# Kloudy-Sky/openintel

Hardware: AMD Instinct MI355X
Metric: queries/sec + p50 latency, 10M-post/768-d hybrid BM25+cosine+RRF top-100 (higher is better)
Workload: dtype f32

## Files before the change

### openintel_amd/csrc/cosine_prefilter.hip

```cpp
#include <algorithm>
#include <cstdlib>
#include <type_traits>

#include "oi_device.h"
#include "oi_internal.h"
#include "oi_lds_dma.h"

typedef float pf_f32x16 __attribute__((ext_vector_type(16)));
typedef float pf_f32x4 __attribute__((ext_vector_type(4)));
typedef __bf16 pf_bf16x8 __attribute__((ext_vector_type(8)));

#define PF_TILE_ROWS 32
#define PF_SLOT_K 32
#define PF_SLOT_BYTES (PF_TILE_ROWS * 128)

__device__ __forceinline__ pf_bf16x8 pf_pack(const pf_f32x4 &a, const pf_f32x4 &b) {
    pf_bf16x8 r;
    r[0] = (__bf16)a[0]; r[1] = (__bf16)a[1]; r[2] = (__bf16)a[2]; r[3] = (__bf16)a[3];
    r[4] = (__bf16)b[0]; r[5] = (__bf16)b[1]; r[6] = (__bf16)b[2]; r[7] = (__bf16)b[3];
    return r;
}

template <int D, int NQT>
__global__ __launch_bounds__(256, 1) void cosine_screen_filter(
    const float *__restrict__ rows, uint64_t row_begin, uint64_t row_end,
    const uint16_t *__restrict__ queries,
    uint32_t n_queries, uint32_t doc_id_base, uint64_t *pools, uint32_t *seg_cnt, uint32_t seg_cnt_stride,
    const uint32_t *tau_keys, uint64_t pool_stride, uint32_t carry_cap, uint32_t seg_cap, uint32_t *overflow) {
    constexpr int NKC = D / PF_SLOT_K;
    constexpr int NBUF = NKC % 8 == 0 ? 8 : (NKC % 6 == 0 ? 6 : NKC);
    constexpr int P = NBUF - 1;
    constexpr int KSTEPS = D / 16;
    static_assert(D % PF_SLOT_K == 0 && NKC % NBUF == 0 && P >= 1 && P < NKC, "unsupported D");
    static_assert(NQT * KSTEPS * 4 <= 400, "the query block must fit the register file");

    extern __shared__ __attribute__((aligned(1024))) unsigned char smem[];
    unsigned char *ring = smem;
    uint32_t *seg_fill = reinterpret_cast<uint32_t *>(smem + 4 * NBUF * PF_SLOT_BYTES);

    OI_CLAIM_WHOLE_SIMD();
    const uint32_t tid = threadIdx.x, lane = tid & 63;
    const uint32_t w = __builtin_amdgcn_readfirstlane(tid >> 6);
    const uint32_t li = lane & 31, lh = lane >> 5;
    uint64_t *stage_keys = reinterpret_cast<uint64_t *>(smem + 4 * NBUF * PF_SLOT_BYTES + 256) + w * OI_STAGE;
    uint32_t *stage_q = reinterpret_cast<uint32_t *>(smem + 4 * NBUF * PF_SLOT_BYTES + 256 + 4 * OI_STAGE * 8) + w * OI_STAGE;
    uint32_t st_head = 0, st_n = 0;

    pf_bf16x8 qreg[NQT][KSTEPS];
#pragma unroll
    for (int t = 0; t < NQT; ++t)
#pragma unroll
        for (int s = 0; s < KSTEPS; ++s)
            qreg[t][s] = *reinterpret_cast<const pf_bf16x8 *>(queries + (uint64_t)(32 * t + li) * D + 16 * s + 8 * lh);
    float tauf[NQT];
#pragma unroll
    for (int t = 0; t < NQT; ++t) {
        const uint32_t q = 32u * t + li;
        const uint32_t k = q < n_queries ? tau_keys[q] : 0xFFFFFFFFu;
        tauf[t] = k <= 0x007FFFFFu ? -__builtin_inff() : oi_key_f32(k);
    }
    if (tid < 32 * NQT) seg_fill[tid] = 0;
    __syncthreads();

    const uint64_t n_rows = row_end - row_begin;
    const uint64_t n_tiles = (n_rows + PF_TILE_ROWS - 1) / PF_TILE_ROWS;
    const uint64_t first = (uint64_t)blockIdx.x * 4 + w, stride = (uint64_t)gridDim.x * 4;
    const uint64_t my_nt = first < n_tiles ? (n_tiles - first + stride - 1) / stride : 0;
    uint64_t *my_seg = pools + carry_cap + (uint64_t)blockIdx.x * seg_cap;

    if (my_nt) {
        uint32_t voff[4];
#pragma unroll
        for (int m = 0; m < 4; ++m) {
            const uint32_t prow = 8 * m + (lane >> 3);
            voff[m] = prow * (uint32_t)(D * 4) + (((lane & 7) ^ ((prow >> 1) & 7)) << 4);
        }
        const uint32_t ring_w = oi_lds_addr(ring) + w * (NBUF * PF_SLOT_BYTES);
        const unsigned char *ring_rd = ring + w * (NBUF * PF_SLOT_BYTES);
        uint32_t frag_off[2][2];
#pragma unroll
        for (int g = 0; g < 2; ++g)
#pragma unroll
            for (int h = 0; h < 2; ++h) frag_off[g][h] = li * 128 + (((4 * g + 2 * lh + h) ^ ((li >> 1) & 7)) << 4);

        auto tile_row0 = [&](uint64_t ti) { return row_begin + (first + ti * stride) * (uint64_t)PF_TILE_ROWS; };
        auto tile_srd = [&](uint64_t ti) {
            const uint64_t r0 = tile_row0(ti < my_nt ? ti : 0);
            return oi_make_srd(rows + r0 * D, ti < my_nt ? (row_end - r0) * (uint64_t)(D * 4) : 0ull);
        };
        oi_u32x4 cur = tile_srd(0), nxt = tile_srd(1);
        __builtin_amdgcn_s_waitcnt(0x0F70);
#pragma unroll
        for (int kc = 0; kc < P; ++kc)
#pragma unroll
            for (int m = 0; m < 4; ++m)
                oi_dma_piece(cur, voff[m], kc * 128, ring_w + (kc % NBUF) * PF_SLOT_BYTES + m * 1024);

        for (uint64_t ti = 0; ti < my_nt; ++ti) {
            pf_f32x16 acc[NQT];
#pragma unroll
            for (int t = 0; t < NQT; ++t)
#pragma unroll
                for (int r = 0; r < 16; ++r) acc[t][r] = 0.f;

            oi_wait_vm<4 * (P - 1)>();
            pf_bf16x8 a_cur = pf_pack(*reinterpret_cast<const pf_f32x4 *>(ring_rd + frag_off[0][0]),
                                      *reinterpret_cast<const pf_f32x4 *>(ring_rd + frag_off[0][1]));
            oi_static_for<0, NKC * 2>([&](auto gi_) {
                constexpr int gi = decltype(gi_)::value;
                constexpr int kc = gi / 2, g = gi % 2;
                constexpr int sn = kc + P;
                pf_f32x4 f0, f1;
                if constexpr (g == 0) {
                    f0 = *reinterpret_cast<const pf_f32x4 *>(ring_rd + (kc % NBUF) * PF_SLOT_BYTES + frag_off[1][0]);
                    f1 = *reinterpret_cast<const pf_f32x4 *>(ring_rd + (kc % NBUF) * PF_SLOT_BYTES + frag_off[1][1]);
                }
#pragma unroll
                for (int t = 0; t < NQT; ++t)
                    acc[t] = __builtin_amdgcn_mfma_f32_32x32x16_bf16(a_cur, qreg[t][gi], acc[t], 0, 0, 0);
#pragma unroll
                for (int m = 2 * g; m < 2 * g + 2; ++m) {
                    if constexpr (sn < NKC)
                        oi_dma_piece(cur, voff[m], sn * 128, ring_w + (sn % NBUF) * PF_SLOT_BYTES + m * 1024);
                    else
                        oi_dma_piece(nxt, voff[m], (sn - NKC) * 128, ring_w + (sn % NBUF) * PF_SLOT_BYTES + m * 1024);
                }
                if constexpr (g == 1 && kc + 1 < NKC) {
                    oi_wait_vm<4 * (P - 1)>();
                    f0 = *reinterpret_cast<const pf_f32x4 *>(ring_rd + ((kc + 1) % NBUF) * PF_SLOT_BYTES + frag_off[0][0]);
                    f1 = *reinterpret_cast<const pf_f32x4 *>(ring_rd + ((kc + 1) % NBUF) * PF_SLOT_BYTES + frag_off[0][1]);
                }
                if constexpr (gi + 1 < NKC * 2) a_cur = pf_pack(f0, f1);
            });

            const uint64_t row0 = tile_row0(ti);
            uint32_t m = 0;
#pragma unroll
            for (int t = 0; t < NQT; ++t)
#pragma unroll
                for (int r = 0; r < 16; ++r) m |= acc[t][r] >= tauf[t] ? 1u << (16 * t + r) : 0u;
            if (row_end - row0 < (uint64_t)PF_TILE_ROWS) {
                const uint32_t left = (uint32_t)(row_end - row0);
#pragma unroll
                for (int r = 0; r < 16; ++r)
                    if ((uint32_t)((r & 3) + 8 * (r >> 2)) + 4u * lh >= left) m &= ~(0x00010001u << r);
            }
            if (__builtin_amdgcn_ballot_w64(m != 0u) != 0ull) {
                const uint32_t cnt = (uint32_t)__builtin_popcount(m);
                const uint32_t incl = oi_wave_incl_scan(cnt);
                const uint32_t total = (uint32_t)__builtin_amdgcn_readlane((int)incl, 63);
                if (total <= OI_STAGE - OI_STAGE_FLUSH) {
                    uint32_t idx = st_head + st_n + incl - cnt;
#pragma unroll
                    for (int t = 0; t < NQT; ++t)
#pragma unroll
                        for (int r = 0; r < 16; ++r)
                            if (m & (1u << (16 * t + r))) {
                                const uint32_t row = (uint32_t)row0 + (r & 3) + 8 * (r >> 2) + 4 * lh;
                                stage_keys[idx & (OI_STAGE - 1)] = oi_rank_key(acc[t][r], doc_id_base + row);
                                stage_q[idx & (OI_STAGE - 1)] = 32u * t + li;
                                ++idx;
                            }
                    st_n += total;
                    while (st_n >= OI_STAGE_FLUSH) {
                        OI_STAGE_FLUSH_TO_POOL(OI_STAGE_FLUSH);
                    }
                } else {
                    uint32_t pos[NQT];
#pragma unroll
                    for (int t = 0; t < NQT; ++t)
                        pos[t] = atomicAdd(&seg_fill[32u * t + li], (uint32_t)__builtin_popcount((m >> (16 * t)) & 0xFFFFu));
#pragma unroll
                    for (int t = 0; t < NQT; ++t) {
                        uint64_t *dst = my_seg + (uint64_t)(32u * t + li) * pool_stride;
#pragma unroll
                        for (int r = 0; r < 16; ++r) {
                            if (m & (1u << (16 * t + r))) {
                                const uint32_t row = (uint32_t)row0 + (r & 3) + 8 * (r >> 2) + 4 * lh;
                                if (pos[t] < seg_cap) dst[pos[t]] = oi_rank_key(acc[t][r], doc_id_base + row);
                                else *overflow = 1u;
                                ++pos[t];
                            }
                        }
                    }
                }
            }
            cur = nxt;
            nxt = tile_srd(ti + 2);
        }
        if (st_n) {
            OI_STAGE_FLUSH_TO_POOL(st_n);
        }
    }
    __syncthreads();
    if (tid < 32 * NQT && tid < n_queries) {
        const uint32_t c = seg_fill[tid];
        seg_cnt[(uint64_t)tid * seg_cnt_stride + blockIdx.x] = c < seg_cap ? c : seg_cap;
    }
}

__global__ __launch_bounds__(256) void pf_row_norm_max_kernel(const float *__restrict__ rows, uint64_t n, uint32_t dim,
                                                              uint32_t *out) {
    double sum_x2 = 0.0, sum_e2 = 0.0;
    const uint32_t lane = threadIdx.x & 63;
    const uint64_t wave = ((uint64_t)blockIdx.x * blockDim.x + threadIdx.x) >> 6;
    const uint64_t n_waves = ((uint64_t)gridDim.x * blockDim.x) >> 6;
    const uint32_t nvec = dim >> 2;
    float best = 0.f, best_e = 0.f;
    bool bad = false;
    for (uint64_t r = wave; r < n; r += n_waves) {
        const float4 *x = reinterpret_cast<const float4 *>(rows + r * dim);
        float ss = 0.f, se = 0.f;
        for (uint32_t v = lane; v < nvec; v += 64) {
            const float4 a = x[v];
            ss = fmaf(a.x, a.x, ss); ss = fmaf(a.y, a.y, ss); ss = fmaf(a.z, a.z, ss); ss = fmaf(a.w, a.w, ss);
            const pf_f32x4 f = {a.x, a.y, a.z, a.w};
            const pf_bf16x8 b = pf_pack(f, f);
            const float e0 = (float)b[0] - a.x, e1 = (float)b[1] - a.y, e2 = (float)b[2] - a.z, e3 = (float)b[3] - a.w;
            se = fmaf(e0, e0, se); se = fmaf(e1, e1, se); se = fmaf(e2, e2, se); se = fmaf(e3, e3, se);
        }
        ss = oi_wave_sum(ss);
        se = oi_wave_sum(se);
        const float nm = sqrtf(ss), ne = sqrtf(se);
        bad = bad || !(nm == nm) || !(ne == ne);
        best = nm > best ? nm : best;
        best_e = ne > best_e ? ne : best_e;
        sum_x2 += (double)ss;
        sum_e2 += (double)se;
    }
    if (lane == 0) {
        atomicMax(out, bad ? 0x7FC00000u : __float_as_uint(best));
        atomicMax(out + 1, bad ? 0x7FC00000u : __float_as_uint(best_e));
        atomicAdd(reinterpret_cast<double *>(out + 2), sum_x2);
        atomicAdd(reinterpret_cast<double *>(out + 4), sum_e2);
    }
}

__global__ __launch_bounds__(256) void pf_row_norm_class_kernel(const float *__restrict__ rows, uint64_t n, uint32_t dim, float X0,
                                                                float E0, uint32_t *cls, uint32_t *bitmap, uint32_t *list,
                                                                uint32_t cap) {
    const uint32_t lane = threadIdx.x & 63;
    const uint64_t wave = ((uint64_t)blockIdx.x * blockDim.x + threadIdx.x) >> 6;
    const uint64_t n_waves = ((uint64_t)gridDim.x * blockDim.x) >> 6;
    const uint32_t nvec = dim >> 2;
    float best = 0.f, best_e = 0.f;
    for (uint64_t r = wave; r < n; r += n_waves) {
        const float4 *x = reinterpret_cast<const float4 *>(rows + r * dim);
        float ss = 0.f, se = 0.f;
        for (uint32_t v = lane; v < nvec; v += 64) {
            const float4 a = x[v];
            ss = fmaf(a.x, a.x, ss); ss = fmaf(a.y, a.y, ss); ss = fmaf(a.z, a.z, ss); ss = fmaf(a.w, a.w, ss);
            const pf_f32x4 f = {a.x, a.y, a.z, a.w};
            const pf_bf16x8 b = pf_pack(f, f);
            const float e0 = (float)b[0] - a.x, e1 = (float)b[1] - a.y, e2 = (float)b[2] - a.z, e3 = (float)b[3] - a.w;
            se = fmaf(e0, e0, se); se = fmaf(e1, e1, se); se = fmaf(e2, e2, se); se = fmaf(e3, e3, se);
        }
        ss = oi_wave_sum(ss);
        se = oi_wave_sum(se);
        const float nm = sqrtf(ss), ne = sqrtf(se);
        if (nm > X0 || ne > E0) {
            if (lane == 0) {
                const uint32_t pos = atomicAdd(cls + 2, 1u);
                if (pos < cap) list[pos] = (uint32_t)r;
                atomicOr(bitmap + (r >> 5), 1u << (r & 31));
            }
        } else {
            best = nm > best ? nm : best;
            best_e = ne > best_e ? ne : best_e;
        }
    }
    if (lane == 0) {
        atomicMax(cls, __float_as_uint(best));
        atomicMax(cls + 1, __float_as_uint(best_e));
    }
}

#define PF_NORM_LIMIT 1.0e15f
#define PF_QNORM_MIN 1.0e-12f
__device__ __forceinline__ float pf_eps(float X, float E, float qn, float qtn, float en, uint32_t dim) {
    const float tiny = 4.0e-18f, d = (float)dim;
    const float Xs = X + tiny, Es = E + tiny, qts = qtn + tiny, ens = en + tiny;
    const float acc = d * 2.384185791015625e-07f;
    return 1.001f * (Es * qts + Xs * ens + acc * (Xs + Es) * qts) + d * 7.5231638452626401e-37f * (Xs + qn) + 1.0e-30f;
}

__global__ __launch_bounds__(256) void pf_stage_queries_kernel(const float *__restrict__ q, uint32_t n_queries,
                                                               uint32_t n_padded, uint32_t dim,
                                                               const uint32_t *__restrict__ max_norm_bits,
                                                               uint16_t *__restrict__ out, float *__restrict__ eps2,
                                                               uint32_t *gate) {
    const uint32_t lane = threadIdx.x & 63;
    const uint32_t wave = (blockIdx.x * blockDim.x + threadIdx.x) >> 6, n_waves = (gridDim.x * blockDim.x) >> 6;
    for (uint32_t row = wave; row < n_padded; row += n_waves) {
        float ss = 0.f, st = 0.f, se = 0.f;
        for (uint32_t k = lane; k < dim; k += 64) {
            uint16_t v = 0;
            if (row < n_queries) {
                const float f = q[(uint64_t)row * dim + k];
                const uint32_t u = __float_as_uint(f);
                v = (u & 0x7F800000u) == 0x7F800000u ? (uint16_t)(u >> 16)
                                                     : (uint16_t)((u + 0x7FFFu + ((u >> 16) & 1u)) >> 16);
                const float ft = __uint_as_float((uint32_t)v << 16), e = ft - f;
                ss = fmaf(f, f, ss);
                st = fmaf(ft, ft, st);
                se = fmaf(e, e, se);
            }
            out[(uint64_t)row * dim + k] = v;
        }
        if (row < n_queries) {
            ss = oi_wave_sum(ss);
            st = oi_wave_sum(st);
            se = oi_wave_sum(se);
            const float qn = sqrtf(ss), qtn = sqrtf(st), en = sqrtf(se);
            const float X = __uint_as_float(max_norm_bits[0]), E = __uint_as_float(max_norm_bits[1]);
            const bool ok = qn < PF_NORM_LIMIT && qn >= PF_QNORM_MIN && qtn < PF_NORM_LIMIT && X < PF_NORM_LIMIT &&
                            E < PF_NORM_LIMIT && en == en;
            if (lane == 0) {
                eps2[row] = ok ? 2.0f * pf_eps(X, E, qn, qtn, en, dim) : __builtin_inff();
                if (!ok) *gate = 1u;
            }
        }
    }
}

__global__ __launch_bounds__(64) void pf_probe_kernel(const float *__restrict__ rows, uint64_t row_begin, uint32_t n_rows,
                                                      uint32_t dim, const uint16_t *__restrict__ queries,
                                                      uint32_t n_queries, float *__restrict__ out) {
    const uint32_t lane = threadIdx.x, li = lane & 31, lh = lane >> 5;
    const uint32_t r0 = blockIdx.x * 32, q0 = blockIdx.y * 32;
    pf_f32x16 acc;
#pragma unroll
    for (int r = 0; r < 16; ++r) acc[r] = 0.f;
    const uint32_t row = r0 + li < n_rows ? r0 + li : n_rows - 1;
    const float *x = rows + (row_begin + row) * (uint64_t)dim;
    const uint16_t *qq = queries + (uint64_t)(q0 + li) * dim;
    for (uint32_t k = 0; k < dim; k += 16) {
        const pf_bf16x8 a = pf_pack(*reinterpret_cast<const pf_f32x4 *>(x + k + 8 * lh),
                                    *reinterpret_cast<const pf_f32x4 *>(x + k + 8 * lh + 4));
        const pf_bf16x8 b = *reinterpret_cast<const pf_bf16x8 *>(qq + k + 8 * lh);
        acc = __builtin_amdgcn_mfma_f32_32x32x16_bf16(a, b, acc, 0, 0, 0);
    }
#pragma unroll
    for (int r = 0; r < 16; ++r) {
        const uint32_t rr = r0 + (r & 3) + 8 * (r >> 2) + 4 * lh, qx = q0 + li;
        if (rr < n_rows && qx < n_queries) out[(uint64_t)qx * n_rows + rr] = acc[r];
    }
}

__global__ __launch_bounds__(256) void pf_make_copy_kernel(const float *__restrict__ rows, uint64_t n_vec8, uint4 *__restrict__ out) {
    for (uint64_t i = (uint64_t)blockIdx.x * blockDim.x + threadIdx.x; i < n_vec8; i += (uint64_t)gridDim.x * blockDim.x) {
        const pf_f32x4 a = *reinterpret_cast<const pf_f32x4 *>(rows + i * 8), b = *reinterpret_cast<const pf_f32x4 *>(rows + i * 8 + 4);
        const pf_bf16x8 v = pf_pack(a, b);
        out[i] = *reinterpret_cast<const uint4 *>(&v);
    }
}
int oi_launch_make_screen_copy(oi_ctx *ctx, const float *rows, uint64_t n, uint32_t dim, uint16_t *out) {
    const uint64_t n_vec8 = n * dim / 8;
    if (n_vec8 == 0) return OI_OK;
    const uint64_t blocks = std::min<uint64_t>((n_vec8 + 255) / 256, (uint64_t)ctx->num_cus * 16);
    hipLaunchKernelGGL(pf_make_copy_kernel, dim3((uint32_t)blocks), dim3(256), 0, ctx->stream, rows, n_vec8, reinterpret_cast<uint4 *>(out));
    OI_HIP_CHECK(hipGetLastError());
    return OI_OK;
}

__global__ __launch_bounds__(256) void pf_rescore_kernel(const float *__restrict__ rows, uint32_t dim, uint32_t doc_id_base,
                                                         uint64_t n_rows, const float *__restrict__ queries,
                                                         const uint64_t *__restrict__ in_pools, const uint32_t *__restrict__ in_cnt,
                                                         uint64_t in_stride, uint32_t cap, uint64_t *out_pools,
                                                         uint32_t *out_cnt, uint64_t out_stride,
                                                         const uint32_t *__restrict__ extra_docs, uint32_t n_extra,
                                                         const uint32_t *__restrict__ spec_max, const uint32_t *__restrict__ tau_final,
                                                         uint32_t *gate, uint32_t *fail_host,
                                                         const uint4 *__restrict__ filt, const uint2 *__restrict__ attrs) {
    if (spec_max && blockIdx.x == 0 && threadIdx.x == 0 && spec_max[blockIdx.y] > tau_final[blockIdx.y]) {
        gate[0] = 1u;
        if (fail_host) *fail_host = 1u;
    }
    const uint32_t q = blockIdx.y, lane = threadIdx.x & 63;
    const uint32_t wave = (blockIdx.x * blockDim.x + threadIdx.x) >> 6, n_waves = (gridDim.x * blockDim.x) >> 6;
    uint32_t c0 = in_cnt[q];
    c0 = c0 < cap ? c0 : cap;
    const uint32_t c = c0 + n_extra;
    const uint32_t nvec = dim >> 2;
    const uint4 fq = filt ? filt[q] : make_uint4(0u, 0u, 0u, 0u);
    auto long_passing = [&](uint32_t j) {
        uint32_t cnt = 0;
        for (uint32_t k0 = 0; k0 < j; k0 += 64) {
            const uint32_t k = k0 + lane;
            cnt += (uint32_t)__popcll(__builtin_amdgcn_ballot_w64(k < j && oi_doc_passes(fq, attrs[extra_docs[k]])));
        }
        return cnt;
    };
    const float4 *qv = reinterpret_cast<const float4 *>(queries + (uint64_t)q * dim);
    for (uint32_t i0 = wave * 4u; i0 < c; i0 += n_waves * 4u) {
        uint32_t doc[4];
        const float4 *x[4];
        float a[4];
#pragma unroll
        for (int u = 0; u < 4; ++u) {
            const uint32_t i = i0 + u < c ? i0 + u : c - 1u;
            doc[u] = i < c0 ? oi_rank_key_doc(in_pools[(uint64_t)q * in_stride + i]) : doc_id_base + extra_docs[i - c0];
            const uint64_t r = (uint64_t)(doc[u] - doc_id_base);
            x[u] = reinterpret_cast<const float4 *>(rows + (r < n_rows ? r : 0) * dim);
            a[u] = 0.f;
        }
        for (uint32_t v = lane; v < nvec; v += 64) {
            const float4 yv = qv[v];
            float4 xv[4];
#pragma unroll
            for (int u = 0; u < 4; ++u) xv[u] = oi_load_stream(x[u] + v);
#pragma unroll
            for (int u = 0; u < 4; ++u) {
                a[u] = oi_fma_unpacked(xv[u].x, yv.x, a[u]); a[u] = oi_fma_unpacked(xv[u].y, yv.y, a[u]);
                a[u] = oi_fma_unpacked(xv[u].z, yv.z, a[u]); a[u] = oi_fma_unpacked(xv[u].w, yv.w, a[u]);
            }
        }
#pragma unroll
        for (int u = 0; u < 4; ++u) {
            const uint64_t r = (uint64_t)(doc[u] - doc_id_base);
            float s = oi_wave_sum(a[u]);
            if (!(r < n_rows)) s = 0.f;
            if (filt && i0 + u >= c0 && i0 + u < c) {
                const uint32_t j = i0 + u - c0, slot = c0 + long_passing(j);
                if (lane == 0 && oi_doc_passes(fq, attrs[extra_docs[j]])) out_pools[(uint64_t)q * out_stride + slot] = oi_rank_key(s, doc[u]);
                continue;
            }
            if (lane == 0 && i0 + u < c) out_pools[(uint64_t)q * out_stride + i0 + u] = oi_rank_key(s, doc[u]);
        }
    }
    if (filt) {
        if (blockIdx.x == 0 && threadIdx.x < 64) {
            const uint32_t cf = c0 + long_passing(n_extra);
            if (threadIdx.x == 0) out_cnt[q] = cf;
        }
    } else if (blockIdx.x == 0 && threadIdx.x == 0) out_cnt[q] = c;
}

__global__ __launch_bounds__(256) void pf_spec_kernel(const uint64_t *__restrict__ pools, const uint32_t *__restrict__ carry_cnt,
                                                      uint64_t stride, uint32_t cap, uint32_t r, const float *__restrict__ eps2,
                                                      const uint32_t *__restrict__ tau_keys, uint32_t *spec_tau, uint32_t *spec_max) {
    __shared__ uint32_t hist[256];
    __shared__ uint32_t s_prefix, s_rank;
    const uint32_t q = blockIdx.x, tid = threadIdx.x;
    uint32_t c = carry_cnt[q];
    if (c > cap) c = cap;
    const uint32_t tau = tau_keys[q];
    if (r == 0 || c < r) {
        if (tid == 0) spec_tau[q] = tau;
        return;
    }
    const uint64_t *k = pools + (uint64_t)q * stride;
    if (tid == 0) { s_prefix = 0; s_rank = r; }
    for (int shift = 24; shift >= 0; shift -= 8) {
        hist[tid] = 0;
        __syncthreads();
        const uint32_t prefix = s_prefix, rank = s_rank, himask = shift == 24 ? 0u : 0xFFFFFFFFu << (shift + 8);
        for (uint32_t i = tid; i < c; i += 256) {
            const uint32_t sk = (uint32_t)(k[i] >> 32);
            if ((sk & himask) == prefix) atomicAdd(&hist[(sk >> shift) & 255u], 1u);
        }
        __syncthreads();
        if (tid < 64) {
            const uint32_t h0 = hist[4 * tid], h1 = hist[4 * tid + 1], h2 = hist[4 * tid + 2], h3 = hist[4 * tid + 3];
            const uint32_t own = h0 + h1 + h2 + h3;
            uint32_t v = own;
#pragma unroll
            for (int o = 1; o < 64; o <<= 1) {
                const uint32_t t = __shfl_down(v, o, 64);
                if (tid + o < 64) v += t;
            }
            uint32_t above = v - own;
            const uint32_t hd[4] = {h3, h2, h1, h0};
#pragma unroll
            for (int d = 0; d < 4; ++d) {
                if (above < rank && rank <= above + hd[d]) {
                    s_prefix = prefix | ((uint32_t)(4 * tid + 3 - d) << shift);
                    s_rank = rank - above;
                }
                above += hd[d];
            }
        }
        __syncthreads();
    }
    if (tid == 0) {
        const float s = oi_key_f32(s_prefix) - eps2[q];
        const uint32_t T = s == s ? oi_f32_key(s) : 0u;
        const uint32_t st = T > tau ? T : tau;
        spec_tau[q] = st;
        if (st > tau && st > spec_max[q]) spec_max[q] = st;
    }
}
int oi_launch_spec_threshold(oi_ctx *ctx, const PoolView &pool, uint32_t n_queries, uint32_t r, const float *eps2, uint32_t *spec_tau,
                             uint32_t *spec_max) {
    if (n_queries == 0) return OI_OK;
    ProfScope ps(ctx, "spec");
    hipLaunchKernelGGL(pf_spec_kernel, dim3(n_queries), dim3(256), 0, ctx->stream, pool.keys, pool.carry_cnt, pool.stride, pool.carry_cap, r,
                       eps2, pool.tau_keys, spec_tau, spec_max);
    OI_HIP_CHECK(hipGetLastError());
    return OI_OK;
}

bool oi_cosine_screen_supported(uint32_t dim) { return dim == 384 || dim == 768; }

void oi_cosine_screen_geometry(const oi_ctx *ctx, uint64_t n_rows, uint32_t *n_segs, uint32_t *seg_cap) {
    const uint64_t n_tiles = (n_rows + PF_TILE_ROWS - 1) / PF_TILE_ROWS;
    const uint64_t quads = (n_tiles + 3) / 4;
    const char *cus_s = oi_ablation_env("OI_SCREEN_CUS");
    const uint64_t cus = cus_s ? (uint64_t)std::max(1, atoi(cus_s)) : std::max<uint64_t>(1, (uint64_t)ctx->num_cus * 7 / 8);
    static const bool small_full = oi_ablation_env("OI_SCREEN_SMALL_FULL") != nullptr;
    const uint64_t grid = small_full && quads <= (uint64_t)ctx->num_cus ? (quads ? quads : 1) : (quads < cus ? (quads ? quads : 1) : cus);
    *n_segs = (uint32_t)grid;
    *seg_cap = (uint32_t)((quads + grid - 1) / grid) * 4 * PF_TILE_ROWS;
}

int oi_launch_row_norm_classes(oi_ctx *ctx, const float *rows, uint64_t n, uint32_t dim, float X0, float E0, uint32_t *cls,
                               uint32_t *bitmap, uint32_t *list, uint32_t cap) {
    OI_HIP_CHECK(hipMemsetAsync(cls, 0, 16, ctx->stream));
    OI_HIP_CHECK(hipMemsetAsync(bitmap, 0, ((n + 31) / 32) * 4, ctx->stream));
    uint64_t blocks = (n + 3) / 4;
    const uint64_t capb = (uint64_t)ctx->num_cus * 8;
    if (blocks > capb) blocks = capb;
    hipLaunchKernelGGL(pf_row_norm_class_kernel, dim3((uint32_t)blocks), dim3(256), 0, ctx->stream, rows, n, dim, X0, E0, cls, bitmap,
                       list, cap);
    OI_HIP_CHECK(hipGetLastError());
    return OI_OK;
}

int oi_launch_row_norm_max(oi_ctx *ctx, const float *rows, uint64_t n, uint32_t dim, uint32_t *max_bits) {
    OI_HIP_CHECK(hipMemsetAsync(max_bits, 0, 24, ctx->stream));
    if (n == 0) return OI_OK;
    uint64_t blocks = (n + 3) / 4;
    const uint64_t cap = (uint64_t)ctx->num_cus * 8;
    if (blocks > cap) blocks = cap;
    hipLaunchKernelGGL(pf_row_norm_max_kernel, dim3((uint32_t)blocks), dim3(256), 0, ctx->stream, rows, n, dim, max_bits);
    OI_HIP_CHECK(hipGetLastError());
    return OI_OK;
}

int oi_launch_screen_stage(oi_ctx *ctx, const float *d_queries, uint32_t n_queries, uint32_t dim,
                           const uint32_t *max_norm_bits, uint16_t *q_bf16, float *eps2, uint32_t *gate) {
    const uint32_t n_padded = (n_queries + 31u) & ~31u;
    hipLaunchKernelGGL(pf_stage_queries_kernel, dim3((n_padded + 3) / 4), dim3(256), 0, ctx->stream, d_queries, n_queries,
                       n_padded, dim, max_norm_bits, q_bf16, eps2, gate);
    OI_HIP_CHECK(hipGetLastError());
    return OI_OK;
}

template <int D, int NQT>
static int launch_screen(oi_ctx *ctx, const float *rows, uint64_t row_begin, uint64_t row_end, const uint16_t *q,
                         uint32_t nq, uint32_t doc_id_base, const PoolView &p) {
    constexpr int NKC = D / PF_SLOT_K, NBUF = NKC % 8 == 0 ? 8 : (NKC % 6 == 0 ? 6 : NKC);
    constexpr size_t smem = 4 * NBUF * PF_SLOT_BYTES + 64 * 4 + OI_STAGE_LDS;
    OI_CHECK(oi_dyn_lds(ctx, reinterpret_cast<const void *>(cosine_screen_filter<D, NQT>), (size_t)(smem)));
    hipLaunchKernelGGL((cosine_screen_filter<D, NQT>), dim3(p.n_segs), dim3(256), smem, ctx->stream, rows, row_begin,
                       row_end, q, nq, doc_id_base, p.keys, p.seg_cnt, p.seg_cnt_stride, p.tau_keys, p.stride,
                       p.carry_cap, p.seg_cap, p.overflow);
    OI_HIP_CHECK(hipGetLastError());
    return OI_OK;
}

int oi_launch_cosine_screen_chunk(oi_ctx *ctx, const float *rows, uint64_t row_begin, uint64_t row_end, uint32_t dim,
                                  const uint16_t *q_bf16, uint32_t n_queries, uint32_t doc_id_base, PoolView &pool) {
    OI_REQUIRE(oi_cosine_screen_supported(dim), "cosine screen: dim %u not instantiated (384, 768)", dim);
    oi_cosine_screen_geometry(ctx, row_end > row_begin ? row_end - row_begin : 0, &pool.n_segs, &pool.seg_cap);
    OI_REQUIRE(pool.n_segs <= pool.seg_cnt_stride && pool.carry_cap + (uint64_t)pool.n_segs * pool.seg_cap <= pool.stride,
               "cosine screen: chunk does not fit the candidate pool");
    OI_REQUIRE(!pool.filt, "cosine screen: a filtered search does not take the f32-stream screen (search.hip routes it)");
    if (row_end <= row_begin || n_queries == 0) return OI_OK;
    ProfScope ps(ctx, "cosine");
    for (uint32_t q0 = 0; q0 < n_queries; q0 += 64) {
        const uint32_t nq_here = std::min(64u, n_queries - q0);
        PoolView p = pool.for_queries(q0);
        static const bool tau_max = oi_ablation_env("OI_SCREEN_TAU_MAX") != nullptr;
        if (tau_max && row_end - row_begin >= (1u << 20)) {
            DevBuf &tb = ctx->buf("abl_tau_max");
            if (!tb.p) { OI_CHECK(tb.ensure(4096 * 4)); OI_HIP_CHECK(hipMemsetAsync(tb.p, 0xFF, 4096 * 4, ctx->stream)); }
            p.tau_keys = tb.as<uint32_t>();
        }
        const uint16_t *qptr = q_bf16 + (uint64_t)q0 * dim;
        const bool two = nq_here > 32;
        if (dim == 768) {
            if (two) OI_CHECK((launch_screen<768, 2>(ctx, rows, row_begin, row_end, qptr, nq_here, doc_id_base, p)));
            else OI_CHECK((launch_screen<768, 1>(ctx, rows, row_begin, row_end, qptr, nq_here, doc_id_base, p)));
        } else {
            if (two) OI_CHECK((launch_screen<384, 2>(ctx, rows, row_begin, row_end, qptr, nq_here, doc_id_base, p)));
            else OI_CHECK((launch_screen<384, 1>(ctx, rows, row_begin, row_end, qptr, nq_here, doc_id_base, p)));
        }
    }
    return OI_OK;
}

int oi_launch_rescore(oi_ctx *ctx, const float *rows, uint64_t n_rows, uint32_t dim, uint32_t doc_id_base,
                      const float *d_queries, uint32_t n_queries, const PoolView &in, const PoolView &out,
                      const uint32_t *extra_docs, uint32_t n_extra, const uint32_t *spec_max, const uint32_t *tau_final,
                      uint32_t *gate, uint32_t *fail_host) {
    if (n_queries == 0) return OI_OK;
    OI_REQUIRE(out.carry_cap >= in.carry_cap + n_extra, "rescore: output pool too small");
    ProfScope ps(ctx, "rescore");
    hipLaunchKernelGGL(pf_rescore_kernel, dim3(64, n_queries), dim3(256), 0, ctx->stream, rows, dim, doc_id_base, n_rows,
                       d_queries, in.keys, in.carry_cnt, in.stride, in.carry_cap, out.keys, out.carry_cnt, out.stride, extra_docs,
                       n_extra, spec_max, tau_final, gate, fail_host, out.filt, out.attrs);
    OI_HIP_CHECK(hipGetLastError());
    return OI_OK;
}

int oi_launch_screen_probe(oi_ctx *ctx, const float *rows, uint64_t row_begin, uint32_t n_rows, uint32_t dim,
                           const uint16_t *q_bf16, uint32_t n_queries, float *d_out) {
    if (n_rows == 0 || n_queries == 0) return OI_OK;
    OI_REQUIRE(dim % 16 == 0, "screen probe: dim %u is not a multiple of 16", dim);
    hipLaunchKernelGGL(pf_probe_kernel, dim3((n_rows + 31) / 32, (n_queries + 31) / 32), dim3(64), 0, ctx->stream, rows,
                       row_begin, n_rows, dim, q_bf16, n_queries, d_out);
    OI_HIP_CHECK(hipGetLastError());
    return OI_OK;
}
```

### openintel_amd/csrc/cosine_screen_i8.hip

```cpp
#include <algorithm>
#include <cmath>
#include <cstdlib>
#include <type_traits>

#include "oi_device.h"
#include "oi_internal.h"
#include "oi_lds_dma.h"

typedef int i8s_i32x4 __attribute__((ext_vector_type(4)));
typedef int i8s_i32x16 __attribute__((ext_vector_type(16)));
typedef float i8s_f32x2 __attribute__((ext_vector_type(2)));
template <int N>
struct i8s_ivec {
    typedef int type __attribute__((ext_vector_type(N)));
};

#define I8S_TILE_ROWS 32
#define I8S_SLOT_BYTES (I8S_TILE_ROWS * 128)
#define I8S_META_BYTES 256
#define I8S_PAD_ROWS 64

size_t oi_screen_i8_meta_offset(uint64_t n, uint32_t dim) { return ((size_t)n * dim + 255) & ~(size_t)255; }
size_t oi_screen_i8_bytes(uint64_t n, uint32_t dim) {
    return oi_screen_i8_meta_offset(n, dim) + 8 * ((size_t)n + I8S_PAD_ROWS) + 256;
}

__global__ __launch_bounds__(256) void i8s_make_kernel(const float *__restrict__ rows, uint64_t n, uint32_t dim,
                                                       const uint32_t *__restrict__ long_bitmap, uint32_t *__restrict__ out_i8,
                                                       float *__restrict__ meta, uint32_t *__restrict__ emax_bits) {
    const uint32_t lane = threadIdx.x & 63;
    const uint64_t wave = ((uint64_t)blockIdx.x * blockDim.x + threadIdx.x) >> 6;
    const uint64_t n_waves = ((uint64_t)gridDim.x * blockDim.x) >> 6;
    const uint32_t nv = dim >> 2;
    float best = 0.f;
    for (uint64_t r = wave; r < n; r += n_waves) {
        const float4 *x = reinterpret_cast<const float4 *>(rows + r * dim);
        float4 v[3];
        float amax = 0.f;
#pragma unroll
        for (int u = 0; u < 3; ++u) {
            const uint32_t j = lane + 64u * u;
            v[u] = j < nv ? x[j] : make_float4(0.f, 0.f, 0.f, 0.f);
            amax = fmaxf(amax, fmaxf(fmaxf(fabsf(v[u].x), fabsf(v[u].y)), fmaxf(fabsf(v[u].z), fabsf(v[u].w))));
        }
#pragma unroll
        for (int o = 32; o > 0; o >>= 1) amax = fmaxf(amax, __shfl_xor(amax, o, OI_WAVE));
        const float s = amax / 127.f;
        double e2 = 0.0;
#pragma unroll
        for (int u = 0; u < 3; ++u) {
            const uint32_t j = lane + 64u * u;
            const float xs[4] = {v[u].x, v[u].y, v[u].z, v[u].w};
            uint32_t packed = 0;
#pragma unroll
            for (int c = 0; c < 4; ++c) {
                float t = s > 0.f ? rintf(xs[c] / s) : 0.f;
                t = fminf(127.f, fmaxf(-127.f, t));
                const int iv = (int)t;
                const double e = (double)s * (double)iv - (double)xs[c];
                e2 += j < nv ? e * e : 0.0;
                packed |= ((uint32_t)iv & 0xFFu) << (8 * c);
            }
            if (j < nv) out_i8[r * nv + j] = packed;
        }
        e2 = oi_wave_sum(e2);
        const float er = (float)sqrt(e2) * 1.00000095367431640625f;
        if (lane == 0) {
            meta[2 * r] = s;
            meta[2 * r + 1] = er;
        }
        const bool is_long = long_bitmap && ((long_bitmap[r >> 5] >> (r & 31)) & 1u);
        if (!is_long) best = fmaxf(best, er);
    }
    if (lane == 0) atomicMax(emax_bits, __float_as_uint(best));
}

int oi_launch_make_screen_i8(oi_ctx *ctx, const float *rows, uint64_t n, uint32_t dim, const uint32_t *long_bitmap, uint8_t *out) {
    OI_REQUIRE(oi_cosine_screen_supported(dim), "int8 screening copy: dim %u not instantiated (384, 768)", dim);
    const size_t mo = oi_screen_i8_meta_offset(n, dim);
    OI_HIP_CHECK(hipMemsetAsync(out + mo, 0, 8 * ((size_t)n + I8S_PAD_ROWS) + 256, ctx->stream));
    if (n == 0) return OI_OK;
    uint64_t blocks = (n + 3) / 4;
    const uint64_t cap = (uint64_t)ctx->num_cus * 8;
    if (blocks > cap) blocks = cap;
    float *meta = reinterpret_cast<float *>(out + mo);
    hipLaunchKernelGGL(i8s_make_kernel, dim3((uint32_t)blocks), dim3(256), 0, ctx->stream, rows, n, dim, long_bitmap,
                       reinterpret_cast<uint32_t *>(out), meta, reinterpret_cast<uint32_t *>(meta + 2 * (n + I8S_PAD_ROWS)));
    OI_HIP_CHECK(hipGetLastError());
    return OI_OK;
}

#define I8S_NORM_LIMIT 1.0e15f
#define I8S_QNORM_MIN 1.0e-12f
__global__ __launch_bounds__(256) void i8s_stage_kernel(const float *__restrict__ q, uint32_t n_queries, uint32_t n_padded, uint32_t dim,
                                                        const uint32_t *__restrict__ max_norm_bits, const uint32_t *__restrict__ emax_bits,
                                                        int8_t *__restrict__ qi8, float *__restrict__ qf, uint32_t *gate) {
    const uint32_t lane = threadIdx.x & 63;
    const uint32_t wave = (blockIdx.x * blockDim.x + threadIdx.x) >> 6, n_waves = (gridDim.x * blockDim.x) >> 6;
    for (uint32_t row = wave; row < n_padded; row += n_waves) {
        const bool real = row < n_queries;
        float amax = 0.f;
        bool fin = true;
        for (uint32_t k = lane; k < dim; k += 64) {
            const float f = real ? q[(uint64_t)row * dim + k] : 0.f;
            fin = fin && (f - f == 0.f);
            amax = fmaxf(amax, fabsf(f));
        }
#pragma unroll
        for (int o = 32; o > 0; o >>= 1) amax = fmaxf(amax, __shfl_xor(amax, o, OI_WAVE));
        fin = __builtin_amdgcn_ballot_w64(!fin) == 0ull;
        const float a = fin ? amax / 127.f : 0.f;
        double qn2 = 0.0, en2 = 0.0;
        for (uint32_t k = lane; k < dim; k += 64) {
            const float f = real ? q[(uint64_t)row * dim + k] : 0.f;
            float h = 0.f, l = 0.f;
            if (a > 0.f) {
                const float t = f / a;
                h = fminf(127.f, fmaxf(-127.f, rintf(t)));
                l = fminf(127.f, fmaxf(-127.f, rintf((t - h) * 128.f)));
            }
            const double qh = (double)a * ((double)h + (double)l * 0.0078125);
            qn2 += qh * qh;
            en2 += (qh - (double)f) * (qh - (double)f);
            qi8[(uint64_t)row * dim + k] = (int8_t)(int)h;
            qi8[((uint64_t)n_padded + row) * dim + k] = (int8_t)(int)l;
        }
        qn2 = oi_wave_sum(qn2);
        en2 = oi_wave_sum(en2);
        if (lane == 0) {
            const float up = 1.00000095367431640625f;
            const float qn = (float)sqrt(qn2) * up, en = (float)sqrt(en2) * up;
            const float X = __uint_as_float(max_norm_bits[0]), em = __uint_as_float(*emax_bits);
            const bool ok = fin && amax > 0.f && qn < I8S_NORM_LIMIT && qn >= I8S_QNORM_MIN && X < I8S_NORM_LIMIT && em < I8S_NORM_LIMIT;
            const float rnd = 3.814697265625e-06f + (float)dim * 2.384185791015625e-07f;
            const float cq = 1.001f * (X * en + rnd * (X + em) * (qn + en)) + 1.0e-27f;
            const float m2 = 2.002f * (em * qn + cq);
            qf[row] = ok ? a : 0.f;
            qf[n_padded + row] = ok ? qn : 0.f;
            qf[2 * n_padded + row] = ok ? cq : 0.f;
            qf[3 * n_padded + row] = ok || !real ? m2 : __builtin_inff();
            if (real && !ok) *gate = 1u;
        }
    }
}

int oi_launch_screen_stage_i8(oi_ctx *ctx, const float *d_queries, uint32_t n_queries, uint32_t dim, const uint32_t *max_norm_bits,
                              const uint8_t *i8_copy, uint64_t n_rows, int8_t *qi8, float *qf, uint32_t *gate) {
    const uint32_t n_padded = (n_queries + 31u) & ~31u;
    if (n_padded == 0) return OI_OK;
    const uint32_t *emax = reinterpret_cast<const uint32_t *>(i8_copy + oi_screen_i8_meta_offset(n_rows, dim)) + 2 * (n_rows + I8S_PAD_ROWS);
    hipLaunchKernelGGL(i8s_stage_kernel, dim3((n_padded + 3) / 4), dim3(256), 0, ctx->stream, d_queries, n_queries, n_padded, dim,
                       max_norm_bits, emax, qi8, qf, gate);
    OI_HIP_CHECK(hipGetLastError());
    return OI_OK;
}

__device__ __forceinline__ void i8s_issue_piece(const oi_u32x4 &srd, uint32_t voff, uint32_t soff, uint32_t lds_dst) {
#ifdef I8S_NO_DMA
    (void)srd; (void)voff; (void)soff; (void)lds_dst;
#else
    oi_dma_piece(srd, voff, soff, lds_dst);
#endif
}
__device__ __forceinline__ void i8s_issue_meta(const oi_u32x4 &srd, uint32_t voff, uint32_t lds_dst) {
#ifdef I8S_NO_DMA
    (void)srd; (void)voff; (void)lds_dst;
#else
    uint32_t keep;
    const uint32_t d = __builtin_amdgcn_readfirstlane(lds_dst);
    asm volatile(
        "s_mov_b32 %0, m0\n\t"
        "s_mov_b32 m0, %3\n\t"
        "s_nop 0\n\t"
        "buffer_load_dword %1, %2, 0 offen " OI_DMA_NT "lds\n\t"
        "s_mov_b32 m0, %0"
        : "=&s"(keep)
        : "v"(voff), "s"(srd), "s"(d)
        : "memory");
#endif
}

template <int D, int NQT, int NBUF, bool FILT>
__global__ __launch_bounds__(256, 1) void cosine_i8_screen(
    const uint8_t *__restrict__ rows, const float *__restrict__ meta, uint64_t row_begin, uint64_t row_end,
    const int8_t *__restrict__ qhi, const int8_t *__restrict__ qlo,
    const float *__restrict__ qf, uint32_t qf_stride, uint32_t n_queries, uint32_t doc_id_base, uint64_t *pools, uint32_t *seg_cnt,
    uint32_t seg_cnt_stride, const uint32_t *tau_keys, uint64_t pool_stride, uint32_t carry_cap, uint32_t seg_cap, uint32_t *overflow,
    const uint4 *__restrict__ filt, const uint2 *__restrict__ attrs) {
    constexpr int NKC = D / 128;
    constexpr int P = NBUF - 1;
    constexpr int KSTEPS = D / 32;
    constexpr uint32_t RING = NBUF * I8S_SLOT_BYTES;
    static_assert(D % 128 == 0 && P >= 2 && P <= 2 * NKC, "unsupported ring depth for this D");
    constexpr uint32_t QLO_LDS = NQT * KSTEPS * 64 * 16;
    static_assert(NQT * KSTEPS * 4 <= 200, "the hi query block must fit the register file");
    static_assert(4 * RING + 4 * 2 * I8S_META_BYTES + 256 + OI_STAGE_LDS + QLO_LDS <= 160 * 1024, "LDS");

    extern __shared__ __attribute__((aligned(1024))) unsigned char smem[];
    unsigned char *ring = smem;
    unsigned char *meta_lds = smem + 4 * RING;
    uint32_t *seg_fill = reinterpret_cast<uint32_t *>(smem + 4 * RING + 8 * I8S_META_BYTES);
    unsigned char *stage_base = smem + 4 * RING + 8 * I8S_META_BYTES + 256;
    unsigned char *qlo_lds = stage_base + OI_STAGE_LDS;

    OI_CLAIM_WHOLE_SIMD();
    const uint32_t tid = threadIdx.x, lane = tid & 63;
    const uint32_t w = __builtin_amdgcn_readfirstlane(tid >> 6);
    const uint32_t li = lane & 31, lh = lane >> 5;
    uint64_t *stage_keys = reinterpret_cast<uint64_t *>(stage_base) + w * OI_STAGE;
    uint32_t *stage_q = reinterpret_cast<uint32_t *>(stage_base + 4 * OI_STAGE * 8) + w * OI_STAGE;
    uint32_t st_head = 0, st_n = 0;

    i8s_i32x4 qh[NQT][KSTEPS];
#pragma unroll
    for (int t = 0; t < NQT; ++t)
#pragma unroll
        for (int s = 0; s < KSTEPS; ++s)
            qh[t][s] = *reinterpret_cast<const i8s_i32x4 *>(qhi + (uint64_t)(32 * t + li) * D + 32 * s + 16 * lh);
    for (uint32_t c = tid; c < (uint32_t)(NQT * KSTEPS * 64); c += 256) {
        const uint32_t t = c / (KSTEPS * 64), s = (c / 64) % KSTEPS, l = c % 64;
        *reinterpret_cast<i8s_i32x4 *>(qlo_lds + c * 16) =
            *reinterpret_cast<const i8s_i32x4 *>(qlo + (uint64_t)(32 * t + (l & 31)) * D + 32 * s + 16 * (l >> 5));
    }
    float qa[NQT], qn[NQT], cq[NQT], tc[NQT];
#pragma unroll
    for (int t = 0; t < NQT; ++t) {
        const uint32_t q = 32u * t + li;
        const bool real = q < n_queries;
        const uint32_t k = real ? tau_keys[q] : 0xFFFFFFFFu;
        const float tau = k <= 0x007FFFFFu ? -__builtin_inff() : oi_key_f32(k);
        qa[t] = real ? qf[q] * 0.0078125f : 0.f;
        qn[t] = real ? qf[qf_stride + q] : 0.f;
        cq[t] = real ? qf[2 * qf_stride + q] : 0.f;
        const float m2 = real ? qf[3 * qf_stride + q] : 0.f;
        const float T = m2 < __builtin_inff() ? (tau + m2) - (fabsf(tau) + m2) * 9.5367431640625e-07f : -__builtin_inff();
        tc[t] = T - cq[t];
    }
    if (tid < 32 * NQT) seg_fill[tid] = 0;
#ifdef I8S_NO_DMA
    for (uint32_t i = tid; i < (4 * RING + 8 * I8S_META_BYTES) / 4; i += 256) reinterpret_cast<uint32_t *>(smem)[i] = 0u;
#endif
    __syncthreads();

    const uint64_t n_rows = row_end - row_begin;
    const uint64_t n_tiles = (n_rows + I8S_TILE_ROWS - 1) / I8S_TILE_ROWS;
    const uint64_t first = (uint64_t)blockIdx.x * 4 + w, stride = (uint64_t)gridDim.x * 4;
    const uint64_t my_nt = first < n_tiles ? (n_tiles - first + stride - 1) / stride : 0;
    uint64_t *my_seg = pools + carry_cap + (uint64_t)blockIdx.x * seg_cap;

    if (my_nt) {
        uint32_t voff[4];
#pragma unroll
        for (int m = 0; m < 4; ++m) {
            const uint32_t prow = 8 * m + (lane >> 3);
            voff[m] = prow * (uint32_t)D + (((lane & 7) ^ ((prow >> 1) & 7)) << 4);
        }
        const uint32_t ring_w = oi_lds_addr(ring) + w * RING;
        const unsigned char *ring_rd = ring + w * RING;
        const uint32_t meta_w = oi_lds_addr(meta_lds) + w * 2 * I8S_META_BYTES;
        const unsigned char *meta_rd = meta_lds + w * 2 * I8S_META_BYTES;
        uint32_t frag_off[4];
#pragma unroll
        for (int g = 0; g < 4; ++g) frag_off[g] = li * 128 + (((2 * g + lh) ^ ((li >> 1) & 7)) << 4);

        auto tile_row0 = [&](uint64_t ti) { return row_begin + (first + ti * stride) * (uint64_t)I8S_TILE_ROWS; };
        auto tile_srd = [&](uint64_t ti) {
            const uint64_t r0 = tile_row0(ti < my_nt ? ti : 0);
            return oi_make_srd(rows + r0 * D, ti < my_nt ? (row_end - r0) * (uint64_t)D : 0ull);
        };
        auto issue_meta = [&](uint64_t ti) {
            const uint64_t r0 = tile_row0(ti);
            i8s_issue_meta(oi_make_srd(meta + 2 * r0, (row_end - r0) * 8ull), lane * 4u, meta_w + (uint32_t)(ti & 1) * I8S_META_BYTES);
        };
        oi_u32x4 s0 = tile_srd(0), s1 = tile_srd(1), s2 = tile_srd(2);
        __builtin_amdgcn_s_waitcnt(0x0F70);
        oi_static_for<0, P>([&](auto j_) {
            constexpr int j = decltype(j_)::value;
            constexpr int tj = j / NKC, kj = j % NKC;
#pragma unroll
            for (int m = 0; m < 4; ++m)
                i8s_issue_piece(tj == 0 ? s0 : (tj == 1 ? s1 : s2), voff[m], kj * 128, ring_w + j * I8S_SLOT_BYTES + m * 1024);
        });
        issue_meta(0);
        uint32_t rd_off = 0, wr_off = (NBUF - 1) * I8S_SLOT_BYTES;
        auto lo_frag = [&](int t, int s) {
            return *reinterpret_cast<const i8s_i32x4 *>(qlo_lds + ((t * KSTEPS + s) * 64 + lane) * 16);
        };
        i8s_i32x4 b_cur[NQT];
#ifndef I8S_NO_MFMA
#pragma unroll
        for (int t = 0; t < NQT; ++t) b_cur[t] = lo_frag(t, 0);
#endif

        oi_wait_vm<4 * (P - 1)>();
        i8s_i32x4 a_cur = *reinterpret_cast<const i8s_i32x4 *>(ring_rd + frag_off[0]);

        constexpr int NS = 16 * NQT;
        constexpr int RPK = KSTEPS >= 20 ? 1 : 2;
        constexpr int NSL = 16 / RPK, T0 = 4;
        static_assert(T0 + NSL <= KSTEPS, "the tile test does not fit the span");
        static_assert(4 * NKC + 4 >= 4 * (P - 1) - 1, "the ring's wait in k-step 3 must retire the previous tile's metadata");
        typename i8s_ivec<NS>::type S;
#pragma unroll
        for (int i = 0; i < NS; ++i) S[i] = 0;
        i8s_i32x16 ah[NQT], al[NQT];
        i8s_f32x2 md_cur[RPK];
#pragma unroll
        for (int u = 0; u < RPK; ++u) md_cur[u] = i8s_f32x2{0.f, 0.f};
        const uint32_t lh32 = 32u * lh;
        auto meta_row = [&](const unsigned char *mt, int r) {
            return *reinterpret_cast<const i8s_f32x2 *>(mt + lh32 + ((r & 3) + 8 * (r >> 2)) * 8);
        };
        auto test_row = [&](int t, int r, const i8s_f32x2 md) -> uint32_t {
            const float sc = oi_mul_unpacked((float)S[16 * t + r], oi_mul_unpacked(md[0], qa[t]));
            return sc >= oi_fma_unpacked(-md[1], qn[t], tc[t]) ? 1u << (16 * t + r) : 0u;
        };

        for (uint64_t ti = 0;; ++ti) {
            const bool live = ti < my_nt;
            const unsigned char *mt = meta_rd + (uint32_t)((ti + 1) & 1) * I8S_META_BYTES;
            uint32_t m = 0;
            if (live) {
#pragma unroll
                for (int t = 0; t < NQT; ++t)
#pragma unroll
                    for (int r = 0; r < 16; ++r) { ah[t][r] = 0; al[t][r] = 0; }

                oi_static_for<0, NKC * 4>([&](auto gi_) {
                    constexpr int gi = decltype(gi_)::value;
                    constexpr int kc = gi / 4, g = gi % 4;
                    constexpr int sn = kc + P;
                    constexpr int tn = sn / NKC, kn = sn % NKC;
                    i8s_i32x4 a_nxt;
                    if constexpr (g < 3) {
                        a_nxt = *reinterpret_cast<const i8s_i32x4 *>(ring_rd + rd_off + frag_off[g + 1]);
                    } else {
                        oi_wait_vm<4 * (P - 1) - 1>();
                        const uint32_t nx_off = rd_off + I8S_SLOT_BYTES == RING ? 0u : rd_off + I8S_SLOT_BYTES;
                        a_nxt = *reinterpret_cast<const i8s_i32x4 *>(ring_rd + nx_off + frag_off[0]);
                    }
                    i8s_f32x2 md_nxt[RPK];
                    if constexpr (gi >= T0 - 1 && gi < T0 - 1 + NSL) {
#pragma unroll
                        for (int u = 0; u < RPK; ++u) md_nxt[u] = meta_row(mt, RPK * (gi - (T0 - 1)) + u);
                    }
#ifndef I8S_NO_MFMA
                    i8s_i32x4 b_nxt[NQT];
#pragma unroll
                    for (int t = 0; t < NQT; ++t) b_nxt[t] = lo_frag(t, (gi + 1) % KSTEPS);
#endif
                    __builtin_amdgcn_sched_barrier(0);
#pragma unroll
                    for (int t = 0; t < NQT; ++t) {
#ifndef I8S_NO_MFMA
                        ah[t] = __builtin_amdgcn_mfma_i32_32x32x32_i8(a_cur, qh[t][gi], ah[t], 0, 0, 0);
                        al[t] = __builtin_amdgcn_mfma_i32_32x32x32_i8(a_cur, b_cur[t], al[t], 0, 0, 0);
#else
                        asm volatile("" : : "v"(a_cur));
#endif
                        if constexpr (gi >= T0 && gi < T0 + NSL) if (t == 0) {
#pragma unroll
                            for (int u = 0; u < RPK; ++u)
#pragma unroll
                                for (int tt = 0; tt < NQT; ++tt) m |= test_row(tt, RPK * (gi - T0) + u, md_cur[u]);
                            asm volatile("" : "+v"(m));
                        }
                        __builtin_amdgcn_sched_barrier(0);
                    }
#ifndef I8S_NO_MFMA
#pragma unroll
                    for (int t = 0; t < NQT; ++t) b_cur[t] = b_nxt[t];
#endif
                    if constexpr (gi >= T0 - 1 && gi < T0 - 1 + NSL) {
#pragma unroll
                        for (int u = 0; u < RPK; ++u) md_cur[u] = md_nxt[u];
                    }
                    i8s_issue_piece(tn == 0 ? s0 : (tn == 1 ? s1 : s2), voff[g], kn * 128, ring_w + wr_off + g * 1024);
                    if constexpr (g == 3) {
                        wr_off = rd_off;
                        rd_off = rd_off + I8S_SLOT_BYTES == RING ? 0u : rd_off + I8S_SLOT_BYTES;
                    }
                    a_cur = a_nxt;
                });
            } else {
                oi_wait_vm<0>();
#pragma unroll
                for (int r = 0; r < 16; ++r) {
                    const i8s_f32x2 md = meta_row(mt, r);
#pragma unroll
                    for (int t = 0; t < NQT; ++t) m |= test_row(t, r, md);
                }
            }

            const uint64_t row0 = tile_row0(ti ? ti - 1 : 0);
            if (ti == 0) m = 0u;
            if (row_end - row0 < (uint64_t)I8S_TILE_ROWS) {
                const uint32_t left = (uint32_t)(row_end - row0);
#pragma unroll
                for (int r = 0; r < 16; ++r)
                    if ((uint32_t)((r & 3) + 8 * (r >> 2)) + 4u * lh >= left) m &= ~(0x00010001u << r);
            }
#if defined(I8S_NO_DMA) || defined(I8S_NO_MFMA)
            if (seg_cap != 0xFFFFFFFFu) m = 0u;
#endif
            if (__builtin_amdgcn_ballot_w64(m != 0u) != 0ull) {
                if constexpr (FILT) m = oi_filter_tile<NQT>(m, filt, attrs, row0, lh, li);
                const uint32_t cnt = (uint32_t)__builtin_popcount(m);
                const uint32_t incl = oi_wave_incl_scan(cnt);
                const uint32_t total = (uint32_t)__builtin_amdgcn_readlane((int)incl, 63);
                const uint32_t any = oi_wave_or(m);
                auto lower_key = [&](int t, uint32_t r) -> uint64_t {
                    const uint32_t rit = (r & 3) + 8 * (r >> 2) + 4 * lh;
                    const i8s_f32x2 md = *reinterpret_cast<const i8s_f32x2 *>(mt + rit * 8);
                    const float sc = (float)S[16 * t + r] * (md[0] * qa[t]);
                    return oi_rank_key(sc - fmaf(md[1], qn[t], cq[t]), doc_id_base + ((uint32_t)row0 + rit));
                };
                if (total <= OI_STAGE - OI_STAGE_FLUSH) {
                    uint32_t idx = st_head + st_n + incl - cnt;
#pragma unroll
                    for (int t = 0; t < NQT; ++t)
                        for (uint32_t wd = (any >> (16 * t)) & 0xFFFFu; wd; wd &= wd - 1) {
                            const uint32_t r = (uint32_t)__builtin_ctz(wd);
                            if (m & (1u << (16 * t + r))) {
                                stage_keys[idx & (OI_STAGE - 1)] = lower_key(t, r);
                                stage_q[idx & (OI_STAGE - 1)] = 32u * t + li;
                                ++idx;
                            }
                        }
                    st_n += total;
                    while (st_n >= OI_STAGE_FLUSH) {
                        OI_STAGE_FLUSH_TO_POOL(OI_STAGE_FLUSH);
                    }
                } else {
                    uint32_t pos[NQT];
#pragma unroll
                    for (int t = 0; t < NQT; ++t)
                        pos[t] = atomicAdd(&seg_fill[32u * t + li], (uint32_t)__builtin_popcount((m >> (16 * t)) & 0xFFFFu));
#pragma unroll
                    for (int t = 0; t < NQT; ++t) {
                        uint64_t *dst = my_seg + (uint64_t)(32u * t + li) * pool_stride;
                        for (uint32_t wd = (any >> (16 * t)) & 0xFFFFu; wd; wd &= wd - 1) {
                            const uint32_t r = (uint32_t)__builtin_ctz(wd);
                            if (m & (1u << (16 * t + r))) {
                                if (pos[t] < seg_cap) dst[pos[t]] = lower_key(t, r);
                                else *overflow = 1u;
                                ++pos[t];
                            }
                        }
                    }
                }
            }
            if (!live) break;
#pragma unroll
            for (int t = 0; t < NQT; ++t)
#pragma unroll
                for (int r = 0; r < 16; ++r) S[16 * t + r] = ah[t][r] * 128 + al[t][r];
            if (ti + 1 < my_nt) issue_meta(ti + 1);
            s0 = s1;
            s1 = s2;
            s2 = tile_srd(ti + 3);
        }
        if (st_n) {
            OI_STAGE_FLUSH_TO_POOL(st_n);
        }
        oi_wait_vm<0>();
    }
    __syncthreads();
    if (tid < 32 * NQT && tid < n_queries) {
        const uint32_t c = seg_fill[tid];
        seg_cnt[(uint64_t)tid * seg_cnt_stride + blockIdx.x] = c < seg_cap ? c : seg_cap;
    }
}

template <int D, int NQT, int NBUF, bool FILT>
static int launch_i8_screen_k(oi_ctx *ctx, const uint8_t *rows, const float *meta, uint64_t row_begin, uint64_t row_end, const int8_t *qhi,
                              const int8_t *qlo, const float *qf, uint32_t qf_stride, uint32_t nq, uint32_t doc_id_base, const PoolView &p) {
    constexpr size_t smem = 4 * NBUF * I8S_SLOT_BYTES + 8 * I8S_META_BYTES + 256 + OI_STAGE_LDS + NQT * (D / 32) * 64 * 16;
    OI_CHECK(oi_dyn_lds(ctx, reinterpret_cast<const void *>(cosine_i8_screen<D, NQT, NBUF, FILT>), (size_t)(smem)));
    hipLaunchKernelGGL((cosine_i8_screen<D, NQT, NBUF, FILT>), dim3(p.n_segs), dim3(256), smem, ctx->stream, rows, meta, row_begin, row_end,
                       qhi, qlo, qf, qf_stride, nq, doc_id_base, p.keys, p.seg_cnt, p.seg_cnt_stride, p.tau_keys, p.stride, p.carry_cap,
                       p.seg_cap, p.overflow, p.filt, p.attrs);
    OI_HIP_CHECK(hipGetLastError());
    return OI_OK;
}
template <int D, int NQT, int NBUF>
static int launch_i8_screen(oi_ctx *ctx, const uint8_t *rows, const float *meta, uint64_t row_begin, uint64_t row_end, const int8_t *qhi,
                            const int8_t *qlo, const float *qf, uint32_t qf_stride, uint32_t nq, uint32_t doc_id_base, const PoolView &p) {
    return p.filt ? launch_i8_screen_k<D, NQT, NBUF, true>(ctx, rows, meta, row_begin, row_end, qhi, qlo, qf, qf_stride, nq, doc_id_base, p)
                  : launch_i8_screen_k<D, NQT, NBUF, false>(ctx, rows, meta, row_begin, row_end, qhi, qlo, qf, qf_stride, nq, doc_id_base, p);
}

int oi_launch_cosine_screen_i8_chunk(oi_ctx *ctx, const uint8_t *i8_copy, uint64_t n_rows_total, uint64_t row_begin, uint64_t row_end,
                                     uint32_t dim, const int8_t *qi8, const float *qf, uint32_t n_queries, uint32_t doc_id_base,
                                     PoolView &pool) {
    OI_REQUIRE(oi_cosine_screen_supported(dim), "cosine screen (int8): dim %u not instantiated (384, 768)", dim);
    OI_REQUIRE(row_end <= n_rows_total, "cosine screen (int8): rows past the copy");
    oi_cosine_screen_geometry(ctx, row_end > row_begin ? row_end - row_begin : 0, &pool.n_segs, &pool.seg_cap);
    OI_REQUIRE(pool.n_segs <= pool.seg_cnt_stride && pool.carry_cap + (uint64_t)pool.n_segs * pool.seg_cap <= pool.stride,
               "cosine screen (int8): chunk does not fit the candidate pool");
    if (row_end <= row_begin || n_queries == 0) return OI_OK;
    const float *meta = reinterpret_cast<const float *>(i8_copy + oi_screen_i8_meta_offset(n_rows_total, dim));
    const uint32_t np = (n_queries + 31u) & ~31u;
    ProfScope ps(ctx, "cosine");
    for (uint32_t q0 = 0; q0 < n_queries; q0 += 64) {
        const uint32_t nq_here = std::min(64u, n_queries - q0);
        const PoolView p = pool.for_queries(q0);
        const int8_t *qhi = qi8 + (uint64_t)q0 * dim, *qlo = qi8 + ((uint64_t)np + q0) * dim;
        const float *qfp = qf + q0;
        const bool two = nq_here > 32;
        if (dim == 768) {
            if (two) OI_CHECK((launch_i8_screen<768, 2, 6>(ctx, i8_copy, meta, row_begin, row_end, qhi, qlo, qfp, np, nq_here, doc_id_base, p)));
            else OI_CHECK((launch_i8_screen<768, 1, 6>(ctx, i8_copy, meta, row_begin, row_end, qhi, qlo, qfp, np, nq_here, doc_id_base, p)));
        } else {
            if (two) OI_CHECK((launch_i8_screen<384, 2, 6>(ctx, i8_copy, meta, row_begin, row_end, qhi, qlo, qfp, np, nq_here, doc_id_base, p)));
            else OI_CHECK((launch_i8_screen<384, 1, 6>(ctx, i8_copy, meta, row_begin, row_end, qhi, qlo, qfp, np, nq_here, doc_id_base, p)));
        }
    }
    return OI_OK;
}

__device__ __forceinline__ float i8s_bf16_lo(uint32_t w) { return __uint_as_float(w << 16); }
__device__ __forceinline__ float i8s_bf16_hi(uint32_t w) { return __uint_as_float(w & 0xFFFF0000u); }
__global__ __launch_bounds__(256) void pf_rescreen_kernel(const uint16_t *__restrict__ copy, uint64_t n_rows, uint32_t dim,
                                                          uint32_t doc_id_base, const uint16_t *__restrict__ qb, uint64_t *pools,
                                                          const uint32_t *__restrict__ cnt, uint64_t stride, uint32_t cap) {
    const uint32_t q = blockIdx.y, lane = threadIdx.x & 63;
    const uint32_t wave = (blockIdx.x * blockDim.x + threadIdx.x) >> 6, n_waves = (gridDim.x * blockDim.x) >> 6;
    uint32_t c = cnt[q];
    c = c < cap ? c : cap;
    uint64_t *keys = pools + (uint64_t)q * stride;
    const uint32_t nvec = dim >> 3;
    const uint4 *qv = reinterpret_cast<const uint4 *>(qb + (uint64_t)q * dim);
    for (uint32_t i0 = wave * 4u; i0 < c; i0 += n_waves * 4u) {
        uint32_t doc[4];
        const uint4 *x[4];
        float a[4];
#pragma unroll
        for (int u = 0; u < 4; ++u) {
            const uint32_t i = i0 + u < c ? i0 + u : c - 1u;
            doc[u] = oi_rank_key_doc(keys[i]);
            const uint64_t r = (uint64_t)(doc[u] - doc_id_base);
            x[u] = reinterpret_cast<const uint4 *>(copy + (r < n_rows ? r : 0) * dim);
            a[u] = 0.f;
        }
        for (uint32_t v = lane; v < nvec; v += 64) {
            const uint4 yv = qv[v];
            uint4 xv[4];
#pragma unroll
            for (int u = 0; u < 4; ++u) xv[u] = oi_load_stream(x[u] + v);
#pragma unroll
            for (int u = 0; u < 4; ++u) {
                const uint32_t xw[4] = {xv[u].x, xv[u].y, xv[u].z, xv[u].w}, yw[4] = {yv.x, yv.y, yv.z, yv.w};
#pragma unroll
                for (int e = 0; e < 4; ++e) {
                    a[u] = oi_fma_unpacked(i8s_bf16_lo(xw[e]), i8s_bf16_lo(yw[e]), a[u]);
                    a[u] = oi_fma_unpacked(i8s_bf16_hi(xw[e]), i8s_bf16_hi(yw[e]), a[u]);
                }
            }
        }
        float s[4];
#pragma unroll
        for (int u = 0; u < 4; ++u) s[u] = oi_wave_sum(a[u]);
#pragma unroll
        for (int u = 0; u < 4; ++u) {
            const uint64_t r = (uint64_t)(doc[u] - doc_id_base);
            const float sc = r < n_rows ? s[u] : 0.f;
            if (lane == 0 && i0 + u < c) keys[i0 + u] = oi_rank_key(sc, doc[u]);
        }
    }
}

int oi_launch_rescreen_bf16(oi_ctx *ctx, const uint16_t *copy_rows, uint64_t n_rows, uint32_t dim, uint32_t doc_id_base,
                            const uint16_t *q_bf16, uint32_t n_queries, const PoolView &pool) {
    if (n_queries == 0) return OI_OK;
    ProfScope ps(ctx, "rescreen");
    hipLaunchKernelGGL(pf_rescreen_kernel, dim3(32, n_queries), dim3(256), 0, ctx->stream, copy_rows, n_rows, dim, doc_id_base, q_bf16,
                       pool.keys, pool.carry_cnt, pool.stride, pool.carry_cap);
    OI_HIP_CHECK(hipGetLastError());
    return OI_OK;
}
```

### openintel_amd/csrc/oi_internal.h

```cpp
#pragma once

#include <hip/hip_runtime.h>

#include <cstdarg>
#include <cstdint>
#include <cstdio>
#include <cstdlib>
#include <cstring>
#include <atomic>
#include <map>
#include <mutex>
#include <string>
#include <utility>
#include <vector>

#include "openintel_hip.h"

void oi_set_error(const char *fmt, ...);

#define OI_HIP_CHECK(expr)                                                                   \
    do {                                                                                     \
        hipError_t oi_e_ = (expr);                                                           \
        if (oi_e_ != hipSuccess) {                                                           \
            oi_set_error("%s failed: %s (%s:%d)", #expr, hipGetErrorString(oi_e_), __FILE__, \
                         __LINE__);                                                          \
            return OI_ERR_HIP;                                                               \
        }                                                                                    \
    } while (0)

#define OI_CHECK(expr)              \
    do {                            \
        int oi_rc_ = (expr);        \
        if (oi_rc_ != OI_OK) return oi_rc_; \
    } while (0)

#define OI_REQUIRE(cond, ...)         \
    do {                              \
        if (!(cond)) {                \
            oi_set_error(__VA_ARGS__); \
            return OI_ERR_INVALID_ARG; \
        }                             \
    } while (0)

struct oi_ctx;
int oi_dyn_lds(oi_ctx *ctx, const void *kernel, size_t bytes);

#ifdef OI_ABLATION
inline const char *oi_ablation_env(const char *name) { return getenv(name); }
#else
inline const char *oi_ablation_env(const char *) { return nullptr; }
#endif

struct DevBuf {
    void *p = nullptr;
    size_t cap = 0;
    bool borrowed = false;
    DevBuf() = default;
    DevBuf(const DevBuf &) = delete;
    DevBuf &operator=(const DevBuf &) = delete;
    ~DevBuf() { release(); }
    int ensure(size_t bytes);
    void release();
    template <class T> T *as() const { return reinterpret_cast<T *>(p); }
};

#define OI_PINNED_STAGE_MAX ((size_t)1 << 20)
struct PinBuf {
    void *p = nullptr;
    size_t cap = 0;
    bool pinned = false;
    PinBuf() = default;
    PinBuf(const PinBuf &) = delete;
    PinBuf &operator=(const PinBuf &) = delete;
    int ensure(size_t bytes);
    void release();
    template <class T> T *as() const { return reinterpret_cast<T *>(p); }
};

struct ProfSpan {
    hipEvent_t a, b;
};

extern std::atomic<uint64_t> g_oi_ws_epoch;

struct GraphEntry {
    uint64_t key[10] = {0, 0, 0, 0, 0, 0, 0, 0, 0, 0};
    uint64_t epoch = 0, last_use = 0;
    int state = 0;
    hipGraph_t graph = nullptr;
    hipGraphExec_t exec = nullptr;
};

struct oi_ctx {
    std::atomic<int> refs{1};
    int device = 0;
    int num_cus = 256;
    hipStream_t stream = nullptr;
    hipStream_t side_stream = nullptr;
    bool side_stream_failed = false;
    hipEvent_t ev_fork = nullptr, ev_join = nullptr;
    bool overlap_legs = true;
    bool speculate = true;
    uint32_t spec_skip = 0, spec_backoff = 0;
    uint32_t *spec_fail_host = nullptr;
    uint64_t spec_searches = 0, spec_failures = 0;
    int cosine_mode = 2;
    std::mutex mu;
    std::map<std::string, DevBuf> ws;
    int prof_enabled = 0;
    const uint32_t *run_gate = nullptr;
    const uint32_t *last_screen_gate = nullptr;
    std::map<std::string, std::vector<ProfSpan>> prof;
    std::vector<hipEvent_t> event_pool;
    bool use_graphs = false;
    std::vector<GraphEntry> graphs;
    uint64_t graph_clock = 0, graph_replays = 0, graph_captures = 0;

    PinBuf pin_in, pin_out;

    DevBuf &buf(const char *name) { return ws[name]; }
    void prof_begin(const char *tag);
    void prof_end(const char *tag);
};

struct ProfScope {
    oi_ctx *c;
    const char *tag;
    bool on;
    ProfScope(oi_ctx *ctx, const char *t) : c(ctx), tag(t) {
        on = c->prof_enabled == 1 || (c->prof_enabled == 2 && strcmp(t, "cosine") == 0);
        if (on) c->prof_begin(tag);
    }
    ~ProfScope() {
        if (on) c->prof_end(tag);
    }
};

#define OI_BM25_FLOOR_RANKS 4
struct oi_index {
    uint64_t uid = 0;
    std::atomic<int> refs{1};
    oi_index *src = nullptr;
    oi_ctx *ctx = nullptr;
    uint64_t n_docs = 0;
    uint32_t dim = 0, vocab = 0, doc_id_base = 0;

    float *rows = nullptr;
    bool rows_owned = false;
    uint16_t *rows_bf16 = nullptr;
    bool rows_bf16_owned = false;
    DevBuf max_row_norm;
    bool screen_ok = false;
    uint32_t n_long = 0;
    DevBuf long_list, long_bitmap;
    DevBuf screen_copy;
    int screen_copy_policy = -1;
    DevBuf screen_i8;
    DevBuf doc_attrs;
    DevBuf signals;

    bool forward_set = false, finalized = false;
    uint64_t total_tokens = 0;
    uint64_t n_postings = 0;
    uint32_t n_blocks = 0;
    uint32_t n_win = 0;
    DevBuf uniq_keys;
    DevBuf tf;
    DevBuf doc_len;
    DevBuf df_local;

    DevBuf postings;
    DevBuf cell_start;
    DevBuf idf;
    DevBuf impact_floor;
    DevBuf fwd_terms;
    DevBuf fwd_offsets;
    float avgdl = 0.f;
    uint32_t max_query_terms = 16;
    int bm25_mode = 0;
    bool is_view = false;
};

int search_lists_device(oi_index *idx, const float *d_qv, const uint32_t *d_qt, const uint32_t *d_qo, uint32_t B, uint32_t depth,
                        float *cos_s, uint32_t *cos_d, uint32_t *cos_c, float *bm_s, uint32_t *bm_d, uint32_t *bm_c,
                        const uint4 *d_filt = nullptr, const uint2 *d_attrs = nullptr);
void oi_spec_take_failure(oi_ctx *ctx);

int oi_launch_lexicon(oi_ctx *ctx, const uint8_t *d_blob, const uint64_t *d_offsets, uint64_t n,
                      uint64_t blob_bytes, double *d_pol, uint8_t *d_spec);
int oi_launch_lexicon_fused(oi_ctx *ctx, const uint8_t *d_blob, const uint64_t *d_offsets, uint64_t n, uint64_t blob_bytes,
                            double *d_pol, uint8_t *d_spec, const uint8_t *d_sources, double tau, oi_social_counters *summary);
int oi_launch_social_summary(oi_ctx *ctx, const uint8_t *d_sources, const double *d_pol,
                             const uint8_t *d_spec, uint64_t n, double tau,
                             oi_social_counters *out_host);
int oi_launch_social_summary_segmented(oi_ctx *ctx, const uint8_t *d_sources, const double *d_pol, const uint8_t *d_spec,
                                       uint64_t n, const uint64_t *d_seg, uint64_t n_seg, double tau,
                                       oi_social_counters *d_out);
int oi_launch_headline_scan(oi_ctx *ctx, const uint8_t *d_blob, const uint64_t *d_offsets, uint64_t n,
                            uint64_t blob_bytes, const uint8_t *ticker, uint64_t ticker_len,
                            const uint8_t *forms_blob, const uint32_t *form_offsets, uint32_t n_forms,
                            uint16_t *d_mask, uint64_t *d_order, uint8_t *d_about);
size_t oi_headline_params_bytes();
int oi_headline_build_params(void *dst, const uint8_t *ticker, uint64_t ticker_len, const uint8_t *forms_blob,
                             const uint32_t *form_offsets, uint32_t n_forms);
int oi_launch_headline_scan_params(oi_ctx *ctx, const uint8_t *d_blob, const uint64_t *d_offsets, uint64_t n,
                                   uint64_t blob_bytes, uint64_t text_bytes, const void *d_params, uint16_t *d_mask,
                                   uint64_t *d_order, uint8_t *d_about);
struct PoolView {
    uint64_t *keys;
    uint32_t *carry_cnt;
    uint32_t *seg_cnt;
    uint32_t *tau_keys;
    uint64_t stride;
    uint32_t carry_cap;
    uint32_t seg_cap;
    uint32_t n_segs;
    uint32_t seg_cnt_stride;
    uint32_t *overflow;
    const uint4 *filt = nullptr;
    const uint2 *attrs = nullptr;

    PoolView for_queries(uint32_t q0) const {
        PoolView p = *this;
        p.keys += (uint64_t)q0 * stride;
        p.carry_cnt += q0;
        p.seg_cnt += (uint64_t)q0 * seg_cnt_stride;
        if (p.tau_keys) p.tau_keys += q0;
        if (p.filt) p.filt += q0;
        return p;
    }
};
struct SelectExtra {
    const float *eps2 = nullptr;
    uint32_t *margin_gate = nullptr;
    const uint32_t *run_gate = nullptr;
    const uint32_t *skip_bitmap = nullptr;
    uint32_t skip_base = 0;
    uint64_t *cand = nullptr;
    uint32_t cand_cap = 0;
    const float *row_meta = nullptr;
    uint32_t meta_base = 0;
    const float *row_qn = nullptr, *row_cq = nullptr;
};
int oi_launch_select(oi_ctx *ctx, const PoolView &pool, uint32_t n_queries, uint32_t k, bool compact,
                     float *out_scores, uint32_t *out_docs, uint32_t *out_counts, uint32_t out_stride,
                     const SelectExtra *extra = nullptr);
int oi_launch_lists_to_pool(oi_ctx *ctx, const float *scores, const uint32_t *docs,
                            const uint32_t *counts, uint64_t shard_stride, uint64_t count_stride,
                            uint32_t n_shards, uint32_t n_queries, uint32_t depth, const PoolView &pool);
int oi_launch_rrf(oi_ctx *ctx, const uint32_t *docs_a, const uint32_t *counts_a, const uint32_t *docs_b,
                  const uint32_t *counts_b, uint32_t n_queries, uint32_t depth, uint32_t k,
                  float *scores_out, uint32_t *docs_out, uint32_t *counts_out);
int oi_launch_collapse(oi_index *idx, const float *d_scores, const uint32_t *d_docs, const uint32_t *d_counts, uint32_t n_queries,
                       uint32_t depth, float threshold, uint32_t k, float *scores_out, uint32_t *docs_out, uint32_t *counts_out,
                       uint32_t *dup_out);
int oi_launch_similar_volume(oi_index *idx, const float *d_q, uint32_t n_queries, const oi_volume_spec &spec, const uint4 *d_filt,
                             uint32_t *d_counts);
int oi_launch_volume_round_queries(oi_ctx *ctx, const float *d_q, uint64_t total, float *d_out);
int oi_launch_pack_signals(oi_ctx *ctx, const double *d_pol, const uint8_t *d_spec, const uint8_t *d_sources, uint64_t n, double tau,
                           uint2 *d_out);
int oi_launch_similar_summary(oi_index *idx, const float *d_q, uint32_t n_queries, const oi_summary_spec &spec, const float *d_thresholds,
                              const uint4 *d_filt, oi_social_counters *d_out);
int oi_launch_cosine_chunk(oi_ctx *ctx, const float *rows, uint64_t row_begin, uint64_t row_end,
                           uint32_t dim, const float *d_queries_padded, uint32_t n_queries,
                           uint32_t n_queries_padded, uint32_t doc_id_base, PoolView &pool);
uint64_t oi_cosine_max_chunk_rows(const oi_ctx *ctx, uint32_t dim, uint32_t n_queries, uint64_t stride,
                                  uint32_t carry_cap);
int oi_launch_l2_normalize(oi_ctx *ctx, float *rows, uint64_t n, uint32_t dim);
bool oi_cosine_split_supported(uint32_t dim);
int oi_launch_cosine_split(oi_ctx *ctx, const float *rows, uint64_t row_begin, uint64_t row_end, uint32_t dim,
                           const float *d_queries, uint32_t nq, uint32_t doc_id_base, const PoolView &p);
bool oi_cosine_bf16_supported(uint32_t dim);
int oi_launch_cosine_bf16_chunk(oi_ctx *ctx, const uint16_t *rows, uint64_t row_begin, uint64_t row_end, uint32_t dim,
                                const float *d_queries, uint32_t n_queries, uint32_t doc_id_base, PoolView &pool);
uint32_t oi_cosine_query_padding(uint32_t n_queries);
bool oi_cosine_ksplit_supported(uint32_t dim);
void oi_cosine_ksplit_geometry(const oi_ctx *ctx, uint64_t n_rows, uint32_t *n_segs, uint32_t *seg_cap);
bool oi_cosine_screen_supported(uint32_t dim);
inline bool oi_index_screenable(const oi_index *idx) {
    return idx->rows && !idx->rows_bf16 && idx->screen_ok && oi_cosine_screen_supported(idx->dim);
}
void oi_cosine_screen_geometry(const oi_ctx *ctx, uint64_t n_rows, uint32_t *n_segs, uint32_t *seg_cap);
int oi_launch_row_norm_max(oi_ctx *ctx, const float *rows, uint64_t n, uint32_t dim, uint32_t *max_bits);
int oi_launch_screen_stage(oi_ctx *ctx, const float *d_queries, uint32_t n_queries, uint32_t dim,
                           const uint32_t *max_norm_bits, uint16_t *q_bf16, float *eps2, uint32_t *gate);
int oi_launch_cosine_screen_chunk(oi_ctx *ctx, const float *rows, uint64_t row_begin, uint64_t row_end, uint32_t dim,
                                  const uint16_t *q_bf16, uint32_t n_queries, uint32_t doc_id_base, PoolView &pool);
int oi_launch_make_screen_copy(oi_ctx *ctx, const float *rows, uint64_t n, uint32_t dim, uint16_t *out);
#define OI_I8_CARRY 16384u
size_t oi_screen_i8_bytes(uint64_t n, uint32_t dim);
size_t oi_screen_i8_meta_offset(uint64_t n, uint32_t dim);
int oi_launch_make_screen_i8(oi_ctx *ctx, const float *rows, uint64_t n, uint32_t dim, const uint32_t *long_bitmap, uint8_t *out);
int oi_launch_screen_stage_i8(oi_ctx *ctx, const float *d_queries, uint32_t n_queries, uint32_t dim, const uint32_t *max_norm_bits,
                              const uint8_t *i8_copy, uint64_t n_rows, int8_t *qi8, float *qf, uint32_t *gate);
int oi_launch_cosine_screen_i8_chunk(oi_ctx *ctx, const uint8_t *i8_copy, uint64_t n_rows_total, uint64_t row_begin, uint64_t row_end,
                                     uint32_t dim, const int8_t *qi8, const float *qf, uint32_t n_queries, uint32_t doc_id_base,
                                     PoolView &pool);
int oi_launch_rescreen_bf16(oi_ctx *ctx, const uint16_t *copy_rows, uint64_t n_rows, uint32_t dim, uint32_t doc_id_base,
                            const uint16_t *q_bf16, uint32_t n_queries, const PoolView &pool);
int oi_launch_cosine_screen_copy_chunk(oi_ctx *ctx, const uint16_t *copy_rows, uint64_t row_begin, uint64_t row_end, uint32_t dim,
                                       const uint16_t *q_bf16, uint32_t n_queries, uint32_t doc_id_base, PoolView &pool);
int oi_launch_screen_probe(oi_ctx *ctx, const float *rows, uint64_t row_begin, uint32_t n_rows, uint32_t dim,
                           const uint16_t *q_bf16, uint32_t n_queries, float *d_out);
int oi_launch_spec_threshold(oi_ctx *ctx, const PoolView &pool, uint32_t n_queries, uint32_t r, const float *eps2, uint32_t *spec_tau,
                             uint32_t *spec_max);
int oi_launch_rescore(oi_ctx *ctx, const float *rows, uint64_t n_rows, uint32_t dim, uint32_t doc_id_base,
                      const float *d_queries, uint32_t n_queries, const PoolView &in, const PoolView &out,
                      const uint32_t *extra_docs = nullptr, uint32_t n_extra = 0, const uint32_t *spec_max = nullptr,
                      const uint32_t *tau_final = nullptr, uint32_t *gate = nullptr, uint32_t *fail_host = nullptr);
#define OI_LONG_ROWS_MAX 1024u
int oi_launch_row_norm_classes(oi_ctx *ctx, const float *rows, uint64_t n, uint32_t dim, float X0, float E0, uint32_t *cls,
                               uint32_t *bitmap, uint32_t *list, uint32_t cap);
int oi_launch_cosine_ksplit(oi_ctx *ctx, const float *rows, uint64_t row_begin, uint64_t row_end, uint32_t dim,
                            const float *q, uint32_t nq, bool two_tiles, uint32_t doc_id_base, const PoolView &p);
int oi_bm25_stage_forward(oi_index *idx, const uint32_t *d_terms, const uint64_t *d_offsets);
int oi_bm25_finalize(oi_index *idx, uint64_t global_n, uint64_t global_tokens, const uint32_t *global_df_host);
void oi_bm25_scan_geometry(const oi_ctx *ctx, uint64_t n_docs, uint32_t *n_segs, uint32_t *seg_cap);
uint32_t oi_bm25_scan_pass_queries(uint32_t max_terms_per_query);
int oi_launch_bm25_scan(oi_index *idx, const uint32_t *d_q_terms, const uint32_t *d_q_offsets, uint32_t q_begin,
                        uint32_t nq, uint64_t doc_begin, uint64_t doc_end, float avgdl, bool run_setup,
                        const PoolView &pool);
uint32_t oi_bm25_wave_pass_queries(void);
int oi_launch_bm25_wave(oi_index *idx, const uint32_t *d_q_terms, const uint32_t *d_q_offsets, uint32_t q_begin,
                        uint32_t nq, const PoolView &pool, uint32_t block_begin, uint32_t block_end);
uint32_t oi_bm25_stream_pass_queries(void);
uint32_t oi_bm25_stream_seg_cap(uint32_t depth, bool first_phase);
int oi_launch_bm25_plan(oi_index *idx, const uint32_t *d_q_terms, const uint32_t *d_q_offsets, uint32_t q_begin, uint32_t nq,
                        uint32_t *state, uint64_t state_words, uint32_t depth, uint32_t tau_off, uint32_t tau_words, bool with_floors);
int oi_launch_bm25_stream(oi_index *idx, const uint32_t *d_q_terms, const uint32_t *d_q_offsets, uint32_t q_begin,
                          uint32_t nq, uint32_t depth, const PoolView &pool, uint32_t block_begin, uint32_t block_end);
int oi_launch_bm25(oi_index *idx, const uint32_t *d_q_terms, const uint32_t *d_q_offsets,
                   uint32_t n_queries, uint32_t depth, const PoolView &pool, uint32_t block_begin,
                   uint32_t block_end);

struct oi_comm {
    oi_ctx *ctx = nullptr;
    void *nccl = nullptr;
    uint32_t rank = 0, world = 1;
};
int oi_rccl_unique_id(uint8_t *id_out);
int oi_rccl_init(void **comm_out, uint32_t world, const uint8_t *id_bytes, uint32_t rank);
void oi_rccl_destroy(void *comm);
int oi_rccl_all_gather_u32(void *comm, const uint32_t *send, uint32_t *recv, size_t words, hipStream_t st);
int oi_rccl_all_reduce_sum(void *comm, void *buf, size_t count, bool u64, hipStream_t st);
```

### openintel_amd/csrc/search.hip

```cpp
#include <algorithm>

#include "oi_internal.h"

namespace {

int env_int(const char *name, int dflt, int lo) { return oi_ablation_env(name) ? std::max(lo, atoi(oi_ablation_env(name))) : dflt; }
bool env_set(const char *name) { return oi_ablation_env(name) != nullptr; }
struct Knobs {
    uint64_t first_mult = env_int("OI_FIRST_CHUNK_MULT", 1, 1), first_div = env_int("OI_FIRST_CHUNK_DIV", 1, 1);
    uint64_t growth = env_int("OI_CHUNK_GROWTH", 0, 2);
    uint64_t spec_growth = env_int("OI_SPEC_GROWTH", 128, 2), spec_first_div = env_int("OI_SPEC_FIRST_DIV", 4, 1);
    uint32_t bm25_first_div = env_int("OI_BM25_FIRST_DIV", 8, 1);
    bool screen_no_round = env_set("OI_SCREEN_NO_ROUND"), no_spec = env_set("OI_NO_SPEC"), no_overlap = env_set("OI_NO_OVERLAP");
    bool bm25_early = env_set("OI_BM25_EARLY"), small_gemv = env_set("OI_SMALL_BATCH_GEMV"), bm25_two_phase = env_set("OI_BM25_TWO_PHASE");
    bool exact_only = env_set("OI_COSINE_V1") || env_set("OI_SELECT_V1");
};
const Knobs &knobs() { static const Knobs k; return k; }

struct Pools { PoolView cos, bm; };
enum { BM25_TAAT = 1, BM25_SCAN = 2, BM25_WAVE = 3, BM25_STREAM = 4 };
int bm25_mode_of(const oi_index *idx) {
    static const char *mode_env = getenv("OI_BM25_MODE");
    int mode = idx->bm25_mode;
    if (mode == 0 && mode_env)
        mode = strcmp(mode_env, "scan") == 0 ? 2 : strcmp(mode_env, "taat") == 0 ? 1 : strcmp(mode_env, "wave") == 0 ? 3 : 4;
    return mode == 0 ? 4 : mode;
}
int prepare_pools(oi_ctx *ctx, uint32_t B, uint64_t cos_alloc_stride, uint64_t cos_stride, uint32_t carry_cap, uint32_t bm_blocks,
                  uint32_t depth, Pools *out, size_t extra_words, uint32_t **extra) {
    DevBuf &flag = ctx->buf("state_flag");
    if (!flag.p) {
        OI_CHECK(flag.ensure(16));
        OI_HIP_CHECK(hipMemsetAsync(flag.p, 0, 16, ctx->stream));
    }
    const uint32_t cos_segs = (uint32_t)ctx->num_cus * (B <= 8 ? 8u : 1u);
    const uint32_t bm_segs = bm_blocks ? bm_blocks : 1;
    const size_t words = (size_t)B * (2 + cos_segs + 2 + bm_segs);
    DevBuf &st = ctx->buf("pool_state");
    OI_CHECK(st.ensure(sizeof(uint32_t) * (words + extra_words)));
    OI_HIP_CHECK(hipMemsetAsync(st.p, 0, sizeof(uint32_t) * (words + extra_words), ctx->stream));
    *extra = st.as<uint32_t>() + words;
    const uint64_t bm_stride = (uint64_t)carry_cap + (uint64_t)bm_segs * depth;
    DevBuf &pc = ctx->buf("pool_cos"), &pb = ctx->buf("pool_bm");
    OI_CHECK(pc.ensure(sizeof(uint64_t) * (size_t)B * cos_alloc_stride));
    OI_CHECK(pb.ensure(sizeof(uint64_t) * (size_t)B * bm_stride));
    uint32_t *s = st.as<uint32_t>();
    uint32_t *cos_carry = s, *cos_tau = s + B, *cos_seg = s + 2 * (size_t)B;
    uint32_t *bm_carry = cos_seg + (size_t)B * cos_segs, *bm_tau = bm_carry + B, *bm_seg = bm_tau + B;
    out->cos = PoolView{pc.as<uint64_t>(), cos_carry, cos_seg, cos_tau, cos_stride, carry_cap, 0, 0, cos_segs, flag.as<uint32_t>()};
    out->bm = PoolView{pb.as<uint64_t>(), bm_carry, bm_seg, bm_tau, bm_stride, carry_cap, depth, bm_segs, bm_segs, flag.as<uint32_t>()};
    return OI_OK;
}

uint64_t oi_first_chunk_rows(uint32_t depth) {
    return std::max<uint64_t>(std::max<uint64_t>(8192, 32ull * depth) * knobs().first_mult / knobs().first_div, 2ull * depth);
}
uint64_t oi_screen_first_chunk_rows(const oi_ctx *ctx, uint32_t depth) {
    uint64_t rows = oi_first_chunk_rows(depth);
    const uint64_t round = 32ull * 4 * std::max<uint64_t>(1, (uint64_t)ctx->num_cus * 7 / 8);
    if (!knobs().screen_no_round && rows >= round) rows -= rows % round;
    return rows;
}
uint64_t oi_chunk_growth(uint32_t B) { return knobs().growth ? knobs().growth : (B <= 8 ? 16 : 8); }
uint64_t oi_chunk_end(uint64_t r, uint64_t chunk, uint64_t n, uint64_t max_chunk, uint64_t next_chunk) {
    uint64_t e = std::min(n, r + chunk);
    if (e < n && (n - e) * 4 <= (e - r) && n - r <= max_chunk) e = n;
    if (e < n && next_chunk >= max_chunk && n - e > max_chunk && n - r <= 2 * max_chunk) e = n - max_chunk;
    return e;
}

struct Chunk { uint64_t r, e; };
std::vector<Chunk> chunk_schedule(uint64_t n, uint64_t first, uint64_t growth, uint64_t max_chunk, bool stretch_first) {
    std::vector<Chunk> out;
    uint64_t chunk = first, r = 0;
    while (r < n) {
        if (chunk > max_chunk) chunk = max_chunk;
        const uint64_t e = oi_chunk_end(r, chunk, n, max_chunk, r == 0 && !stretch_first ? 0 : chunk * growth);
        out.push_back(Chunk{r, e});
        r = e;
        chunk *= growth;
    }
    return out;
}

struct Search {
    oi_index *idx; oi_ctx *ctx;
    const float *qv; const uint32_t *qt, *qo;
    uint32_t B, depth;
    float *cos_s; uint32_t *cos_d, *cos_c;
    float *bm_s; uint32_t *bm_d, *bm_c;
    const uint4 *filt; const uint2 *attrs;
};
enum class CosRoute { none, bf16, exact, screen_f32, screen_copy, screen_i8 };

struct Plan {
    CosRoute cos = CosRoute::none;
    int bm25 = BM25_STREAM;
    uint64_t cos_stride = 0, pf_stride = 0, pf_slack = 0;
    uint32_t pf_carry = 4096;
    bool spec = false;
    std::vector<Chunk> screen_chunks;
    bool overlap = false, late_fork = false;
};
bool screened(CosRoute c) { return c == CosRoute::screen_f32 || c == CosRoute::screen_copy || c == CosRoute::screen_i8; }

Plan plan_search(const Search &s) {
    oi_index *idx = s.idx; oi_ctx *ctx = s.ctx;
    const Knobs &K = knobs();
    const uint64_t n = idx->n_docs;
    const uint32_t B = s.B, depth = s.depth, carry_cap = OI_MAX_DEPTH;
    Plan p;
    const int mode = ctx->cosine_mode;
    const bool want_copy = mode != OI_COSINE_SCREEN_STREAM && (idx->screen_copy.p != nullptr || (mode == OI_COSINE_SCREEN_COPY && !idx->is_view));
    const bool screen = (mode == OI_COSINE_SCREEN || mode == OI_COSINE_SCREEN_COPY || mode == OI_COSINE_SCREEN_STREAM) &&
                        oi_index_screenable(idx) && (B > 8 || (want_copy && !K.small_gemv)) && !K.exact_only;
    if (!s.cos_s) p.cos = CosRoute::none;
    else if (idx->rows_bf16) p.cos = CosRoute::bf16;
    else if (!screen) p.cos = CosRoute::exact;
    else if (!want_copy) p.cos = s.filt ? CosRoute::exact : CosRoute::screen_f32;
    else if (B > 8 && idx->screen_copy.p && idx->screen_i8.p) p.cos = CosRoute::screen_i8;
    else p.cos = CosRoute::screen_copy;
    p.bm25 = bm25_mode_of(idx);
    if (p.bm25 == BM25_SCAN && !(idx->fwd_terms.p && idx->total_tokens > 0)) p.bm25 = BM25_STREAM;
    if (s.filt) p.bm25 = BM25_STREAM;
    const uint64_t slack = (idx->rows_bf16 ? 128ull : 32ull) * ((uint64_t)ctx->num_cus + 1);
    const uint64_t budget = (idx->rows_bf16 ? (8ull << 30) : (13ull << 28)) / 8 / B;
    p.cos_stride = std::min<uint64_t>(carry_cap + n + slack, std::max<uint64_t>(std::min<uint64_t>(1ull << 24, budget), carry_cap + 4 * slack));
    p.pf_carry = p.cos == CosRoute::screen_i8 ? OI_I8_CARRY : 4096;
    p.pf_slack = 128ull * ((uint64_t)ctx->num_cus + 1);
    p.pf_stride = std::min<uint64_t>(p.pf_carry + n + p.pf_slack, std::max<uint64_t>(std::min<uint64_t>(1ull << 24, budget), p.pf_carry + 4 * p.pf_slack));
    uint64_t first = oi_screen_first_chunk_rows(ctx, depth), growth = oi_chunk_growth(B);
    const uint64_t pool_max = p.pf_stride - p.pf_carry - p.pf_slack;
    if (screened(p.cos) && B > 8 && !s.filt) {
        oi_spec_take_failure(ctx);
        p.spec = ctx->speculate && !K.no_spec && !ctx->use_graphs;
        if (p.spec && ctx->spec_skip) { --ctx->spec_skip; p.spec = false; }
        if (p.spec && !ctx->spec_fail_host) {
            if (hipHostMalloc(reinterpret_cast<void **>(&ctx->spec_fail_host), 64, hipHostMallocDefault) == hipSuccess) *ctx->spec_fail_host = 0;
            else { (void)hipGetLastError(); ctx->spec_fail_host = nullptr; p.spec = false; }
        }
        if (p.spec && n) {
            const uint64_t first_short = std::min<uint64_t>(n, std::max<uint64_t>(std::max<uint64_t>(8192, 8ull * depth), first / K.spec_first_div));
            if (n - first_short <= pool_max && 2 * ((3ull * depth * first_short + n - 1) / n + 12) <= depth) {
                growth = K.spec_growth;
                first = first_short;
            } else if (2 * ((3ull * depth * std::min<uint64_t>(n, first) + n - 1) / n + 12) <= depth) growth = K.spec_growth;
        }
    }
    if (screened(p.cos)) p.screen_chunks = chunk_schedule(n, first, growth, pool_max, false);
    if (s.cos_s && s.bm_s && !ctx->side_stream && !ctx->side_stream_failed && ctx->overlap_legs && !K.no_overlap) {
        if (hipStreamCreateWithFlags(&ctx->side_stream, hipStreamNonBlocking) != hipSuccess) { ctx->side_stream = nullptr; ctx->side_stream_failed = true; }
    }
    p.overlap = s.cos_s && s.bm_s && ctx->side_stream && ctx->ev_fork && ctx->ev_join && ctx->overlap_legs && !K.no_overlap;
    p.late_fork = p.overlap && !K.bm25_early && B > 8 && !p.screen_chunks.empty() &&
                  p.screen_chunks.back().e - p.screen_chunks.back().r >= (512u << 10);
    return p;
}

int bm25_stream(const Search &s, const PoolView &bm) {
    oi_index *idx = s.idx; oi_ctx *ctx = s.ctx;
    const uint32_t B = s.B, depth = s.depth, carry_cap = OI_MAX_DEPTH, nb = idx->n_blocks;
    if (nb == 0 || idx->n_postings == 0) {
        OI_HIP_CHECK(hipMemsetAsync(s.bm_c, 0, sizeof(uint32_t) * B, ctx->stream));
        return OI_OK;
    }
    const bool floors = idx->impact_floor.p != nullptr && !knobs().bm25_two_phase && !s.filt;
    const uint32_t first = floors ? nb : nb > 48 ? std::max<uint32_t>(8, nb / knobs().bm25_first_div) : nb;
    const uint32_t cap1 = oi_bm25_stream_seg_cap(depth, !floors), cap2 = oi_bm25_stream_seg_cap(depth, false);
    const uint64_t sstride = (uint64_t)carry_cap + std::max<uint64_t>((uint64_t)first * cap1, (uint64_t)nb * cap2);
    uint64_t pass = (2ull << 30) / 8 / sstride;
    pass = std::max<uint64_t>(1, std::min<uint64_t>(pass, std::min<uint32_t>(B, oi_bm25_stream_pass_queries())));
    DevBuf &sp = ctx->buf("pool_bm_stream"), &sc = ctx->buf("pool_bm_stream_state");
    OI_CHECK(sp.ensure(sizeof(uint64_t) * (size_t)pass * sstride));
    const size_t swords = (size_t)pass * (2 + nb);
    OI_CHECK(sc.ensure(sizeof(uint32_t) * swords));
    for (uint32_t q0 = 0; q0 < B; q0 += (uint32_t)pass) {
        const uint32_t nq = std::min<uint32_t>((uint32_t)pass, B - q0);
        uint32_t *w = sc.as<uint32_t>();
        OI_CHECK(oi_launch_bm25_plan(idx, s.qt, s.qo, q0, nq, w, swords, depth, (uint32_t)pass, (uint32_t)pass, floors));
        PoolView W1{sp.as<uint64_t>(), w, w + 2 * (size_t)pass, w + pass, sstride, carry_cap, cap1, first, nb, bm.overflow, s.filt, s.attrs};
        OI_CHECK(oi_launch_bm25_stream(idx, s.qt, s.qo, q0, nq, depth, W1, 0, first));
        PoolView W2 = W1;
        if (first < nb) {
            OI_CHECK(oi_launch_select(ctx, W1, nq, depth, true, nullptr, nullptr, nullptr, depth));
            W2.seg_cap = cap2; W2.n_segs = nb;
            OI_CHECK(oi_launch_bm25_stream(idx, s.qt, s.qo, q0, nq, depth, W2, first, nb));
        }
        OI_CHECK(oi_launch_select(ctx, W2, nq, depth, false, s.bm_s + (size_t)q0 * depth, s.bm_d + (size_t)q0 * depth, s.bm_c + q0, depth));
    }
    return OI_OK;
}
int bm25_wave(const Search &s, const PoolView &bm) {
    oi_index *idx = s.idx; oi_ctx *ctx = s.ctx;
    const uint32_t B = s.B, depth = s.depth, carry_cap = OI_MAX_DEPTH, nb = idx->n_blocks;
    if (nb == 0 || idx->n_postings == 0) {
        OI_HIP_CHECK(hipMemsetAsync(s.bm_c, 0, sizeof(uint32_t) * B, ctx->stream));
        return OI_OK;
    }
    const uint64_t wstride = (uint64_t)carry_cap + (uint64_t)nb * OI_BM25_BLOCK_DOCS;
    uint64_t pass = (6ull << 30) / 8 / wstride;
    pass = std::max<uint64_t>(1, std::min<uint64_t>(pass, std::min<uint32_t>(B, oi_bm25_wave_pass_queries())));
    DevBuf &wp = ctx->buf("pool_bm_wave"), &wc = ctx->buf("pool_bm_wave_state");
    OI_CHECK(wp.ensure(sizeof(uint64_t) * (size_t)pass * wstride));
    const size_t wwords = (size_t)pass * (2 + nb);
    OI_CHECK(wc.ensure(sizeof(uint32_t) * wwords));
    const uint32_t first = nb > 16 ? std::max<uint32_t>(8, nb / 8) : nb;
    for (uint32_t q0 = 0; q0 < B; q0 += (uint32_t)pass) {
        const uint32_t nq = std::min<uint32_t>((uint32_t)pass, B - q0);
        OI_HIP_CHECK(hipMemsetAsync(wc.p, 0, sizeof(uint32_t) * wwords, ctx->stream));
        uint32_t *w = wc.as<uint32_t>();
        PoolView W{wp.as<uint64_t>(), w, w + 2 * (size_t)pass, w + pass, wstride, carry_cap, OI_BM25_BLOCK_DOCS, nb, nb, bm.overflow};
        OI_CHECK(oi_launch_bm25_wave(idx, s.qt, s.qo, q0, nq, W, 0, first));
        if (first < nb) {
            OI_CHECK(oi_launch_select(ctx, W, nq, depth, true, nullptr, nullptr, nullptr, depth));
            OI_CHECK(oi_launch_bm25_wave(idx, s.qt, s.qo, q0, nq, W, first, nb));
        }
        OI_CHECK(oi_launch_select(ctx, W, nq, depth, false, s.bm_s + (size_t)q0 * depth, s.bm_d + (size_t)q0 * depth, s.bm_c + q0, depth));
    }
    return OI_OK;
}
int bm25_taat(const Search &s, const PoolView &bm) {
    const uint32_t nb = s.idx->n_blocks;
    const uint32_t first = nb > 16 ? std::max<uint32_t>(8, nb / 8) : nb;
    OI_CHECK(oi_launch_bm25(s.idx, s.qt, s.qo, s.B, s.depth, bm, 0, first));
    if (first < nb) {
        OI_CHECK(oi_launch_select(s.ctx, bm, s.B, s.depth, true, nullptr, nullptr, nullptr, s.depth));
        OI_CHECK(oi_launch_bm25(s.idx, s.qt, s.qo, s.B, s.depth, bm, first, nb));
    }
    return oi_launch_select(s.ctx, bm, s.B, s.depth, false, s.bm_s, s.bm_d, s.bm_c, s.depth);
}
int bm25_scan(const Search &s, const PoolView &bm) {
    oi_index *idx = s.idx; oi_ctx *ctx = s.ctx;
    const uint64_t n = idx->n_docs;
    const uint32_t B = s.B, depth = s.depth, carry_cap = OI_MAX_DEPTH;
    const uint32_t segs = 2u * (uint32_t)ctx->num_cus;
    const uint64_t sslack = 1024ull * (segs + 1);
    uint64_t sstride = carry_cap + std::min<uint64_t>(n, 1ull << 23) + sslack;
    const uint64_t sbudget = (4ull << 30) / 8 / B;
    if (sstride > sbudget) sstride = std::max<uint64_t>(sbudget, carry_cap + 4 * sslack);
    DevBuf &sp = ctx->buf("pool_bm_scan"), &sc = ctx->buf("pool_bm_scan_state");
    OI_CHECK(sp.ensure(sizeof(uint64_t) * (size_t)B * sstride));
    const size_t swords = (size_t)B * (2 + segs);
    OI_CHECK(sc.ensure(sizeof(uint32_t) * swords));
    OI_HIP_CHECK(hipMemsetAsync(sc.p, 0, sizeof(uint32_t) * swords, ctx->stream));
    uint32_t *w = sc.as<uint32_t>();
    PoolView SP{sp.as<uint64_t>(), w, w + 2 * (size_t)B, w + B, sstride, carry_cap, 0, 0, segs, bm.overflow};
    const uint64_t max_chunk = sstride - carry_cap - sslack;
    const uint32_t pass = oi_bm25_scan_pass_queries(idx->max_query_terms);
    for (uint32_t q0 = 0; q0 < B; q0 += pass) {
        const uint32_t nq = std::min(pass, B - q0);
        PoolView V = SP;
        V.carry_cnt += q0; V.tau_keys += q0;
        uint64_t r = 0, chunk = std::max<uint64_t>(n / 8, 65536);
        while (r < n) {
            if (chunk > max_chunk) chunk = max_chunk;
            const uint64_t e = std::min(n, r + chunk);
            oi_bm25_scan_geometry(ctx, e - r, &V.n_segs, &V.seg_cap);
            SP.n_segs = V.n_segs; SP.seg_cap = V.seg_cap;
            OI_CHECK(oi_launch_bm25_scan(idx, s.qt, s.qo, q0, nq, r, e, idx->avgdl, r == 0, SP));
            const bool last = e == n;
            PoolView S2 = SP;
            S2.keys += (uint64_t)q0 * sstride; S2.carry_cnt += q0; S2.tau_keys += q0; S2.seg_cnt += (uint64_t)q0 * segs;
            OI_CHECK(oi_launch_select(ctx, S2, nq, depth, !last, last ? s.bm_s + (size_t)q0 * depth : nullptr,
                                      last ? s.bm_d + (size_t)q0 * depth : nullptr, last ? s.bm_c + q0 : nullptr, depth));
            r = e;
            chunk = n;
        }
    }
    return OI_OK;
}
int bm25_leg(const Search &s, const Plan &p, const PoolView &bm) {
    OI_REQUIRE(s.idx->finalized, "search: index not finalized");
    return p.bm25 == BM25_TAAT ? bm25_taat(s, bm) : p.bm25 == BM25_SCAN ? bm25_scan(s, bm) : p.bm25 == BM25_WAVE ? bm25_wave(s, bm)
                                                                                                               : bm25_stream(s, bm);
}
int fork_bm25(const Search &s, const Plan &p, const PoolView &bm) {
    oi_ctx *ctx = s.ctx;
    hipStream_t st = ctx->stream;
    OI_HIP_CHECK(hipStreamWaitEvent(ctx->side_stream, ctx->ev_fork, 0));
    ctx->stream = ctx->side_stream;
    const int rc = bm25_leg(s, p, bm);
    ctx->stream = st;
    if (rc != OI_OK) { (void)hipStreamSynchronize(ctx->side_stream); return rc; }
    OI_HIP_CHECK(hipEventRecord(ctx->ev_join, ctx->side_stream));
    return OI_OK;
}

int cosine_bf16(const Search &s, const Plan &p, PoolView C) {
    oi_index *idx = s.idx;
    C.filt = s.filt; C.attrs = s.attrs;
    const uint64_t bslack = 128ull * ((uint64_t)s.ctx->num_cus + 1), room = p.cos_stride - OI_MAX_DEPTH;
    const uint64_t max_chunk = room > bslack ? room - bslack : 0;
    if (max_chunk == 0) { oi_set_error("search: cosine pool too small"); return OI_ERR_STATE; }
    for (const Chunk &c : chunk_schedule(idx->n_docs, oi_first_chunk_rows(s.depth), oi_chunk_growth(s.B), max_chunk, true)) {
        OI_CHECK(oi_launch_cosine_bf16_chunk(s.ctx, idx->rows_bf16, c.r, c.e, idx->dim, s.qv, s.B, idx->doc_id_base, C));
        const bool last = c.e == idx->n_docs;
        OI_CHECK(oi_launch_select(s.ctx, C, s.B, s.depth, !last, last ? s.cos_s : nullptr,
                                  last ? s.cos_d : nullptr, last ? s.cos_c : nullptr, s.depth));
    }
    return OI_OK;
}
int cosine_exact(const Search &s, PoolView X, const float *q, uint32_t Bp, uint64_t max_chunk, const uint32_t *gate, uint32_t *screen_tau) {
    oi_index *idx = s.idx;
    SelectExtra ex; ex.run_gate = gate;
    if (screen_tau) X.tau_keys = screen_tau;
    X.filt = s.filt; X.attrs = s.attrs;
    const uint64_t first = gate ? max_chunk : oi_first_chunk_rows(s.depth);
    for (const Chunk &c : chunk_schedule(idx->n_docs, first, oi_chunk_growth(s.B), max_chunk, true)) {
        OI_CHECK(oi_launch_cosine_chunk(s.ctx, idx->rows, c.r, c.e, idx->dim, q, s.B, Bp, idx->doc_id_base, X));
        const bool last = c.e == idx->n_docs;
        OI_CHECK(oi_launch_select(s.ctx, X, s.B, s.depth, !last, last ? s.cos_s : nullptr,
                                  last ? s.cos_d : nullptr, last ? s.cos_c : nullptr, s.depth, gate ? &ex : nullptr));
    }
    return OI_OK;
}
int cosine_screen(const Search &s, const Plan &p, const Pools &P, uint32_t *w, const float *q, uint32_t Bp, uint64_t max_chunk) {
    oi_index *idx = s.idx; oi_ctx *ctx = s.ctx;
    const uint64_t n = idx->n_docs;
    const uint32_t B = s.B, depth = s.depth, dim = idx->dim;
    const bool i8 = p.cos == CosRoute::screen_i8, copy = p.cos != CosRoute::screen_f32;
    const uint32_t segs = (uint32_t)ctx->num_cus;
    DevBuf &pk = ctx->buf("pool_cos"), &rk = ctx->buf("screen_rescored"), &qb = ctx->buf("screen_q_bf16");
    const uint32_t rs_cap = p.pf_carry + OI_LONG_ROWS_MAX;
    OI_CHECK(rk.ensure(sizeof(uint64_t) * (size_t)B * rs_cap));
    const uint32_t n_padded = (B + 31u) & ~31u;
    OI_CHECK(qb.ensure(sizeof(uint16_t) * (size_t)(n_padded + 64) * dim));
    uint32_t *pf_cnt = w, *pf_tau = w + B, *rs_cnt = w + 2 * (size_t)B;
    float *eps2 = reinterpret_cast<float *>(w + 3 * (size_t)B);
    uint32_t *gate = w + 4 * (size_t)B, *pf_seg = gate + 4;
    uint32_t *spec_tau = pf_seg + (size_t)B * segs, *spec_max = spec_tau + B;
    PoolView PF{pk.as<uint64_t>(), pf_cnt, pf_seg, pf_tau, p.pf_stride, p.pf_carry, 0, 0, segs, P.cos.overflow, s.filt, s.attrs};
    PoolView RS{rk.as<uint64_t>(), rs_cnt, pf_seg, nullptr, rs_cap, rs_cap, 0, 0, segs, P.cos.overflow, s.filt, s.attrs};
    OI_CHECK(oi_launch_screen_stage(ctx, s.qv, B, dim, idx->max_row_norm.as<uint32_t>(), qb.as<uint16_t>(), eps2, gate));
    SelectExtra mx; mx.eps2 = eps2; mx.margin_gate = gate;
    if (idx->n_long) { mx.skip_bitmap = idx->long_bitmap.as<uint32_t>(); mx.skip_base = idx->doc_id_base; }
    if (copy && !idx->screen_copy.p) {
        OI_CHECK(idx->screen_copy.ensure(sizeof(uint16_t) * (size_t)n * dim + 64));
        OI_CHECK(oi_launch_make_screen_copy(ctx, idx->rows, n, dim, idx->screen_copy.as<uint16_t>()));
    }
    int8_t *qi8 = nullptr; float *qf8 = nullptr;
    SelectExtra m8 = mx;
    if (i8) {
        DevBuf &qs = ctx->buf("screen_q_i8"), &cb = ctx->buf("screen_i8_cand");
        const size_t qi8_bytes = ((2 * (size_t)n_padded * dim) + 255) & ~(size_t)255;
        OI_CHECK(qs.ensure(qi8_bytes + sizeof(float) * 4 * (size_t)n_padded));
        OI_CHECK(cb.ensure(sizeof(uint64_t) * (size_t)B * OI_I8_CARRY));
        qi8 = reinterpret_cast<int8_t *>(qs.p);
        qf8 = reinterpret_cast<float *>(reinterpret_cast<unsigned char *>(qs.p) + qi8_bytes);
        OI_CHECK(oi_launch_screen_stage_i8(ctx, s.qv, B, dim, idx->max_row_norm.as<uint32_t>(), idx->screen_i8.as<uint8_t>(), n,
                                           qi8, qf8, gate));
        m8.eps2 = qf8 + 3 * (size_t)n_padded; m8.row_qn = qf8 + (size_t)n_padded; m8.row_cq = qf8 + 2 * (size_t)n_padded;
        m8.cand = cb.as<uint64_t>(); m8.cand_cap = OI_I8_CARRY;
        m8.row_meta = reinterpret_cast<const float *>(idx->screen_i8.as<uint8_t>() + oi_screen_i8_meta_offset(n, dim));
        m8.meta_base = idx->doc_id_base;
    }
    bool spec_next = false, spec_any = false;
    for (size_t i = 0; i < p.screen_chunks.size(); ++i) {
        const uint64_t r = p.screen_chunks[i].r, e = p.screen_chunks[i].e;
        const bool last = i + 1 == p.screen_chunks.size();
        if (p.late_fork && last) OI_HIP_CHECK(hipEventRecord(ctx->ev_fork, ctx->stream));
        uint32_t *const proven_tau = PF.tau_keys;
        if (spec_next) PF.tau_keys = spec_tau;
        const int rc_screen = i8 ? oi_launch_cosine_screen_i8_chunk(ctx, idx->screen_i8.as<uint8_t>(), n, r, e, dim, qi8, qf8, B, idx->doc_id_base, PF)
                              : copy ? oi_launch_cosine_screen_copy_chunk(ctx, idx->screen_copy.as<uint16_t>(), r, e, dim, qb.as<uint16_t>(), B, idx->doc_id_base, PF)
                                     : oi_launch_cosine_screen_chunk(ctx, idx->rows, r, e, dim, qb.as<uint16_t>(), B, idx->doc_id_base, PF);
        PF.tau_keys = proven_tau;
        OI_CHECK(rc_screen);
        if (p.late_fork && last) OI_CHECK(fork_bm25(s, p, P.bm));
        OI_CHECK(oi_launch_select(ctx, PF, B, depth, true, nullptr, nullptr, nullptr, depth, i8 ? &m8 : &mx));
        spec_next = false;
        if (p.spec && !last) {
            const uint64_t rank = (3ull * depth * e + n - 1) / n + 12;
            if (2 * rank <= depth) {
                OI_CHECK(oi_launch_spec_threshold(ctx, PF, B, (uint32_t)rank, i8 ? m8.eps2 : eps2, spec_tau, spec_max));
                spec_next = spec_any = true;
            }
        }
    }
    if (spec_any) ++ctx->spec_searches;
    PoolView PR = PF;
    if (i8) {
        OI_CHECK(oi_launch_rescreen_bf16(ctx, idx->screen_copy.as<uint16_t>(), n, dim, idx->doc_id_base, qb.as<uint16_t>(), B, PF));
        PoolView PB = PF; PB.tau_keys = nullptr; PB.n_segs = 0;
        OI_CHECK(oi_launch_select(ctx, PB, B, depth, true, nullptr, nullptr, nullptr, depth, &mx));
        PR.carry_cap = 4096;
    }
    OI_CHECK(oi_launch_rescore(ctx, idx->rows, n, dim, idx->doc_id_base, s.qv, B, PR, RS,
                               idx->n_long ? idx->long_list.as<uint32_t>() : nullptr, idx->n_long,
                               spec_any ? spec_max : nullptr, pf_tau, gate, ctx->spec_fail_host));
    RS.n_segs = 0;
    OI_CHECK(oi_launch_select(ctx, RS, B, depth, false, s.cos_s, s.cos_d, s.cos_c, depth));
    ctx->run_gate = ctx->last_screen_gate = gate;
    const int rc = cosine_exact(s, P.cos, q, Bp, max_chunk, gate, pf_tau);
    ctx->run_gate = nullptr;
    return rc;
}

int cosine_leg(const Search &s, const Plan &p, const Pools &P, uint32_t *screen_state) {
    if (p.cos == CosRoute::none) return OI_OK;
    if (p.cos == CosRoute::bf16) return cosine_bf16(s, p, P.cos);
    oi_index *idx = s.idx; oi_ctx *ctx = s.ctx;
    OI_REQUIRE(idx->rows, "search: embeddings not set");
    const uint32_t Bp = oi_cosine_query_padding(s.B);
    const float *q = s.qv;
    if (Bp != s.B) {
        DevBuf &qp = ctx->buf("q_padded");
        OI_CHECK(qp.ensure(sizeof(float) * (size_t)Bp * idx->dim));
        OI_HIP_CHECK(hipMemsetAsync(qp.p, 0, sizeof(float) * (size_t)Bp * idx->dim, ctx->stream));
        OI_HIP_CHECK(hipMemcpyAsync(qp.p, s.qv, sizeof(float) * (size_t)s.B * idx->dim, hipMemcpyDeviceToDevice, ctx->stream));
        q = qp.as<float>();
    }
    const uint64_t max_chunk = oi_cosine_max_chunk_rows(ctx, idx->dim, s.B, p.cos_stride, OI_MAX_DEPTH);
    if (max_chunk == 0) { oi_set_error("search: cosine pool too small"); return OI_ERR_STATE; }
    if (p.cos == CosRoute::exact) {
        ctx->last_screen_gate = nullptr;
        return cosine_exact(s, P.cos, q, Bp, max_chunk, nullptr, nullptr);
    }
    return cosine_screen(s, p, P, screen_state, q, Bp, max_chunk);
}

}

void oi_spec_take_failure(oi_ctx *ctx) {
    if (!ctx->spec_fail_host || !*ctx->spec_fail_host) return;
    *ctx->spec_fail_host = 0; ++ctx->spec_failures;
    ctx->spec_backoff = ctx->spec_backoff ? std::min(1024u, 2 * ctx->spec_backoff) : 16u;
    ctx->spec_skip = ctx->spec_backoff;
}
int search_lists_device(oi_index *idx, const float *d_qv, const uint32_t *d_qt, const uint32_t *d_qo, uint32_t B, uint32_t depth,
                        float *cos_s, uint32_t *cos_d, uint32_t *cos_c, float *bm_s, uint32_t *bm_d, uint32_t *bm_c,
                        const uint4 *d_filt, const uint2 *d_attrs) {
    oi_ctx *ctx = idx->ctx;
    const Search s{idx, ctx, d_qv, d_qt, d_qo, B, depth, cos_s, cos_d, cos_c, bm_s, bm_d, bm_c, d_filt, d_attrs};
    const Plan p = plan_search(s);
    Pools P;
    const size_t screen_words = (size_t)B * (6 + (size_t)ctx->num_cus) + 4;
    uint32_t *screen_state = nullptr;
    OI_CHECK(prepare_pools(ctx, B, std::max<uint64_t>(p.cos_stride, idx->rows_bf16 ? 0ull : p.pf_stride), p.cos_stride, OI_MAX_DEPTH,
                           p.bm25 == BM25_TAAT ? idx->n_blocks : 0, depth, &P, screen_words, &screen_state));
    if (p.overlap && !p.late_fork) {
        OI_HIP_CHECK(hipEventRecord(ctx->ev_fork, ctx->stream));
        OI_CHECK(fork_bm25(s, p, P.bm));
    }
    const int rc = cosine_leg(s, p, P, screen_state);
    if (rc != OI_OK) {
        if (p.overlap) (void)hipStreamSynchronize(ctx->side_stream);
        return rc;
    }
    if (p.overlap) OI_HIP_CHECK(hipStreamWaitEvent(ctx->stream, ctx->ev_join, 0));
    else if (bm_s) OI_CHECK(bm25_leg(s, p, P.bm));
    return OI_OK;
}
```

### openintel_amd/csrc/select.hip

```cpp
#include "oi_device.h"
#include "oi_internal.h"

#define SEL_THREADS 1024
#define SEL_MAX 1024

__device__ void bitonic_sort_desc(uint64_t *a, uint32_t P) {
    const uint32_t tid = threadIdx.x;
    for (uint32_t size = 2; size <= P; size <<= 1) {
        for (uint32_t stride = size >> 1; stride > 0; stride >>= 1) {
            for (uint32_t t = tid; t < (P >> 1); t += SEL_THREADS) {
                uint32_t lo = 2 * t - (t & (stride - 1));
                uint32_t hi = lo + stride;
                bool desc = ((lo & size) == 0);
                uint64_t x = a[lo], y = a[hi];
                if ((x < y) == desc) { a[lo] = y; a[hi] = x; }
            }
            __syncthreads();
        }
    }
}

#define SEL_LDS_KEYS 8192

struct SelSource {
    const uint64_t *pool;
    const uint32_t *segc;
    const uint64_t *lds_keys;
    uint32_t n, c0, carry_cap, seg_cap, n_segs;
};

template <class F>
__device__ __forceinline__ void sel_for_each(const SelSource &S, F &&f) {
    const uint32_t tid = threadIdx.x;
    if (S.lds_keys) {
        for (uint32_t i = tid; i < S.n; i += SEL_THREADS) f(S.lds_keys[i]);
        return;
    }
    for (uint32_t i = tid; i < S.c0; i += SEL_THREADS) f(S.pool[i]);
    const uint32_t lane = tid & 63, wv = tid >> 6;
    for (uint32_t sg = wv; sg < S.n_segs; sg += SEL_THREADS / 64) {
        uint32_t c = S.segc[sg];
        if (c > S.seg_cap) c = S.seg_cap;
        const uint64_t *base = S.pool + S.carry_cap + (uint64_t)sg * S.seg_cap;
        for (uint32_t i = lane; i < c; i += 64) f(base[i]);
    }
}

__global__ __launch_bounds__(SEL_THREADS) void select_topk_kernel(
    uint64_t *pools, uint32_t *carry_cnt, uint32_t *seg_cnt, uint32_t *tau_keys, uint64_t pool_stride,
    uint32_t carry_cap, uint32_t seg_cap, uint32_t n_segs, uint32_t seg_cnt_stride, uint32_t *overflow,
    uint32_t k, int compact, float *out_scores, uint32_t *out_docs, uint32_t *out_counts, uint32_t out_stride) {
    __shared__ uint32_t hist[256];
    __shared__ uint64_t sel[2 * SEL_MAX];
    __shared__ uint64_t lds_keys[SEL_LDS_KEYS];
    __shared__ uint32_t s_cnt, s_kk, s_bin_cnt, s_total;
    __shared__ uint64_t s_prefix;

    const uint32_t q = blockIdx.x, tid = threadIdx.x;
    uint64_t *pool = pools + (uint64_t)q * pool_stride;
    uint32_t *segc = seg_cnt + (uint64_t)q * seg_cnt_stride;
    SelSource S;
    S.pool = pool; S.segc = segc; S.lds_keys = nullptr;
    S.carry_cap = carry_cap; S.seg_cap = seg_cap; S.n_segs = n_segs;
    S.c0 = carry_cnt[q] < carry_cap ? carry_cnt[q] : carry_cap;
    if (tid == 0) { s_cnt = 0; s_total = 0; }
    __syncthreads();
    {
        uint32_t local = 0;
        for (uint32_t sg = tid; sg < n_segs; sg += SEL_THREADS) {
            uint32_t c = segc[sg];
            if (c > seg_cap) { *overflow = 1u; c = seg_cap; }
            local += c;
        }
        local = oi_wave_sum(local);
        if ((tid & 63) == 0 && local) atomicAdd(&s_total, local);
    }
    __syncthreads();
    const uint32_t n = S.c0 + s_total;
    S.n = n;
    if (n <= SEL_LDS_KEYS) {
        sel_for_each(S, [&](uint64_t key) { lds_keys[atomicAdd(&s_cnt, 1u)] = key; });
        __syncthreads();
        S.lds_keys = lds_keys;
        if (tid == 0) s_cnt = 0;
        __syncthreads();
    }

    uint32_t m;
    if (n <= k) {
        sel_for_each(S, [&](uint64_t key) { sel[atomicAdd(&s_cnt, 1u)] = key; });
        m = n;
        __syncthreads();
    } else {
        if (tid == 0) { s_prefix = 0; s_kk = k; }
        int shift = 56;
        for (;; shift -= 8) {
            if (tid < 256) hist[tid] = 0;
            __syncthreads();
            const uint64_t prefix = s_prefix;
            if (shift == 56)
                sel_for_each(S, [&](uint64_t key) { atomicAdd(&hist[(uint32_t)(key >> 56)], 1u); });
            else
                sel_for_each(S, [&](uint64_t key) {
                    if ((key >> (shift + 8)) == prefix) atomicAdd(&hist[(uint32_t)(key >> shift) & 255u], 1u);
                });
            __syncthreads();
            if (tid < 64) {
                const uint32_t kk = s_kk;
                uint32_t mine = 0;
                for (int i = 0; i < 4; ++i) mine += hist[255 - (tid * 4 + i)];
                uint32_t incl = mine;
#pragma unroll
                for (int o = 1; o < 64; o <<= 1) {
                    uint32_t v = __shfl_up(incl, o, OI_WAVE);
                    if ((int)tid >= o) incl += v;
                }
                const unsigned long long ball = __ballot(incl >= kk);
                const uint32_t owner = ball ? (uint32_t)__builtin_ctzll(ball) : 63u;
                if (tid == owner) {
                    uint32_t cum = incl - mine;
                    int d = 255 - (int)(tid * 4);
                    for (int i = 0; i < 3; ++i, --d) {
                        const uint32_t c = hist[d];
                        if (cum + c >= kk) break;
                        cum += c;
                    }
                    s_prefix = (prefix << 8) | (uint64_t)d;
                    s_kk = kk - cum;
                    s_bin_cnt = hist[d];
                }
            }
            __syncthreads();
            if (s_bin_cnt == 1 || shift == 0) break;
        }
        const uint64_t prefix = s_prefix;
        sel_for_each(S, [&](uint64_t key) {
            if ((key >> shift) >= prefix) {
                const uint32_t pos = atomicAdd(&s_cnt, 1u);
                if (pos < SEL_MAX) sel[pos] = key;
            }
        });
        __syncthreads();
        m = s_cnt < k ? s_cnt : k;
    }
    __shared__ unsigned long long s_min;
    if (out_scores) {
        uint32_t P = 2;
        while (P < m) P <<= 1;
        for (uint32_t i = m + tid; i < P; i += SEL_THREADS) sel[i] = 0;
        __syncthreads();
        bitonic_sort_desc(sel, P);
        for (uint32_t i = tid; i < m; i += SEL_THREADS) {
            const uint64_t key = sel[i];
            out_scores[(uint64_t)q * out_stride + i] = oi_rank_key_score(key);
            out_docs[(uint64_t)q * out_stride + i] = oi_rank_key_doc(key);
        }
        if (tid == 0) { out_counts[q] = m; s_min = m ? sel[m - 1] : 0; }
    } else {
        if (tid == 0) s_min = ~0ull;
        __syncthreads();
        unsigned long long lo = ~0ull;
        for (uint32_t i = tid; i < m; i += SEL_THREADS) lo = sel[i] < lo ? sel[i] : lo;
#pragma unroll
        for (int o = 32; o > 0; o >>= 1) {
            const unsigned long long v = __shfl_xor(lo, o, OI_WAVE);
            lo = v < lo ? v : lo;
        }
        if ((tid & 63) == 0 && lo != ~0ull) atomicMin(&s_min, lo);
    }
    __syncthreads();
    if (compact) {
        for (uint32_t i = tid; i < m; i += SEL_THREADS) pool[i] = sel[i];
        for (uint32_t sg = tid; sg < n_segs; sg += SEL_THREADS) segc[sg] = 0;
        if (tid == 0) {
            carry_cnt[q] = m;
            if (m == k && tau_keys) {
                const uint32_t t = (uint32_t)(s_min >> 32);
                if (t > tau_keys[q]) tau_keys[q] = t;
            }
        }
    }
}

#define SEL_MAX_SEGS 4096
#define SEL_KPT_MAX 32
#ifdef OI_ABLATION
__device__ int sel_dbg_on;
__device__ unsigned long long sel_dbg_t[16];
#define SEL_STAMP(i) do { if (sel_dbg_on && blockIdx.x == 0 && threadIdx.x == 0) sel_dbg_t[i] = __builtin_readcyclecounter(); } while (0)
#else
#define SEL_STAMP(i) do { } while (0)
#endif
#define SEL_CAND 4096

struct SelRowMargin {
    const float *meta;
    uint32_t base;
    float qn, cq;
};
__device__ __forceinline__ bool sel_row_keep(const SelRowMargin *rm, uint64_t kv, float edge, float eps2) {
    if (!rm) return true;
    const float e = rm->meta[2 * (uint64_t)(oi_rank_key_doc(kv) - rm->base) + 1];
    const float u = oi_rank_key_score(kv) + 2.002f * (e * rm->qn + rm->cq);
    return u >= edge - 9.5367431640625e-07f * (fabsf(edge) + eps2);
}

struct SelShared {
    uint32_t hist[256];
    uint32_t hist2k[2048];
    uint32_t seg_off[SEL_MAX_SEGS + 1];
    uint32_t wave_tot[SEL_THREADS / 64];
    uint32_t cnt, kk, bin_cnt, n_samples;
    uint64_t prefix;
    unsigned long long min_key;
};

struct SelFlat {
    const uint64_t *pool;
    const uint32_t *seg_off;
    uint32_t n, c0, carry_cap, seg_cap, n_segs, steps;
};
struct SelCursor {
    uint32_t sg, lo, hi;
};
__device__ __forceinline__ SelCursor sel_seek(const SelFlat &K, uint32_t i) {
    const uint32_t e = i < K.c0 ? 0u : i - K.c0;
    uint32_t lo = 0, hi = K.n_segs;
    for (uint32_t s = 0; s < K.steps; ++s) {
        const uint32_t mid = (lo + hi) >> 1;
        const bool up = K.seg_off[mid] <= e;
        lo = up ? mid : lo;
        hi = up ? hi : mid;
    }
    SelCursor c;
    c.sg = lo; c.lo = K.seg_off[lo]; c.hi = K.seg_off[lo + 1];
    return c;
}
__device__ __forceinline__ uint64_t sel_at(const SelFlat &K, SelCursor &c, uint32_t i) {
    if (i < K.c0) return i;
    const uint32_t e = i - K.c0;
    while (e >= c.hi) {
        ++c.sg;
        c.lo = c.hi;
        c.hi = K.seg_off[c.sg + 1];
    }
    return (uint64_t)K.carry_cap + (uint64_t)c.sg * K.seg_cap + (e - c.lo);
}

__device__ __forceinline__ void sel_hist_add(uint32_t *hist, bool active, uint32_t digit) {
    const uint32_t lane = threadIdx.x & 63;
#pragma unroll
    for (int r = 0; r < 2; ++r) {
        const unsigned long long m = __ballot(active);
        if (!m) return;
        const uint32_t leader = (uint32_t)__builtin_ctzll(m);
        const uint32_t d0 = (uint32_t)__shfl((int)digit, (int)leader, OI_WAVE);
        const unsigned long long same = __ballot(active && digit == d0);
        if (lane == leader) atomicAdd(&hist[d0], (uint32_t)__popcll(same));
        active = active && digit != d0;
    }
    if (active) atomicAdd(&hist[digit], 1u);
}

__device__ __forceinline__ void sel_append(uint64_t *dst, uint32_t *count, uint32_t cap, bool take, uint64_t key) {
    const unsigned long long m = __ballot(take);
    if (!m) return;
    const uint32_t lane = threadIdx.x & 63, leader = (uint32_t)__builtin_ctzll(m);
    uint32_t base = 0;
    if (lane == leader) base = atomicAdd(count, (uint32_t)__popcll(m));
    base = (uint32_t)__shfl((int)base, (int)leader, OI_WAVE);
    const uint32_t pos = base + (uint32_t)__popcll(m & ((1ull << lane) - 1ull));
    if (take && pos < cap) dst[pos] = key;
}

__device__ __forceinline__ void sel_hist_add_w(uint32_t *hist, bool active, uint32_t digit, uint32_t weight) {
    const uint32_t lane = threadIdx.x & 63;
#pragma unroll
    for (int r = 0; r < 2; ++r) {
        const unsigned long long m = __ballot(active);
        if (!m) return;
        const uint32_t leader = (uint32_t)__builtin_ctzll(m);
        const uint32_t d0 = (uint32_t)__builtin_amdgcn_readlane((int)digit, (int)leader);
        const bool same = active && digit == d0;
        const uint32_t sum = (uint32_t)__builtin_amdgcn_readlane((int)oi_wave_incl_scan(same ? weight : 0u), 63);
        if (lane == leader) atomicAdd(&hist[d0], sum);
        active = active && !same;
    }
    if (active) atomicAdd(&hist[digit], weight);
}

template <class FE>
__device__ __forceinline__ void sel_threshold(FE &&for_each, uint32_t kk_in, SelShared &sh, int &shift_out, uint64_t &prefix_out) {
    const uint32_t tid = threadIdx.x;
    if (tid == 0) { sh.prefix = 0; sh.kk = kk_in; }
    int shift = 56;
    for (;; shift -= 8) {
        if (tid < 256) sh.hist[tid] = 0;
        __syncthreads();
        const uint64_t prefix = sh.prefix;
        const bool top = shift == 56;
        for_each([&](bool valid, uint64_t kv) {
            sel_hist_add(sh.hist, valid && (top || (kv >> ((shift + 8) & 63)) == prefix), (uint32_t)(kv >> shift) & 255u);
        });
        __syncthreads();
        if (tid < 64) {
            const uint32_t kk = sh.kk;
            uint32_t mine = 0;
            for (int i = 0; i < 4; ++i) mine += sh.hist[255 - (tid * 4 + i)];
            uint32_t incl = mine;
#pragma unroll
            for (int o = 1; o < 64; o <<= 1) {
                const uint32_t v = __shfl_up(incl, o, OI_WAVE);
                if ((int)tid >= o) incl += v;
            }
            const unsigned long long ball = __ballot(incl >= kk);
            const uint32_t owner = ball ? (uint32_t)__builtin_ctzll(ball) : 63u;
            if (tid == owner) {
                uint32_t cum = incl - mine;
                int d = 255 - (int)(tid * 4);
                for (int i = 0; i < 3; ++i, --d) {
                    const uint32_t c = sh.hist[d];
                    if (cum + c >= kk) break;
                    cum += c;
                }
                sh.prefix = (prefix << 8) | (uint64_t)d;
                sh.kk = kk - cum;
                sh.bin_cnt = sh.hist[d];
            }
        }
        __syncthreads();
        if (sh.bin_cnt == 1 || shift == 0) break;
    }
    shift_out = shift;
    prefix_out = sh.prefix;
    __syncthreads();
}

template <int KPT>
__device__ __forceinline__ uint32_t sel_flat_select(const SelFlat &K, uint32_t k, SelShared &sh, uint64_t *sel,
                                                    uint64_t *cand, float eps2, bool *in_cand, uint32_t *margin_tau,
                                                    bool *margin_overflow, const uint32_t *skip, uint32_t skip_base,
                                                    uint64_t *mc, uint32_t mcap, const SelRowMargin *rm) {
    auto skipped = [&](uint64_t kv) -> bool {
        const uint32_t d = oi_rank_key_doc(kv) - skip_base;
        return (skip[d >> 5] >> (d & 31u)) & 1u;
    };
    const uint32_t tid = threadIdx.x, lane = tid & 63, wv = tid >> 6, n = K.n;
    *in_cand = false;
    *margin_overflow = false;
    if (n == 0) return 0;
    const uint32_t kpt = (n + SEL_THREADS - 1) / SEL_THREADS;
    const uint32_t first = wv * kpt * 64 + lane, last = n - 1;
    constexpr int NR = KPT > 0 ? KPT : 1;
    uint64_t key[NR];
    uint32_t dead = 0;
    if constexpr (KPT > 0) {
        SelCursor cur = sel_seek(K, first < n ? first : last);
        uint64_t at = sel_at(K, cur, first < n ? first : last);
#pragma unroll
        for (int j = 0; j < KPT; ++j) {
            const uint32_t i = first + (uint32_t)j * 64;
            if ((uint32_t)j < kpt && i < n) at = sel_at(K, cur, i);
            key[j] = K.pool[at];
        }
        if (skip) {
#pragma unroll
            for (int j = 0; j < KPT; ++j)
                if ((uint32_t)j < kpt && first + (uint32_t)j * 64 < n && skipped(key[j])) dead |= 1u << j;
        }
    }
    auto for_each = [&](auto &&f) {
        if constexpr (KPT > 0) {
#pragma unroll
            for (int j = 0; j < KPT; ++j)
                if ((uint32_t)j < kpt) f(first + (uint32_t)j * 64 < n && !((dead >> j) & 1u), key[j]);
        } else {
            SelCursor cur = sel_seek(K, first < n ? first : last);
            uint64_t at = sel_at(K, cur, first < n ? first : last);
            for (uint32_t j0 = 0; j0 < kpt; j0 += 4) {
                uint64_t kx[4];
                bool ok[4];
#pragma unroll
                for (int u = 0; u < 4; ++u) {
                    const uint32_t i = first + (j0 + u) * 64;
                    ok[u] = j0 + u < kpt && i < n;
                    if (ok[u]) at = sel_at(K, cur, i);
                    kx[u] = K.pool[at];
                }
#pragma unroll
                for (int u = 0; u < 4; ++u) f(ok[u] && !(skip && skipped(kx[u])), kx[u]);
            }
        }
    };
    if (n <= k) {
        for_each([&](bool valid, uint64_t kv) { sel_append(sel, &sh.cnt, 2 * SEL_MAX, valid, kv); });
        __syncthreads();
        return skip ? sh.cnt : n;
    }
    SEL_STAMP(2);
    if (eps2 >= 0.f) {
        uint32_t kk = k;
        uint32_t pfx = 0;
        bool enough = true;
#pragma unroll
        for (int pass = 0; pass < 2; ++pass) {
            const int shift = 53 - 11 * pass;
            sh.hist2k[tid] = 0;
            sh.hist2k[tid + SEL_THREADS] = 0;
            __syncthreads();
            if (pass == 0) {
                uint32_t run_d = 0, run_c = 0;
                for_each([&](bool valid, uint64_t kv) {
                    if (valid) {
                        const uint32_t d = (uint32_t)(kv >> 53);
                        if (run_c && d != run_d) { atomicAdd(&sh.hist2k[run_d], run_c); run_c = 0; }
                        run_d = d;
                        ++run_c;
                    }
                });
                sel_hist_add_w(sh.hist2k, run_c != 0u, run_d, run_c);
            } else {
                for_each([&](bool valid, uint64_t kv) {
                    if (valid && (uint32_t)(kv >> 53) == pfx) atomicAdd(&sh.hist2k[(uint32_t)(kv >> shift) & 2047u], 1u);
                });
            }
            __syncthreads();
            {
                uint32_t v = sh.hist2k[2 * tid] + sh.hist2k[2 * tid + 1];
                v += (uint32_t)__builtin_amdgcn_update_dpp(0, (int)v, 0x111, 0xf, 0xf, false);
                v += (uint32_t)__builtin_amdgcn_update_dpp(0, (int)v, 0x112, 0xf, 0xf, false);
                v += (uint32_t)__builtin_amdgcn_update_dpp(0, (int)v, 0x114, 0xf, 0xf, false);
                v += (uint32_t)__builtin_amdgcn_update_dpp(0, (int)v, 0x118, 0xf, 0xf, false);
                if ((tid & 15u) == 15u) sh.hist[tid >> 4] = v;
            }
            __syncthreads();
            if (tid < 64) {
                const uint32_t x = sh.hist[63u - tid];
                const uint32_t incl = oi_wave_incl_scan(x);
                const unsigned long long ball = __ballot(incl >= kk);
                if (!ball) {
                    if (tid == 0) sh.bin_cnt = 0xFFFFFFFFu;
                } else {
                    const uint32_t l1 = (uint32_t)__builtin_ctzll(ball), sb = 63u - l1;
                    const uint32_t kk2 = kk - (uint32_t)__builtin_amdgcn_readlane((int)(incl - x), (int)l1);
                    const uint32_t y = tid < 32u ? sh.hist2k[32u * sb + 31u - tid] : 0u;
                    const uint32_t incl2 = oi_wave_incl_scan(y);
                    const unsigned long long ball2 = __ballot(incl2 >= kk2);
                    const uint32_t l2 = ball2 ? (uint32_t)__builtin_ctzll(ball2) : 31u;
                    const uint32_t above = (uint32_t)__builtin_amdgcn_readlane((int)(incl2 - y), (int)l2);
                    if (tid == 0) {
                        sh.prefix = (uint64_t)(32u * sb + 31u - l2);
                        sh.kk = kk2 - above;
                        sh.bin_cnt = 1u;
#ifdef OI_ABLATION
                        if (sel_dbg_on > 1) {
                            uint32_t cum = 0; int dd = 2047;
                            for (; dd >= 0; --dd) { if (cum + sh.hist2k[dd] >= kk) break; cum += sh.hist2k[dd]; }
                            if ((uint32_t)dd != (uint32_t)sh.prefix || kk - cum != sh.kk)
                                printf("MISMATCH q=%u pass=%d kk=%u: walk (%d, %u) super-bin (%u, %u) sb=%u l1=%u kk2=%u l2=%u\n", blockIdx.x, pass, kk, dd, kk - cum,
                                       (uint32_t)sh.prefix, sh.kk, sb, l1, kk2, l2);
                        }
#endif
                    }
                }
            }
            __syncthreads();
            enough = sh.bin_cnt != 0xFFFFFFFFu;
            const uint32_t d = (uint32_t)sh.prefix;
            kk = sh.kk;
            __syncthreads();
            if (!enough) break;
            if (pass == 0) pfx = d;
            else pfx = (pfx << 11) | d;
            SEL_STAMP(3 + pass);
        }
        if (enough) {
            uint32_t tkey = pfx << 10;
            tkey = tkey < 0x007FFFFFu ? 0x007FFFFFu : tkey;
            const uint32_t t32 = eps2 < __builtin_inff() ? oi_f32_key(oi_key_f32(tkey) - eps2) : 0u;
            uint32_t mine = 0;
            const float edge = oi_key_f32(tkey);
            auto keep = [&](bool valid, uint64_t kv) { return valid && (uint32_t)(kv >> 32) >= t32 && sel_row_keep(rm, kv, edge, eps2); };
            for_each([&](bool valid, uint64_t kv) { mine += keep(valid, kv) ? 1u : 0u; });
            const uint32_t incl = oi_wave_incl_scan(mine);
            const uint32_t tot = (uint32_t)__builtin_amdgcn_readlane((int)incl, 63);
            uint32_t base = 0;
            if (lane == 0 && tot) base = atomicAdd(&sh.cnt, tot);
            uint32_t pos = (uint32_t)__builtin_amdgcn_readfirstlane((int)base) + incl - mine;
            for_each([&](bool valid, uint64_t kv) {
                if (keep(valid, kv)) {
                    if (pos < mcap) mc[pos] = kv;
                    ++pos;
                }
            });
            __syncthreads();
            const uint32_t c = sh.cnt;
            *in_cand = true;
            *margin_tau = t32;
            *margin_overflow = c > mcap;
            SEL_STAMP(5);
            return c > mcap ? mcap : c;
        }
    }
    int shift;
    uint64_t prefix;
    bool selected = false;
    if (KPT != 4 && n > SEL_CAND) {
        const uint32_t js = lane % kpt, is = first + js * 64;
        bool sv = is < n;
        uint64_t sk;
        if constexpr (KPT > 0) {
            sk = key[0];
#pragma unroll
            for (int j = 1; j < KPT; ++j) sk = (uint32_t)j == js ? key[j] : sk;
            sv = sv && !((dead >> js) & 1u);
        } else {
            SelCursor cur = sel_seek(K, sv ? is : last);
            sk = K.pool[sel_at(K, cur, sv ? is : last)];
            sv = sv && !(skip && skipped(sk));
        }
        if (tid == 0) sh.n_samples = 0;
        __syncthreads();
        {
            const unsigned long long m = __ballot(sv);
            if (lane == 0 && m) atomicAdd(&sh.n_samples, (uint32_t)__popcll(m));
        }
        __syncthreads();
        const uint32_t ns = sh.n_samples;
        uint32_t r = (uint32_t)(((uint64_t)ns * (2 * k) + n - 1) / n) + 1;
        r = r > ns ? ns : r;
        sel_threshold([&](auto &&f) { f(sv, sk); }, r, sh, shift, prefix);
        for_each([&](bool valid, uint64_t kv) { sel_append(cand, &sh.cnt, SEL_CAND, valid && (kv >> shift) >= prefix, kv); });
        __syncthreads();
        const uint32_t c = sh.cnt;
        __syncthreads();
        if (tid == 0) sh.cnt = 0;
        __syncthreads();
        if (c >= k && c <= SEL_CAND) {
            uint64_t ck[SEL_CAND / SEL_THREADS];
#pragma unroll
            for (int j = 0; j < SEL_CAND / SEL_THREADS; ++j) {
                const uint32_t i = (uint32_t)j * SEL_THREADS + tid;
                ck[j] = cand[i < c ? i : c - 1];
            }
            auto cand_each = [&](auto &&f) {
#pragma unroll
                for (int j = 0; j < SEL_CAND / SEL_THREADS; ++j)
                    if ((uint32_t)j * SEL_THREADS < c) f((uint32_t)j * SEL_THREADS + tid < c, ck[j]);
            };
            if (c == k) {
                cand_each([&](bool valid, uint64_t kv) { sel_append(sel, &sh.cnt, SEL_MAX, valid, kv); });
            } else {
                sel_threshold(cand_each, k, sh, shift, prefix);
                cand_each([&](bool valid, uint64_t kv) { sel_append(sel, &sh.cnt, SEL_MAX, valid && (kv >> shift) >= prefix, kv); });
            }
            __syncthreads();
            selected = true;
        }
    }
    if (!selected) {
        sel_threshold(for_each, k, sh, shift, prefix);
        for_each([&](bool valid, uint64_t kv) { sel_append(sel, &sh.cnt, SEL_MAX, valid && (kv >> shift) >= prefix, kv); });
        __syncthreads();
    }
    const uint32_t m = sh.cnt < k ? sh.cnt : k;
    if (!(eps2 >= 0.f) || m < k) return m;
    __syncthreads();
    unsigned long long lo = ~0ull;
    for (uint32_t i = tid; i < m; i += SEL_THREADS) lo = sel[i] < lo ? sel[i] : lo;
#pragma unroll
    for (int o = 32; o > 0; o >>= 1) {
        const unsigned long long v = __shfl_xor(lo, o, OI_WAVE);
        lo = v < lo ? v : lo;
    }
    if (lane == 0 && lo != ~0ull) atomicMin(&sh.min_key, lo);
    if (tid == 0) sh.cnt = 0;
    __syncthreads();
    const uint32_t t32 = eps2 < __builtin_inff() ? oi_f32_key(oi_key_f32((uint32_t)(sh.min_key >> 32)) - eps2) : 0u;
    const float edge = oi_key_f32((uint32_t)(sh.min_key >> 32));
    for_each([&](bool valid, uint64_t kv) {
        sel_append(mc, &sh.cnt, mcap, valid && (uint32_t)(kv >> 32) >= t32 && sel_row_keep(rm, kv, edge, eps2), kv);
    });
    __syncthreads();
    const uint32_t c = sh.cnt;
    *in_cand = true;
    *margin_tau = t32;
    *margin_overflow = c > mcap;
    return c > mcap ? mcap : c;
}

__global__ __launch_bounds__(SEL_THREADS) void select_flat_kernel(
    uint64_t *pools, uint32_t *carry_cnt, uint32_t *seg_cnt, uint32_t *tau_keys, uint64_t pool_stride,
    uint32_t carry_cap, uint32_t seg_cap, uint32_t n_segs, uint32_t seg_cnt_stride, uint32_t *overflow,
    uint32_t k, int compact, float *out_scores, uint32_t *out_docs, uint32_t *out_counts, uint32_t out_stride,
    const float *eps2, uint32_t *margin_gate, const uint32_t *run_gate, const uint32_t *skip, uint32_t skip_base,
    uint64_t *cand_g, uint32_t cand_cap, const float *row_meta, uint32_t meta_base, const float *row_qn, const float *row_cq) {
    if (run_gate && *run_gate == 0u) return;
    __shared__ SelShared sh;
    __shared__ uint64_t sel[2 * SEL_MAX];
    __shared__ uint64_t cand[SEL_CAND];
    const uint32_t q = blockIdx.x, tid = threadIdx.x, lane = tid & 63, wv = tid >> 6;
    uint64_t *pool = pools + (uint64_t)q * pool_stride;
    uint32_t *segc = seg_cnt + (uint64_t)q * seg_cnt_stride;
    SEL_STAMP(0);
    const uint32_t c0_raw = carry_cnt[q];
    const float e2 = eps2 ? eps2[q] : -1.f;
    uint64_t *const mc = cand_g ? cand_g + (uint64_t)q * cand_cap : cand;
    const uint32_t mcap = cand_g ? cand_cap : SEL_CAND;
    SelRowMargin rm_v;
    if (row_meta) rm_v = SelRowMargin{row_meta, meta_base, row_qn[q], row_cq[q]};
    const SelRowMargin *rm = row_meta && e2 < __builtin_inff() ? &rm_v : nullptr;

    constexpr int SPT = SEL_MAX_SEGS / SEL_THREADS;
    uint32_t c[SPT], local = 0;
#pragma unroll
    for (int u = 0; u < SPT; ++u) {
        const uint32_t sg = tid * SPT + u;
        uint32_t v = segc[sg < n_segs ? sg : 0];
        if (sg >= n_segs) v = 0;
        if (v > seg_cap) { *overflow = 1u; v = seg_cap; }
        c[u] = v;
        local += v;
    }
    const uint32_t incl = oi_wave_incl_scan(local);
    if (lane == 63) sh.wave_tot[wv] = incl;
    if (tid == 0) { sh.cnt = 0; sh.min_key = ~0ull; }
    __syncthreads();
    uint32_t base = 0, total = 0;
#pragma unroll
    for (int w = 0; w < SEL_THREADS / 64; ++w) {
        const uint32_t t = sh.wave_tot[w];
        base += (uint32_t)w < wv ? t : 0u;
        total += t;
    }
    uint32_t run = base + incl - local;
#pragma unroll
    for (int u = 0; u < SPT; ++u) {
        const uint32_t sg = tid * SPT + u;
        if (sg < n_segs) sh.seg_off[sg] = run;
        run += c[u];
    }
    if (tid == 0) sh.seg_off[n_segs] = total;
    __syncthreads();

    SelFlat K;
    K.pool = pool; K.seg_off = sh.seg_off; K.carry_cap = carry_cap; K.seg_cap = seg_cap; K.n_segs = n_segs;
    K.c0 = c0_raw < carry_cap ? c0_raw : carry_cap;
    K.n = K.c0 + total;
    K.steps = 0;
    while ((1u << K.steps) < n_segs) ++K.steps;
    SEL_STAMP(1);

    uint32_t m, m_tau = 0;
    bool in_cand = false, m_over = false;
    if (K.n <= 4 * SEL_THREADS) m = sel_flat_select<4>(K, k, sh, sel, cand, e2, &in_cand, &m_tau, &m_over, skip, skip_base, mc, mcap, rm);
    else if (K.n <= 8 * SEL_THREADS) m = sel_flat_select<8>(K, k, sh, sel, cand, e2, &in_cand, &m_tau, &m_over, skip, skip_base, mc, mcap, rm);
    else if (K.n <= 16 * SEL_THREADS) m = sel_flat_select<16>(K, k, sh, sel, cand, e2, &in_cand, &m_tau, &m_over, skip, skip_base, mc, mcap, rm);
    else if (K.n <= SEL_KPT_MAX * SEL_THREADS) m = sel_flat_select<SEL_KPT_MAX>(K, k, sh, sel, cand, e2, &in_cand, &m_tau, &m_over, skip, skip_base, mc, mcap, rm);
    else m = sel_flat_select<0>(K, k, sh, sel, cand, e2, &in_cand, &m_tau, &m_over, skip, skip_base, mc, mcap, rm);
    if (in_cand) {
        if (m_over && tid == 0 && margin_gate) *margin_gate = 1u;
        for (uint32_t i = tid; i < m; i += SEL_THREADS) pool[i] = mc[i];
        for (uint32_t sg = tid; sg < n_segs; sg += SEL_THREADS) segc[sg] = 0;
        if (tid == 0) {
            carry_cnt[q] = m;
            if (tau_keys && m_tau > tau_keys[q]) tau_keys[q] = m_tau;
        }
#ifdef OI_ABLATION
        __syncthreads();
        if (sel_dbg_on && blockIdx.x == 0 && tid == 0) {
            const unsigned long long e = __builtin_readcyclecounter();
            printf("select margin n=%u m=%u segs=%u: scan %llu, loads+skip %llu, pass0 %llu, pass1 %llu, filter %llu, compact %llu (cycles)\n", K.n, m, n_segs,
                   sel_dbg_t[1] - sel_dbg_t[0], sel_dbg_t[2] - sel_dbg_t[1], sel_dbg_t[3] - sel_dbg_t[2], sel_dbg_t[4] - sel_dbg_t[3], sel_dbg_t[5] - sel_dbg_t[4], e - sel_dbg_t[5]);
        }
#endif
        return;
    }

    if (out_scores) {
        uint32_t P = 2;
        while (P < m) P <<= 1;
        for (uint32_t i = m + tid; i < P; i += SEL_THREADS) sel[i] = 0;
        __syncthreads();
        bitonic_sort_desc(sel, P);
        for (uint32_t i = tid; i < m; i += SEL_THREADS) {
            const uint64_t key = sel[i];
            out_scores[(uint64_t)q * out_stride + i] = oi_rank_key_score(key);
            out_docs[(uint64_t)q * out_stride + i] = oi_rank_key_doc(key);
        }
        if (tid == 0) { out_counts[q] = m; sh.min_key = m ? sel[m - 1] : 0; }
    } else {
        unsigned long long lo = ~0ull;
        for (uint32_t i = tid; i < m; i += SEL_THREADS) lo = sel[i] < lo ? sel[i] : lo;
#pragma unroll
        for (int o = 32; o > 0; o >>= 1) {
            const unsigned long long v = __shfl_xor(lo, o, OI_WAVE);
            lo = v < lo ? v : lo;
        }
        if (lane == 0 && lo != ~0ull) atomicMin(&sh.min_key, lo);
    }
    __syncthreads();
    if (compact) {
        for (uint32_t i = tid; i < m; i += SEL_THREADS) pool[i] = sel[i];
        for (uint32_t sg = tid; sg < n_segs; sg += SEL_THREADS) segc[sg] = 0;
        if (tid == 0) {
            carry_cnt[q] = m;
            if (m == k && tau_keys && !eps2) {
                const uint32_t t = (uint32_t)(sh.min_key >> 32);
                if (t > tau_keys[q]) tau_keys[q] = t;
            }
        }
    }
}

int oi_launch_select(oi_ctx *ctx, const PoolView &pool, uint32_t n_queries, uint32_t k, bool compact,
                     float *out_scores, uint32_t *out_docs, uint32_t *out_counts, uint32_t out_stride,
                     const SelectExtra *extra) {
    if (n_queries == 0) return OI_OK;
    OI_REQUIRE(k >= 1 && k <= OI_MAX_DEPTH && k <= pool.carry_cap, "select: k=%u outside [1,%u]", k, OI_MAX_DEPTH);
    ProfScope ps(ctx, "select");
    static const bool v1 = oi_ablation_env("OI_SELECT_V1") != nullptr;
#ifdef OI_ABLATION
    static const bool stamps = [] {
        const int on = oi_ablation_env("OI_SELECT_STAMPS") ? std::max(1, atoi(oi_ablation_env("OI_SELECT_STAMPS"))) : 0;
        (void)hipMemcpyToSymbol(HIP_SYMBOL(sel_dbg_on), &on, sizeof(int));
        return on != 0;
    }();
    (void)stamps;
#endif
    const bool special = extra && (extra->eps2 || extra->run_gate);
    if (special) {
        OI_REQUIRE(pool.n_segs <= SEL_MAX_SEGS, "select: %u segments (margin / gated selects take <= %u)", pool.n_segs, SEL_MAX_SEGS);
        const uint32_t mcap = extra->cand ? extra->cand_cap : SEL_CAND;
        OI_REQUIRE(!extra->eps2 || (compact && !out_scores && pool.carry_cap >= mcap),
                   "select: margin mode compacts into a carry region of >= %u keys", mcap);
    }
    if ((!v1 || special) && pool.n_segs <= SEL_MAX_SEGS) {
        hipLaunchKernelGGL(select_flat_kernel, dim3(n_queries), dim3(SEL_THREADS), 0, ctx->stream, pool.keys,
                           pool.carry_cnt, pool.seg_cnt, pool.tau_keys, pool.stride, pool.carry_cap, pool.seg_cap,
                           pool.n_segs, pool.seg_cnt_stride, pool.overflow, k, compact ? 1 : 0, out_scores, out_docs,
                           out_counts, out_stride, extra ? extra->eps2 : nullptr, extra ? extra->margin_gate : nullptr,
                           extra ? extra->run_gate : nullptr, extra && extra->eps2 ? extra->skip_bitmap : nullptr,
                           extra ? extra->skip_base : 0u, extra && extra->eps2 ? extra->cand : nullptr,
                           extra && extra->eps2 ? extra->cand_cap : 0u, extra && extra->eps2 ? extra->row_meta : nullptr,
                           extra ? extra->meta_base : 0u, extra ? extra->row_qn : nullptr, extra ? extra->row_cq : nullptr);
        OI_HIP_CHECK(hipGetLastError());
        return OI_OK;
    }
    hipLaunchKernelGGL(select_topk_kernel, dim3(n_queries), dim3(SEL_THREADS), 0, ctx->stream, pool.keys,
                       pool.carry_cnt, pool.seg_cnt, pool.tau_keys, pool.stride, pool.carry_cap, pool.seg_cap,
                       pool.n_segs, pool.seg_cnt_stride, pool.overflow, k, compact ? 1 : 0, out_scores, out_docs,
                       out_counts, out_stride);
    OI_HIP_CHECK(hipGetLastError());
    return OI_OK;
}

__global__ void lists_to_pool_kernel(const float *scores, const uint32_t *docs, const uint32_t *counts,
                                     uint64_t shard_stride, uint64_t count_stride, uint32_t n_queries,
                                     uint32_t depth, uint64_t *pools, uint32_t *carry_cnt,
                                     uint32_t *seg_cnt, uint64_t pool_stride, uint32_t carry_cap,
                                     uint32_t seg_cnt_stride) {
    const uint32_t q = blockIdx.x, sh = blockIdx.y;
    uint32_t c = counts[(uint64_t)sh * count_stride + q];
    if (c > depth) c = depth;
    const uint64_t src = (uint64_t)sh * shard_stride + (uint64_t)q * depth;
    uint64_t *seg = pools + (uint64_t)q * pool_stride + carry_cap + (uint64_t)sh * depth;
    for (uint32_t i = threadIdx.x; i < c; i += blockDim.x) seg[i] = oi_rank_key(scores[src + i], docs[src + i]);
    if (threadIdx.x == 0) {
        seg_cnt[(uint64_t)q * seg_cnt_stride + sh] = c;
        if (sh == 0) carry_cnt[q] = 0;
    }
}

int oi_launch_lists_to_pool(oi_ctx *ctx, const float *scores, const uint32_t *docs,
                            const uint32_t *counts, uint64_t shard_stride, uint64_t count_stride,
                            uint32_t n_shards, uint32_t n_queries, uint32_t depth, const PoolView &pool) {
    if (n_queries == 0) return OI_OK;
    OI_REQUIRE(pool.seg_cap == depth && pool.n_segs == n_shards, "merge: pool geometry mismatch");
    hipLaunchKernelGGL(lists_to_pool_kernel, dim3(n_queries, n_shards), dim3(256), 0, ctx->stream, scores, docs,
                       counts, shard_stride, count_stride, n_queries, depth, pool.keys, pool.carry_cnt, pool.seg_cnt, pool.stride,
                       pool.carry_cap, pool.seg_cnt_stride);
    OI_HIP_CHECK(hipGetLastError());
    return OI_OK;
}

#define RRF_HASH 4096
__global__ __launch_bounds__(SEL_THREADS) void rrf_kernel(const uint32_t *docs_a, const uint32_t *counts_a,
                                                          const uint32_t *docs_b, const uint32_t *counts_b,
                                                          uint32_t depth, uint32_t k, float *scores_out,
                                                          uint32_t *docs_out, uint32_t *counts_out) {
    __shared__ uint32_t h_doc[RRF_HASH];
    __shared__ uint32_t h_idx[RRF_HASH];
    __shared__ uint32_t a_match[SEL_MAX];
    __shared__ uint64_t u[2 * SEL_MAX];
    __shared__ uint32_t s_extra;

    const uint32_t q = blockIdx.x, tid = threadIdx.x;
    uint32_t na = counts_a[q], nb = counts_b[q];
    if (na > depth) na = depth;
    if (nb > depth) nb = depth;
    const uint32_t *da = docs_a + (uint64_t)q * depth, *db = docs_b + (uint64_t)q * depth;

    for (uint32_t i = tid; i < RRF_HASH; i += SEL_THREADS) h_idx[i] = 0;
    for (uint32_t i = tid; i < SEL_MAX; i += SEL_THREADS) a_match[i] = 0;
    if (tid == 0) s_extra = 0;
    __syncthreads();
    for (uint32_t i = tid; i < na; i += SEL_THREADS) {
        uint32_t d = da[i];
        uint32_t h = (d * 2654435761u) >> 20;
        for (;;) {
            uint32_t prev = atomicCAS(&h_idx[h], 0u, i + 1);
            if (prev == 0) { h_doc[h] = d; break; }
            h = (h + 1) & (RRF_HASH - 1);
        }
    }
    __syncthreads();
    for (uint32_t j = tid; j < nb; j += SEL_THREADS) {
        uint32_t d = db[j];
        uint32_t h = (d * 2654435761u) >> 20;
        uint32_t hit = 0;
        for (;;) {
            uint32_t ix = h_idx[h];
            if (ix == 0) break;
            if (h_doc[h] == d) { hit = ix; break; }
            h = (h + 1) & (RRF_HASH - 1);
        }
        if (hit) a_match[hit - 1] = j + 1;
        else {
            uint32_t pos = atomicAdd(&s_extra, 1u);
            float c = 1.0f / (60.0f + (float)(j + 1));
            u[na + pos] = oi_rank_key(c, d);
        }
    }
    __syncthreads();
    for (uint32_t i = tid; i < na; i += SEL_THREADS) {
        float s = 1.0f / (60.0f + (float)(i + 1));
        uint32_t j1 = a_match[i];
        if (j1) s = s + 1.0f / (60.0f + (float)j1);
        u[i] = oi_rank_key(s, da[i]);
    }
    __syncthreads();
    const uint32_t m = na + s_extra;
    uint32_t P = 2;
    while (P < m) P <<= 1;
    for (uint32_t i = m + tid; i < P; i += SEL_THREADS) u[i] = 0;
    __syncthreads();
    bitonic_sort_desc(u, P);
    const uint32_t out = m < k ? m : k;
    for (uint32_t i = tid; i < out; i += SEL_THREADS) {
        scores_out[(uint64_t)q * k + i] = oi_rank_key_score(u[i]);
        docs_out[(uint64_t)q * k + i] = oi_rank_key_doc(u[i]);
    }
    if (tid == 0) counts_out[q] = out;
}

int oi_launch_rrf(oi_ctx *ctx, const uint32_t *docs_a, const uint32_t *counts_a, const uint32_t *docs_b,
                  const uint32_t *counts_b, uint32_t n_queries, uint32_t depth, uint32_t k,
                  float *scores_out, uint32_t *docs_out, uint32_t *counts_out) {
    if (n_queries == 0) return OI_OK;
    OI_REQUIRE(depth >= 1 && depth <= OI_MAX_DEPTH, "rrf: depth=%u outside [1,%u]", depth, OI_MAX_DEPTH);
    OI_REQUIRE(k >= 1 && k <= OI_MAX_DEPTH, "rrf: k=%u outside [1,%u]", k, OI_MAX_DEPTH);
    ProfScope ps(ctx, "rrf");
    hipLaunchKernelGGL(rrf_kernel, dim3(n_queries), dim3(SEL_THREADS), 0, ctx->stream, docs_a, counts_a,
                       docs_b, counts_b, depth, k, scores_out, docs_out, counts_out);
    OI_HIP_CHECK(hipGetLastError());
    return OI_OK;
}
```

Before: 32850.

## Fuse bf16 and int8 query staging; compute speculative threshold inside select

Moves the bf16 query staging into a shared header so one kernel can stage both the int8 and bf16 query forms in a single pass, replacing two launches. The select kernel can now compute the speculative rank threshold (spec_tau/spec_max) directly from its candidates and write survivors straight into the carry region, so the separate pf_spec_kernel pass and a copy are no longer needed. It also adds an ablation-only comparison kernel to check the fused threshold against the old one. The cost is more register pressure and complexity in select, plus the risk of a mismatch with the old threshold.

```diff
diff --git a/openintel_amd/csrc/cosine_prefilter.hip b/openintel_amd/csrc/cosine_prefilter.hip
--- a/openintel_amd/csrc/cosine_prefilter.hip
+++ b/openintel_amd/csrc/cosine_prefilter.hip
@@ -4,6 +4,7 @@
 
 #include "oi_device.h"
 #include "oi_internal.h"
+#include "oi_screen_stage.h"
 #include "oi_lds_dma.h"
 
 typedef float pf_f32x16 __attribute__((ext_vector_type(16)));
@@ -275,51 +276,14 @@
     }
 }
 
-#define PF_NORM_LIMIT 1.0e15f
-#define PF_QNORM_MIN 1.0e-12f
-__device__ __forceinline__ float pf_eps(float X, float E, float qn, float qtn, float en, uint32_t dim) {
-    const float tiny = 4.0e-18f, d = (float)dim;
-    const float Xs = X + tiny, Es = E + tiny, qts = qtn + tiny, ens = en + tiny;
-    const float acc = d * 2.384185791015625e-07f;
-    return 1.001f * (Es * qts + Xs * ens + acc * (Xs + Es) * qts) + d * 7.5231638452626401e-37f * (Xs + qn) + 1.0e-30f;
-}
-
 __global__ __launch_bounds__(256) void pf_stage_queries_kernel(const float *__restrict__ q, uint32_t n_queries,
                                                                uint32_t n_padded, uint32_t dim,
                                                                const uint32_t *__restrict__ max_norm_bits,
                                                                uint16_t *__restrict__ out, float *__restrict__ eps2,
                                                                uint32_t *gate) {
-    const uint32_t lane = threadIdx.x & 63;
     const uint32_t wave = (blockIdx.x * blockDim.x + threadIdx.x) >> 6, n_waves = (gridDim.x * blockDim.x) >> 6;
     for (uint32_t row = wave; row < n_padded; row += n_waves) {
-        float ss = 0.f, st = 0.f, se = 0.f;
-        for (uint32_t k = lane; k < dim; k += 64) {
-            uint16_t v = 0;
-            if (row < n_queries) {
-                const float f = q[(uint64_t)row * dim + k];
-                const uint32_t u = __float_as_uint(f);
-                v = (u & 0x7F800000u) == 0x7F800000u ? (uint16_t)(u >> 16)
-                                                     : (uint16_t)((u + 0x7FFFu + ((u >> 16) & 1u)) >> 16);
-                const float ft = __uint_as_float((uint32_t)v << 16), e = ft - f;
-                ss = fmaf(f, f, ss);
-                st = fmaf(ft, ft, st);
-                se = fmaf(e, e, se);
-            }
-            out[(uint64_t)row * dim + k] = v;
-        }
-        if (row < n_queries) {
-            ss = oi_wave_sum(ss);
-            st = oi_wave_sum(st);
-            se = oi_wave_sum(se);
-            const float qn = sqrtf(ss), qtn = sqrtf(st), en = sqrtf(se);
-            const float X = __uint_as_float(max_norm_bits[0]), E = __uint_as_float(max_norm_bits[1]);
-            const bool ok = qn < PF_NORM_LIMIT && qn >= PF_QNORM_MIN && qtn < PF_NORM_LIMIT && X < PF_NORM_LIMIT &&
-                            E < PF_NORM_LIMIT && en == en;
-            if (lane == 0) {
-                eps2[row] = ok ? 2.0f * pf_eps(X, E, qn, qtn, en, dim) : __builtin_inff();
-                if (!ok) *gate = 1u;
-            }
-        }
+        pf_stage_query_row(q, row, n_queries, dim, max_norm_bits, out, eps2, gate);
     }
 }
 
@@ -497,6 +461,23 @@
     hipLaunchKernelGGL(pf_spec_kernel, dim3(n_queries), dim3(256), 0, ctx->stream, pool.keys, pool.carry_cnt, pool.stride, pool.carry_cap, r,
                        eps2, pool.tau_keys, spec_tau, spec_max);
     OI_HIP_CHECK(hipGetLastError());
+    return OI_OK;
+}
+
+#ifdef OI_ABLATION
+__global__ void pf_spec_compare_kernel(uint32_t n, const uint32_t *tau_a, const uint32_t *max_a, const uint32_t *tau_b, const uint32_t *max_b) {
+    const uint32_t q = blockIdx.x * blockDim.x + threadIdx.x;
+    if (q < n && (tau_a[q] != tau_b[q] || max_a[q] != max_b[q]))
+        printf("SPEC MISMATCH q=%u: select (%08x, %08x) pf_spec_kernel (%08x, %08x)\n", q, tau_a[q], max_a[q], tau_b[q], max_b[q]);
+}
+#endif
+int oi_launch_spec_compare(oi_ctx *ctx, uint32_t n_queries, const uint32_t *tau_a, const uint32_t *max_a, const uint32_t *tau_b,
+                           const uint32_t *max_b) {
+#ifdef OI_ABLATION
+    if (n_queries == 0) return OI_OK;
+    hipLaunchKernelGGL(pf_spec_compare_kernel, dim3((n_queries + 255) / 256), dim3(256), 0, ctx->stream, n_queries, tau_a, max_a, tau_b, max_b);
+    OI_HIP_CHECK(hipGetLastError());
+#endif
     return OI_OK;
 }
 
diff --git a/openintel_amd/csrc/cosine_screen_i8.hip b/openintel_amd/csrc/cosine_screen_i8.hip
--- a/openintel_amd/csrc/cosine_screen_i8.hip
+++ b/openintel_amd/csrc/cosine_screen_i8.hip
@@ -5,6 +5,7 @@
 
 #include "oi_device.h"
 #include "oi_internal.h"
+#include "oi_screen_stage.h"
 #include "oi_lds_dma.h"
 
 typedef int i8s_i32x4 __attribute__((ext_vector_type(4)));
@@ -92,65 +93,86 @@
 
 #define I8S_NORM_LIMIT 1.0e15f
 #define I8S_QNORM_MIN 1.0e-12f
+__device__ __forceinline__ void i8s_stage_query_row(const float *__restrict__ q, uint32_t row, uint32_t n_queries, uint32_t n_padded, uint32_t dim,
+                                                    const uint32_t *__restrict__ max_norm_bits, const uint32_t *__restrict__ emax_bits,
+                                                    int8_t *__restrict__ qi8, float *__restrict__ qf, uint32_t *gate) {
+    const uint32_t lane = threadIdx.x & 63;
+    const bool real = row < n_queries;
+    float amax = 0.f;
+    bool fin = true;
+    for (uint32_t k = lane; k < dim; k += 64) {
+        const float f = real ? q[(uint64_t)row * dim + k] : 0.f;
+        fin = fin && (f - f == 0.f);
+        amax = fmaxf(amax, fabsf(f));
+    }
+#pragma unroll
+    for (int o = 32; o > 0; o >>= 1) amax = fmaxf(amax, __shfl_xor(amax, o, OI_WAVE));
+    fin = __builtin_amdgcn_ballot_w64(!fin) == 0ull;
+    const float a = fin ? amax / 127.f : 0.f;
+    double qn2 = 0.0, en2 = 0.0;
+    for (uint32_t k = lane; k < dim; k += 64) {
+        const float f = real ? q[(uint64_t)row * dim + k] : 0.f;
+        float h = 0.f, l = 0.f;
+        if (a > 0.f) {
+            const float t = f / a;
+            h = fminf(127.f, fmaxf(-127.f, rintf(t)));
+            l = fminf(127.f, fmaxf(-127.f, rintf((t - h) * 128.f)));
+        }
+        const double qh = (double)a * ((double)h + (double)l * 0.0078125);
+        qn2 += qh * qh;
+        en2 += (qh - (double)f) * (qh - (double)f);
+        qi8[(uint64_t)row * dim + k] = (int8_t)(int)h;
+        qi8[((uint64_t)n_padded + row) * dim + k] = (int8_t)(int)l;
+    }
+    qn2 = oi_wave_sum(qn2);
+    en2 = oi_wave_sum(en2);
+    if (lane == 0) {
+        const float up = 1.00000095367431640625f;
+        const float qn = (float)sqrt(qn2) * up, en = (float)sqrt(en2) * up;
+        const float X = __uint_as_float(max_norm_bits[0]), em = __uint_as_float(*emax_bits);
+        const bool ok = fin && amax > 0.f && qn < I8S_NORM_LIMIT && qn >= I8S_QNORM_MIN && X < I8S_NORM_LIMIT && em < I8S_NORM_LIMIT;
+        const float rnd = 3.814697265625e-06f + (float)dim * 2.384185791015625e-07f;
+        const float cq = 1.001f * (X * en + rnd * (X + em) * (qn + en)) + 1.0e-27f;
+        const float m2 = 2.002f * (em * qn + cq);
+        qf[row] = ok ? a : 0.f;
+        qf[n_padded + row] = ok ? qn : 0.f;
+        qf[2 * n_padded + row] = ok ? cq : 0.f;
+        qf[3 * n_padded + row] = ok || !real ? m2 : __builtin_inff();
+        if (real && !ok) *gate = 1u;
+    }
+}
 __global__ __launch_bounds__(256) void i8s_stage_kernel(const float *__restrict__ q, uint32_t n_queries, uint32_t n_padded, uint32_t dim,
                                                         const uint32_t *__restrict__ max_norm_bits, const uint32_t *__restrict__ emax_bits,
                                                         int8_t *__restrict__ qi8, float *__restrict__ qf, uint32_t *gate) {
-    const uint32_t lane = threadIdx.x & 63;
     const uint32_t wave = (blockIdx.x * blockDim.x + threadIdx.x) >> 6, n_waves = (gridDim.x * blockDim.x) >> 6;
     for (uint32_t row = wave; row < n_padded; row += n_waves) {
-        const bool real = row < n_queries;
-        float amax = 0.f;
-        bool fin = true;
-        for (uint32_t k = lane; k < dim; k += 64) {
-            const float f = real ? q[(uint64_t)row * dim + k] : 0.f;
-            fin = fin && (f - f == 0.f);
-            amax = fmaxf(amax, fabsf(f));
-        }
-#pragma unroll
-        for (int o = 32; o > 0; o >>= 1) amax = fmaxf(amax, __shfl_xor(amax, o, OI_WAVE));
-        fin = __builtin_amdgcn_ballot_w64(!fin) == 0ull;
-        const float a = fin ? amax / 127.f : 0.f;
-        double qn2 = 0.0, en2 = 0.0;
-        for (uint32_t k = lane; k < dim; k += 64) {
-            const float f = real ? q[(uint64_t)row * dim + k] : 0.f;
-            float h = 0.f, l = 0.f;
-            if (a > 0.f) {
-                const float t = f / a;
-                h = fminf(127.f, fmaxf(-127.f, rintf(t)));
-                l = fminf(127.f, fmaxf(-127.f, rintf((t - h) * 128.f)));
-            }
-            const double qh = (double)a * ((double)h + (double)l * 0.0078125);
-            qn2 += qh * qh;
-            en2 += (qh - (double)f) * (qh - (double)f);
-            qi8[(uint64_t)row * dim + k] = (int8_t)(int)h;
-            qi8[((uint64_t)n_padded + row) * dim + k] = (int8_t)(int)l;
-        }
-        qn2 = oi_wave_sum(qn2);
-        en2 = oi_wave_sum(en2);
-        if (lane == 0) {
-            const float up = 1.00000095367431640625f;
-            const float qn = (float)sqrt(qn2) * up, en = (float)sqrt(en2) * up;
-            const float X = __uint_as_float(max_norm_bits[0]), em = __uint_as_float(*emax_bits);
-            const bool ok = fin && amax > 0.f && qn < I8S_NORM_LIMIT && qn >= I8S_QNORM_MIN && X < I8S_NORM_LIMIT && em < I8S_NORM_LIMIT;
-            const float rnd = 3.814697265625e-06f + (float)dim * 2.384185791015625e-07f;
-            const float cq = 1.001f * (X * en + rnd * (X + em) * (qn + en)) + 1.0e-27f;
-            const float m2 = 2.002f * (em * qn + cq);
-            qf[row] = ok ? a : 0.f;
-            qf[n_padded + row] = ok ? qn : 0.f;
-            qf[2 * n_padded + row] = ok ? cq : 0.f;
-            qf[3 * n_padded + row] = ok || !real ? m2 : __builtin_inff();
-            if (real && !ok) *gate = 1u;
-        }
+        i8s_stage_query_row(q, row, n_queries, n_padded, dim, max_norm_bits, emax_bits, qi8, qf, gate);
+    }
+}
+
+__global__ __launch_bounds__(256) void i8s_stage_both_kernel(const float *__restrict__ q, uint32_t n_queries, uint32_t n_padded, uint32_t dim,
+                                                             const uint32_t *__restrict__ max_norm_bits, const uint32_t *__restrict__ emax_bits,
+                                                             int8_t *__restrict__ qi8, float *__restrict__ qf, uint16_t *__restrict__ q_bf16,
+                                                             float *__restrict__ eps2, uint32_t *gate) {
+    const uint32_t wave = (blockIdx.x * blockDim.x + threadIdx.x) >> 6, n_waves = (gridDim.x * blockDim.x) >> 6;
+    for (uint32_t row = wave; row < n_padded; row += n_waves) {
+        i8s_stage_query_row(q, row, n_queries, n_padded, dim, max_norm_bits, emax_bits, qi8, qf, gate);
+        pf_stage_query_row(q, row, n_queries, dim, max_norm_bits, q_bf16, eps2, gate);
     }
 }
 
 int oi_launch_screen_stage_i8(oi_ctx *ctx, const float *d_queries, uint32_t n_queries, uint32_t dim, const uint32_t *max_norm_bits,
-                              const uint8_t *i8_copy, uint64_t n_rows, int8_t *qi8, float *qf, uint32_t *gate) {
+                              const uint8_t *i8_copy, uint64_t n_rows, int8_t *qi8, float *qf, uint32_t *gate, uint16_t *q_bf16,
+                              float *eps2) {
     const uint32_t n_padded = (n_queries + 31u) & ~31u;
     if (n_padded == 0) return OI_OK;
     const uint32_t *emax = reinterpret_cast<const uint32_t *>(i8_copy + oi_screen_i8_meta_offset(n_rows, dim)) + 2 * (n_rows + I8S_PAD_ROWS);
-    hipLaunchKernelGGL(i8s_stage_kernel, dim3((n_padded + 3) / 4), dim3(256), 0, ctx->stream, d_queries, n_queries, n_padded, dim,
-                       max_norm_bits, emax, qi8, qf, gate);
+    if (q_bf16)
+        hipLaunchKernelGGL(i8s_stage_both_kernel, dim3((n_padded + 3) / 4), dim3(256), 0, ctx->stream, d_queries, n_queries, n_padded, dim,
+                           max_norm_bits, emax, qi8, qf, q_bf16, eps2, gate);
+    else
+        hipLaunchKernelGGL(i8s_stage_kernel, dim3((n_padded + 3) / 4), dim3(256), 0, ctx->stream, d_queries, n_queries, n_padded, dim,
+                           max_norm_bits, emax, qi8, qf, gate);
     OI_HIP_CHECK(hipGetLastError());
     return OI_OK;
 }
diff --git a/openintel_amd/csrc/oi_internal.h b/openintel_amd/csrc/oi_internal.h
--- a/openintel_amd/csrc/oi_internal.h
+++ b/openintel_amd/csrc/oi_internal.h
@@ -241,6 +241,8 @@
     const float *row_meta = nullptr;
     uint32_t meta_base = 0;
     const float *row_qn = nullptr, *row_cq = nullptr;
+    uint32_t spec_rank = 0;
+    uint32_t *spec_tau = nullptr, *spec_max = nullptr;
 };
 int oi_launch_select(oi_ctx *ctx, const PoolView &pool, uint32_t n_queries, uint32_t k, bool compact,
                      float *out_scores, uint32_t *out_docs, uint32_t *out_counts, uint32_t out_stride,
@@ -292,7 +294,8 @@
 size_t oi_screen_i8_meta_offset(uint64_t n, uint32_t dim);
 int oi_launch_make_screen_i8(oi_ctx *ctx, const float *rows, uint64_t n, uint32_t dim, const uint32_t *long_bitmap, uint8_t *out);
 int oi_launch_screen_stage_i8(oi_ctx *ctx, const float *d_queries, uint32_t n_queries, uint32_t dim, const uint32_t *max_norm_bits,
-                              const uint8_t *i8_copy, uint64_t n_rows, int8_t *qi8, float *qf, uint32_t *gate);
+                              const uint8_t *i8_copy, uint64_t n_rows, int8_t *qi8, float *qf, uint32_t *gate,
+                              uint16_t *q_bf16 = nullptr, float *eps2 = nullptr);
 int oi_launch_cosine_screen_i8_chunk(oi_ctx *ctx, const uint8_t *i8_copy, uint64_t n_rows_total, uint64_t row_begin, uint64_t row_end,
                                      uint32_t dim, const int8_t *qi8, const float *qf, uint32_t n_queries, uint32_t doc_id_base,
                                      PoolView &pool);
@@ -304,6 +307,8 @@
                            const uint16_t *q_bf16, uint32_t n_queries, float *d_out);
 int oi_launch_spec_threshold(oi_ctx *ctx, const PoolView &pool, uint32_t n_queries, uint32_t r, const float *eps2, uint32_t *spec_tau,
                              uint32_t *spec_max);
+int oi_launch_spec_compare(oi_ctx *ctx, uint32_t n_queries, const uint32_t *tau_a, const uint32_t *max_a, const uint32_t *tau_b,
+                           const uint32_t *max_b);
 int oi_launch_rescore(oi_ctx *ctx, const float *rows, uint64_t n_rows, uint32_t dim, uint32_t doc_id_base,
                       const float *d_queries, uint32_t n_queries, const PoolView &in, const PoolView &out,
                       const uint32_t *extra_docs = nullptr, uint32_t n_extra = 0, const uint32_t *spec_max = nullptr,
diff --git a/openintel_amd/csrc/oi_screen_stage.h b/openintel_amd/csrc/oi_screen_stage.h
--- /dev/null
+++ b/openintel_amd/csrc/oi_screen_stage.h
@@ -0,0 +1,45 @@
+#pragma once
+#include "oi_device.h"
+
+#define PF_NORM_LIMIT 1.0e15f
+#define PF_QNORM_MIN 1.0e-12f
+__device__ __forceinline__ float pf_eps(float X, float E, float qn, float qtn, float en, uint32_t dim) {
+    const float tiny = 4.0e-18f, d = (float)dim;
+    const float Xs = X + tiny, Es = E + tiny, qts = qtn + tiny, ens = en + tiny;
+    const float acc = d * 2.384185791015625e-07f;
+    return 1.001f * (Es * qts + Xs * ens + acc * (Xs + Es) * qts) + d * 7.5231638452626401e-37f * (Xs + qn) + 1.0e-30f;
+}
+
+__device__ __forceinline__ void pf_stage_query_row(const float *__restrict__ q, uint32_t row, uint32_t n_queries, uint32_t dim,
+                                                   const uint32_t *__restrict__ max_norm_bits, uint16_t *__restrict__ out,
+                                                   float *__restrict__ eps2, uint32_t *gate) {
+    const uint32_t lane = threadIdx.x & 63;
+    float ss = 0.f, st = 0.f, se = 0.f;
+    for (uint32_t k = lane; k < dim; k += 64) {
+        uint16_t v = 0;
+        if (row < n_queries) {
+            const float f = q[(uint64_t)row * dim + k];
+            const uint32_t u = __float_as_uint(f);
+            v = (u & 0x7F800000u) == 0x7F800000u ? (uint16_t)(u >> 16)
+                                                 : (uint16_t)((u + 0x7FFFu + ((u >> 16) & 1u)) >> 16);
+            const float ft = __uint_as_float((uint32_t)v << 16), e = ft - f;
+            ss = fmaf(f, f, ss);
+            st = fmaf(ft, ft, st);
+            se = fmaf(e, e, se);
+        }
+        out[(uint64_t)row * dim + k] = v;
+    }
+    if (row < n_queries) {
+        ss = oi_wave_sum(ss);
+        st = oi_wave_sum(st);
+        se = oi_wave_sum(se);
+        const float qn = sqrtf(ss), qtn = sqrtf(st), en = sqrtf(se);
+        const float X = __uint_as_float(max_norm_bits[0]), E = __uint_as_float(max_norm_bits[1]);
+        const bool ok = qn < PF_NORM_LIMIT && qn >= PF_QNORM_MIN && qtn < PF_NORM_LIMIT && X < PF_NORM_LIMIT &&
+                        E < PF_NORM_LIMIT && en == en;
+        if (lane == 0) {
+            eps2[row] = ok ? 2.0f * pf_eps(X, E, qn, qtn, en, dim) : __builtin_inff();
+            if (!ok) *gate = 1u;
+        }
+    }
+}
diff --git a/openintel_amd/csrc/search.hip b/openintel_amd/csrc/search.hip
--- a/openintel_amd/csrc/search.hip
+++ b/openintel_amd/csrc/search.hip
@@ -331,7 +331,8 @@
     uint32_t *spec_tau = pf_seg + (size_t)B * segs, *spec_max = spec_tau + B;
     PoolView PF{pk.as<uint64_t>(), pf_cnt, pf_seg, pf_tau, p.pf_stride, p.pf_carry, 0, 0, segs, P.cos.overflow, s.filt, s.attrs};
     PoolView RS{rk.as<uint64_t>(), rs_cnt, pf_seg, nullptr, rs_cap, rs_cap, 0, 0, segs, P.cos.overflow, s.filt, s.attrs};
-    OI_CHECK(oi_launch_screen_stage(ctx, s.qv, B, dim, idx->max_row_norm.as<uint32_t>(), qb.as<uint16_t>(), eps2, gate));
+    static const bool stage_split = oi_ablation_env("OI_STAGE_SPLIT") != nullptr;
+    if (!i8 || stage_split) OI_CHECK(oi_launch_screen_stage(ctx, s.qv, B, dim, idx->max_row_norm.as<uint32_t>(), qb.as<uint16_t>(), eps2, gate));
     SelectExtra mx; mx.eps2 = eps2; mx.margin_gate = gate;
     if (idx->n_long) { mx.skip_bitmap = idx->long_bitmap.as<uint32_t>(); mx.skip_base = idx->doc_id_base; }
     if (copy && !idx->screen_copy.p) {
@@ -348,7 +349,7 @@
         qi8 = reinterpret_cast<int8_t *>(qs.p);
         qf8 = reinterpret_cast<float *>(reinterpret_cast<unsigned char *>(qs.p) + qi8_bytes);
         OI_CHECK(oi_launch_screen_stage_i8(ctx, s.qv, B, dim, idx->max_row_norm.as<uint32_t>(), idx->screen_i8.as<uint8_t>(), n,
-                                           qi8, qf8, gate));
+                                           qi8, qf8, gate, stage_split ? nullptr : qb.as<uint16_t>(), stage_split ? nullptr : eps2));
         m8.eps2 = qf8 + 3 * (size_t)n_padded; m8.row_qn = qf8 + (size_t)n_padded; m8.row_cq = qf8 + 2 * (size_t)n_padded;
         m8.cand = cb.as<uint64_t>(); m8.cand_cap = OI_I8_CARRY;
         m8.row_meta = reinterpret_cast<const float *>(idx->screen_i8.as<uint8_t>() + oi_screen_i8_meta_offset(n, dim));
@@ -367,14 +368,28 @@
         PF.tau_keys = proven_tau;
         OI_CHECK(rc_screen);
         if (p.late_fork && last) OI_CHECK(fork_bm25(s, p, P.bm));
-        OI_CHECK(oi_launch_select(ctx, PF, B, depth, true, nullptr, nullptr, nullptr, depth, i8 ? &m8 : &mx));
+        static const int spec_kernel = oi_ablation_env("OI_SPEC_KERNEL") ? atoi(oi_ablation_env("OI_SPEC_KERNEL")) : 0;
+        const uint64_t rank = (3ull * depth * e + n - 1) / n + 12;
+        const bool spec_here = p.spec && !last && 2 * rank <= depth;
+        SelectExtra sx = i8 ? m8 : mx;
+        if (spec_here && spec_kernel != 1) { sx.spec_rank = (uint32_t)rank; sx.spec_tau = spec_tau; sx.spec_max = spec_max; }
+        uint32_t *chk = nullptr;
+        if (spec_here && spec_kernel == 2) {
+            DevBuf &cw = ctx->buf("spec_check");
+            OI_CHECK(cw.ensure(sizeof(uint32_t) * 2 * (size_t)B));
+            chk = cw.as<uint32_t>();
+            OI_HIP_CHECK(hipMemcpyAsync(chk + B, spec_max, sizeof(uint32_t) * B, hipMemcpyDeviceToDevice, ctx->stream));
+        }
+        OI_CHECK(oi_launch_select(ctx, PF, B, depth, true, nullptr, nullptr, nullptr, depth, &sx));
         spec_next = false;
-        if (p.spec && !last) {
-            const uint64_t rank = (3ull * depth * e + n - 1) / n + 12;
-            if (2 * rank <= depth) {
-                OI_CHECK(oi_launch_spec_threshold(ctx, PF, B, (uint32_t)rank, i8 ? m8.eps2 : eps2, spec_tau, spec_max));
-                spec_next = spec_any = true;
+        if (spec_here) {
+            if (spec_kernel != 1) { ProfScope ps(ctx, "spec"); }
+            if (spec_kernel == 1) OI_CHECK(oi_launch_spec_threshold(ctx, PF, B, (uint32_t)rank, sx.eps2, spec_tau, spec_max));
+            if (chk) {
+                OI_CHECK(oi_launch_spec_threshold(ctx, PF, B, (uint32_t)rank, sx.eps2, chk, chk + B));
+                OI_CHECK(oi_launch_spec_compare(ctx, B, spec_tau, spec_max, chk, chk + B));
             }
+            spec_next = spec_any = true;
         }
     }
     if (spec_any) ++ctx->spec_searches;
diff --git a/openintel_amd/csrc/select.hip b/openintel_amd/csrc/select.hip
--- a/openintel_amd/csrc/select.hip
+++ b/openintel_amd/csrc/select.hip
@@ -198,11 +198,25 @@
     uint32_t base;
     float qn, cq;
 };
+__device__ __forceinline__ float sel_row_e(const SelRowMargin *rm, uint64_t kv) {
+    return rm->meta[2 * (uint64_t)(oi_rank_key_doc(kv) - rm->base) + 1];
+}
+__device__ __forceinline__ bool sel_row_test(const SelRowMargin *rm, uint64_t kv, float e, float edge, float eps2) {
+    const float u = oi_rank_key_score(kv) + 2.002f * (e * rm->qn + rm->cq);
+    return u >= edge - 9.5367431640625e-07f * (fabsf(edge) + eps2);
+}
 __device__ __forceinline__ bool sel_row_keep(const SelRowMargin *rm, uint64_t kv, float edge, float eps2) {
     if (!rm) return true;
-    const float e = rm->meta[2 * (uint64_t)(oi_rank_key_doc(kv) - rm->base) + 1];
-    const float u = oi_rank_key_score(kv) + 2.002f * (e * rm->qn + rm->cq);
-    return u >= edge - 9.5367431640625e-07f * (fabsf(edge) + eps2);
+    return sel_row_test(rm, kv, sel_row_e(rm, kv), edge, eps2);
+}
+
+__device__ __forceinline__ void sel_spec_words(bool have, uint32_t rth_key, float eps2, uint32_t tau, uint32_t *spec_tau, uint32_t *spec_max) {
+    if (!have) { *spec_tau = tau; return; }
+    const float s = oi_key_f32(rth_key) - eps2;
+    const uint32_t T = s == s ? oi_f32_key(s) : 0u;
+    const uint32_t st = T > tau ? T : tau;
+    *spec_tau = st;
+    if (st > tau && st > *spec_max) *spec_max = st;
 }
 
 struct SelShared {
@@ -336,11 +350,93 @@
     __syncthreads();
 }
 
+__device__ __forceinline__ void sel_rank_bin2k(SelShared &sh, uint32_t kk, int pass) {
+    const uint32_t tid = threadIdx.x;
+    {
+        uint32_t v = sh.hist2k[2 * tid] + sh.hist2k[2 * tid + 1];
+        v += (uint32_t)__builtin_amdgcn_update_dpp(0, (int)v, 0x111, 0xf, 0xf, false);
+        v += (uint32_t)__builtin_amdgcn_update_dpp(0, (int)v, 0x112, 0xf, 0xf, false);
+        v += (uint32_t)__builtin_amdgcn_update_dpp(0, (int)v, 0x114, 0xf, 0xf, false);
+        v += (uint32_t)__builtin_amdgcn_update_dpp(0, (int)v, 0x118, 0xf, 0xf, false);
+        if ((tid & 15u) == 15u) sh.hist[tid >> 4] = v;
+    }
+    __syncthreads();
+    if (tid < 64) {
+        const uint32_t x = sh.hist[63u - tid];
+        const uint32_t incl = oi_wave_incl_scan(x);
+        const unsigned long long ball = __ballot(incl >= kk);
+        if (!ball) {
+            if (tid == 0) sh.bin_cnt = 0xFFFFFFFFu;
+        } else {
+            const uint32_t l1 = (uint32_t)__builtin_ctzll(ball), sb = 63u - l1;
+            const uint32_t kk2 = kk - (uint32_t)__builtin_amdgcn_readlane((int)(incl - x), (int)l1);
+            const uint32_t y = tid < 32u ? sh.hist2k[32u * sb + 31u - tid] : 0u;
+            const uint32_t incl2 = oi_wave_incl_scan(y);
+            const unsigned long long ball2 = __ballot(incl2 >= kk2);
+            const uint32_t l2 = ball2 ? (uint32_t)__builtin_ctzll(ball2) : 31u;
+            const uint32_t above = (uint32_t)__builtin_amdgcn_readlane((int)(incl2 - y), (int)l2);
+            if (tid == 0) {
+                sh.prefix = (uint64_t)(32u * sb + 31u - l2);
+                sh.kk = kk2 - above;
+                sh.bin_cnt = 1u;
+#ifdef OI_ABLATION
+                if (sel_dbg_on > 1) {
+                    uint32_t cum = 0; int dd = 2047;
+                    for (; dd >= 0; --dd) { if (cum + sh.hist2k[dd] >= kk) break; cum += sh.hist2k[dd]; }
+                    if ((uint32_t)dd != (uint32_t)sh.prefix || kk - cum != sh.kk)
+                        printf("MISMATCH q=%u pass=%d kk=%u: walk (%d, %u) super-bin (%u, %u) sb=%u l1=%u kk2=%u l2=%u\n", blockIdx.x, pass, kk, dd, kk - cum,
+                               (uint32_t)sh.prefix, sh.kk, sb, l1, kk2, l2);
+                }
+#endif
+            }
+        }
+    }
+    __syncthreads();
+}
+
+template <class FE>
+__device__ __forceinline__ uint32_t sel_rth_score_key(FE &&for_each, uint32_t r, SelShared &sh) {
+    const uint32_t tid = threadIdx.x;
+    uint32_t kk = r, pfx = 0;
+#pragma unroll
+    for (int pass = 0; pass < 3; ++pass) {
+        const int shift = pass == 0 ? 21 : pass == 1 ? 10 : 0, bits = pass == 2 ? 10 : 11;
+        sh.hist2k[tid] = 0;
+        sh.hist2k[tid + SEL_THREADS] = 0;
+        __syncthreads();
+        if (pass == 0) {
+            uint32_t run_d = 0, run_c = 0;
+            for_each([&](bool valid, uint64_t kv) {
+                if (valid) {
+                    const uint32_t d = (uint32_t)(kv >> 53);
+                    if (run_c && d != run_d) { atomicAdd(&sh.hist2k[run_d], run_c); run_c = 0; }
+                    run_d = d;
+                    ++run_c;
+                }
+            });
+            sel_hist_add_w(sh.hist2k, run_c != 0u, run_d, run_c);
+        } else {
+            for_each([&](bool valid, uint64_t kv) {
+                const uint32_t sk = (uint32_t)(kv >> 32);
+                if (valid && (sk >> (shift + bits)) == pfx) atomicAdd(&sh.hist2k[(sk >> shift) & ((1u << bits) - 1u)], 1u);
+            });
+        }
+        __syncthreads();
+        sel_rank_bin2k(sh, kk, 2 + pass);
+        const uint32_t d = sh.bin_cnt != 0xFFFFFFFFu ? (uint32_t)sh.prefix : 0u;
+        kk = sh.kk;
+        __syncthreads();
+        pfx = (pfx << bits) | d;
+    }
+    return pfx;
+}
+
 template <int KPT>
 __device__ __forceinline__ uint32_t sel_flat_select(const SelFlat &K, uint32_t k, SelShared &sh, uint64_t *sel,
                                                     uint64_t *cand, float eps2, bool *in_cand, uint32_t *margin_tau,
                                                     bool *margin_overflow, const uint32_t *skip, uint32_t skip_base,
-                                                    uint64_t *mc, uint32_t mcap, const SelRowMargin *rm) {
+                                                    uint64_t *mc, uint32_t mcap, const SelRowMargin *rm, uint64_t *carry,
+                                                    bool *in_carry, uint32_t spec_rank, uint32_t *spec_key) {
     auto skipped = [&](uint64_t kv) -> bool {
         const uint32_t d = oi_rank_key_doc(kv) - skip_base;
         return (skip[d >> 5] >> (d & 31u)) & 1u;
@@ -425,46 +521,7 @@
                 });
             }
             __syncthreads();
-            {
-                uint32_t v = sh.hist2k[2 * tid] + sh.hist2k[2 * tid + 1];
-                v += (uint32_t)__builtin_amdgcn_update_dpp(0, (int)v, 0x111, 0xf, 0xf, false);
-                v += (uint32_t)__builtin_amdgcn_update_dpp(0, (int)v, 0x112, 0xf, 0xf, false);
-                v += (uint32_t)__builtin_amdgcn_update_dpp(0, (int)v, 0x114, 0xf, 0xf, false);
-                v += (uint32_t)__builtin_amdgcn_update_dpp(0, (int)v, 0x118, 0xf, 0xf, false);
-                if ((tid & 15u) == 15u) sh.hist[tid >> 4] = v;
-            }
-            __syncthreads();
-            if (tid < 64) {
-                const uint32_t x = sh.hist[63u - tid];
-                const uint32_t incl = oi_wave_incl_scan(x);
-                const unsigned long long ball = __ballot(incl >= kk);
-                if (!ball) {
-                    if (tid == 0) sh.bin_cnt = 0xFFFFFFFFu;
-                } else {
-                    const uint32_t l1 = (uint32_t)__builtin_ctzll(ball), sb = 63u - l1;
-                    const uint32_t kk2 = kk - (uint32_t)__builtin_amdgcn_readlane((int)(incl - x), (int)l1);
-                    const uint32_t y = tid < 32u ? sh.hist2k[32u * sb + 31u - tid] : 0u;
-                    const uint32_t incl2 = oi_wave_incl_scan(y);
-                    const unsigned long long ball2 = __ballot(incl2 >= kk2);
-                    const uint32_t l2 = ball2 ? (uint32_t)__builtin_ctzll(ball2) : 31u;
-                    const uint32_t above = (uint32_t)__builtin_amdgcn_readlane((int)(incl2 - y), (int)l2);
-                    if (tid == 0) {
-                        sh.prefix = (uint64_t)(32u * sb + 31u - l2);
-                        sh.kk = kk2 - above;
-                        sh.bin_cnt = 1u;
-#ifdef OI_ABLATION
-                        if (sel_dbg_on > 1) {
-                            uint32_t cum = 0; int dd = 2047;
-                            for (; dd >= 0; --dd) { if (cum + sh.hist2k[dd] >= kk) break; cum += sh.hist2k[dd]; }
-                            if ((uint32_t)dd != (uint32_t)sh.prefix || kk - cum != sh.kk)
-                                printf("MISMATCH q=%u pass=%d kk=%u: walk (%d, %u) super-bin (%u, %u) sb=%u l1=%u kk2=%u l2=%u\n", blockIdx.x, pass, kk, dd, kk - cum,
-                                       (uint32_t)sh.prefix, sh.kk, sb, l1, kk2, l2);
-                        }
-#endif
-                    }
-                }
-            }
-            __syncthreads();
+            sel_rank_bin2k(sh, kk, pass);
             enough = sh.bin_cnt != 0xFFFFFFFFu;
             const uint32_t d = (uint32_t)sh.prefix;
             kk = sh.kk;
@@ -481,18 +538,65 @@
             uint32_t mine = 0;
             const float edge = oi_key_f32(tkey);
             auto keep = [&](bool valid, uint64_t kv) { return valid && (uint32_t)(kv >> 32) >= t32 && sel_row_keep(rm, kv, edge, eps2); };
-            for_each([&](bool valid, uint64_t kv) { mine += keep(valid, kv) ? 1u : 0u; });
+            uint32_t verdict = 0;
+            if constexpr (KPT > 0) {
+#pragma unroll
+                for (int j = 0; j < KPT; ++j)
+                    if ((uint32_t)j < kpt && first + (uint32_t)j * 64 < n && !((dead >> j) & 1u) && (uint32_t)(key[j] >> 32) >= t32) verdict |= 1u << j;
+                if (rm) {
+                    constexpr int G = KPT < 8 ? KPT : 8;
+#pragma unroll
+                    for (int j0 = 0; j0 < KPT; j0 += G) {
+                        if ((uint32_t)j0 < kpt) {
+                            float e[G];
+#pragma unroll
+                            for (int u = 0; u < G; ++u) e[u] = (verdict >> (j0 + u)) & 1u ? sel_row_e(rm, key[j0 + u]) : 0.f;
+#pragma unroll
+                            for (int u = 0; u < G; ++u)
+                                if (((verdict >> (j0 + u)) & 1u) && !sel_row_test(rm, key[j0 + u], e[u], edge, eps2)) verdict &= ~(1u << (j0 + u));
+                        }
+                    }
+                }
+                mine = (uint32_t)__popc(verdict);
+            } else {
+                for_each([&](bool valid, uint64_t kv) { mine += keep(valid, kv) ? 1u : 0u; });
+            }
             const uint32_t incl = oi_wave_incl_scan(mine);
             const uint32_t tot = (uint32_t)__builtin_amdgcn_readlane((int)incl, 63);
             uint32_t base = 0;
             if (lane == 0 && tot) base = atomicAdd(&sh.cnt, tot);
             uint32_t pos = (uint32_t)__builtin_amdgcn_readfirstlane((int)base) + incl - mine;
-            for_each([&](bool valid, uint64_t kv) {
-                if (keep(valid, kv)) {
-                    if (pos < mcap) mc[pos] = kv;
-                    ++pos;
+            if constexpr (KPT > 0) {
+                uint32_t stored = 0;
+#pragma unroll
+                for (int j = 0; j < KPT; ++j) {
+                    if ((verdict >> j) & 1u) {
+                        if (pos < mcap) { carry[pos] = key[j]; stored |= 1u << j; }
+                        ++pos;
+                    }
                 }
-            });
+                *in_carry = true;
+                __syncthreads();
+                const uint32_t c = sh.cnt, kept = c > mcap ? mcap : c;
+                SEL_STAMP(5);
+                if (spec_rank && kept >= spec_rank)
+                    *spec_key = sel_rth_score_key([&](auto &&f) {
+#pragma unroll
+                        for (int j = 0; j < KPT; ++j)
+                            if ((uint32_t)j < kpt) f((stored >> j) & 1u, key[j]);
+                    }, spec_rank, sh);
+                *in_cand = true;
+                *margin_tau = t32;
+                *margin_overflow = c > mcap;
+                return kept;
+            } else {
+                for_each([&](bool valid, uint64_t kv) {
+                    if (keep(valid, kv)) {
+                        if (pos < mcap) mc[pos] = kv;
+                        ++pos;
+                    }
+                });
+            }
             __syncthreads();
             const uint32_t c = sh.cnt;
             *in_cand = true;
@@ -594,7 +698,8 @@
     uint32_t carry_cap, uint32_t seg_cap, uint32_t n_segs, uint32_t seg_cnt_stride, uint32_t *overflow,
     uint32_t k, int compact, float *out_scores, uint32_t *out_docs, uint32_t *out_counts, uint32_t out_stride,
     const float *eps2, uint32_t *margin_gate, const uint32_t *run_gate, const uint32_t *skip, uint32_t skip_base,
-    uint64_t *cand_g, uint32_t cand_cap, const float *row_meta, uint32_t meta_base, const float *row_qn, const float *row_cq) {
+    uint64_t *cand_g, uint32_t cand_cap, const float *row_meta, uint32_t meta_base, const float *row_qn, const float *row_cq,
+    uint32_t spec_rank, uint32_t *spec_tau, uint32_t *spec_max) {
     if (run_gate && *run_gate == 0u) return;
     __shared__ SelShared sh;
     __shared__ uint64_t sel[2 * SEL_MAX];
@@ -652,19 +757,27 @@
     SEL_STAMP(1);
 
     uint32_t m, m_tau = 0;
-    bool in_cand = false, m_over = false;
-    if (K.n <= 4 * SEL_THREADS) m = sel_flat_select<4>(K, k, sh, sel, cand, e2, &in_cand, &m_tau, &m_over, skip, skip_base, mc, mcap, rm);
-    else if (K.n <= 8 * SEL_THREADS) m = sel_flat_select<8>(K, k, sh, sel, cand, e2, &in_cand, &m_tau, &m_over, skip, skip_base, mc, mcap, rm);
-    else if (K.n <= 16 * SEL_THREADS) m = sel_flat_select<16>(K, k, sh, sel, cand, e2, &in_cand, &m_tau, &m_over, skip, skip_base, mc, mcap, rm);
-    else if (K.n <= SEL_KPT_MAX * SEL_THREADS) m = sel_flat_select<SEL_KPT_MAX>(K, k, sh, sel, cand, e2, &in_cand, &m_tau, &m_over, skip, skip_base, mc, mcap, rm);
-    else m = sel_flat_select<0>(K, k, sh, sel, cand, e2, &in_cand, &m_tau, &m_over, skip, skip_base, mc, mcap, rm);
+    bool in_cand = false, m_over = false, in_carry = false;
+    uint32_t spec_key = 0;
+    if (K.n <= 4 * SEL_THREADS) m = sel_flat_select<4>(K, k, sh, sel, cand, e2, &in_cand, &m_tau, &m_over, skip, skip_base, mc, mcap, rm, pool, &in_carry, spec_rank, &spec_key);
+    else if (K.n <= 8 * SEL_THREADS) m = sel_flat_select<8>(K, k, sh, sel, cand, e2, &in_cand, &m_tau, &m_over, skip, skip_base, mc, mcap, rm, pool, &in_carry, spec_rank, &spec_key);
+    else if (K.n <= 16 * SEL_THREADS) m = sel_flat_select<16>(K, k, sh, sel, cand, e2, &in_cand, &m_tau, &m_over, skip, skip_base, mc, mcap, rm, pool, &in_carry, spec_rank, &spec_key);
+    else if (K.n <= SEL_KPT_MAX * SEL_THREADS) m = sel_flat_select<SEL_KPT_MAX>(K, k, sh, sel, cand, e2, &in_cand, &m_tau, &m_over, skip, skip_base, mc, mcap, rm, pool, &in_carry, spec_rank, &spec_key);
+    else m = sel_flat_select<0>(K, k, sh, sel, cand, e2, &in_cand, &m_tau, &m_over, skip, skip_base, mc, mcap, rm, pool, &in_carry, spec_rank, &spec_key);
     if (in_cand) {
         if (m_over && tid == 0 && margin_gate) *margin_gate = 1u;
-        for (uint32_t i = tid; i < m; i += SEL_THREADS) pool[i] = mc[i];
+        if (!in_carry)
+            for (uint32_t i = tid; i < m; i += SEL_THREADS) pool[i] = mc[i];
         for (uint32_t sg = tid; sg < n_segs; sg += SEL_THREADS) segc[sg] = 0;
+        if (spec_rank && !in_carry && m >= spec_rank)
+            spec_key = sel_rth_score_key([&](auto &&f) {
+                for (uint32_t i0 = 0; i0 < m; i0 += SEL_THREADS) f(i0 + tid < m, mc[i0 + tid < m ? i0 + tid : 0]);
+            }, spec_rank, sh);
         if (tid == 0) {
             carry_cnt[q] = m;
-            if (tau_keys && m_tau > tau_keys[q]) tau_keys[q] = m_tau;
+            uint32_t tau = tau_keys ? tau_keys[q] : 0u;
+            if (tau_keys && m_tau > tau) tau_keys[q] = tau = m_tau;
+            if (spec_rank) sel_spec_words(m >= spec_rank, spec_key, e2, tau, spec_tau + q, spec_max + q);
         }
 #ifdef OI_ABLATION
         __syncthreads();
@@ -709,6 +822,14 @@
                 const uint32_t t = (uint32_t)(sh.min_key >> 32);
                 if (t > tau_keys[q]) tau_keys[q] = t;
             }
+        }
+        if (spec_rank) {
+            __syncthreads();
+            if (m >= spec_rank)
+                spec_key = sel_rth_score_key([&](auto &&f) {
+                    for (uint32_t i0 = 0; i0 < m; i0 += SEL_THREADS) f(i0 + tid < m, sel[i0 + tid < m ? i0 + tid : 0]);
+                }, spec_rank, sh);
+            if (tid == 0) sel_spec_words(m >= spec_rank, spec_key, e2, tau_keys ? tau_keys[q] : 0u, spec_tau + q, spec_max + q);
         }
     }
 }
@@ -735,6 +856,9 @@
         OI_REQUIRE(!extra->eps2 || (compact && !out_scores && pool.carry_cap >= mcap),
                    "select: margin mode compacts into a carry region of >= %u keys", mcap);
     }
+    const bool spec = extra && extra->spec_rank;
+    OI_REQUIRE(!spec || (extra->eps2 && extra->spec_tau && extra->spec_max && pool.tau_keys),
+               "select: a speculative threshold needs margin mode, thresholds and both output arrays");
     if ((!v1 || special) && pool.n_segs <= SEL_MAX_SEGS) {
         hipLaunchKernelGGL(select_flat_kernel, dim3(n_queries), dim3(SEL_THREADS), 0, ctx->stream, pool.keys,
                            pool.carry_cnt, pool.seg_cnt, pool.tau_keys, pool.stride, pool.carry_cap, pool.seg_cap,
@@ -743,7 +867,8 @@
                            extra ? extra->run_gate : nullptr, extra && extra->eps2 ? extra->skip_bitmap : nullptr,
                            extra ? extra->skip_base : 0u, extra && extra->eps2 ? extra->cand : nullptr,
                            extra && extra->eps2 ? extra->cand_cap : 0u, extra && extra->eps2 ? extra->row_meta : nullptr,
-                           extra ? extra->meta_base : 0u, extra ? extra->row_qn : nullptr, extra ? extra->row_cq : nullptr);
+                           extra ? extra->meta_base : 0u, extra ? extra->row_qn : nullptr, extra ? extra->row_cq : nullptr,
+                           spec ? extra->spec_rank : 0u, spec ? extra->spec_tau : nullptr, spec ? extra->spec_max : nullptr);
         OI_HIP_CHECK(hipGetLastError());
         return OI_OK;
     }
```

Result: faster. 34030 (median of 6 runs) (+3.6%).
